# whatshap/whatshap

Hardware: AMD Instinct MI355X
Metric: variant-columns/sec at max-coverage 20 (bipartition-costs/sec reported alongside) (higher is better)
Workload: dtype u32; 1 GPU; synthetic diploid single-individual, max-coverage 20: 1 block of 200000 SNVs (BASELINE configs[2]); blocks=1, blocks_in_flight_per_gpu=1, tables_per_launch=1, max_coverage=20, optimal_cost_checksum=1611545, rendezvous=none

## Files before the change

include/whatshap_amd_debug.h:

```cpp
#ifndef WHATSHAP_AMD_DEBUG_H
#define WHATSHAP_AMD_DEBUG_H

#include "whatshap_amd.h"

#ifdef __cplusplus
extern "C" {
#endif

whamd_status_t whamd_debug_emulate_slot_plan(const whamd_readset_view* readset, const uint32_t* recombcost, size_t n_recombcost,
                                            const whamd_pedigree_view* pedigree, int distrust_genotypes,
                                            const uint32_t* positions, size_t n_positions, int slot_l, int symmetry,
                                            uint32_t* index_out, uint32_t* score_out, uint64_t* n_run_columns_out);

whamd_status_t whamd_debug_emulate_pedslot_plan(const whamd_readset_view* readset, const uint32_t* recombcost, size_t n_recombcost,
                                               const whamd_pedigree_view* pedigree, int distrust_genotypes,
                                               const uint32_t* positions, size_t n_positions, int slot_l,
                                               uint32_t* index_out, uint32_t* transmission_out, uint32_t* score_out,
                                               uint64_t* n_run_columns_out);

whamd_status_t whamd_debug_lazy_terms_check(const whamd_readset_view* readset, const uint32_t* recombcost, size_t n_recombcost,
                                            const whamd_pedigree_view* pedigree, int distrust_genotypes,
                                            const uint32_t* positions, size_t n_positions, const uint8_t* need, int rounds,
                                            int* lazy_out, uint64_t* differences_out, uint64_t* built_before_out, uint64_t* built_after_out);

// ... 5 lines not shown
whamd_status_t whamd_debug_realign_detect_host(const whamd_realign_alignments_view* alignments, const whamd_realign_variants_view* variants,
                                               const whamd_realign_reference_view* reference, const whamd_realign_params* params,
                                               whamd_realign** out);
whamd_status_t whamd_debug_edit_distance_host(uint64_t n_pairs, const uint64_t* query_ptr, const uint8_t* query, const uint64_t* target_ptr,
                                              const uint8_t* target, int use_affine, const float* mismatch_cost, int32_t gap_start,
                                              int32_t gap_extend, int64_t* distance_out);

whamd_status_t whamd_debug_poly_score_host(const whamd_poly_matrix_view* matrices, uint64_t n_matrices, uint32_t min_overlap, uint32_t ploidy,
                                           double err, whamd_poly_scores** out);

whamd_status_t whamd_debug_progeny_score_host(const whamd_progeny_view* problems, uint64_t n_problems, whamd_progeny_scores** out);
whamd_status_t whamd_debug_progeny_score_entries_host(const whamd_progeny_view* problem, uint64_t n_entries, const uint32_t* i, const uint32_t* j,
                                                      double* score_out, uint8_t* stored_out);
whamd_status_t whamd_debug_progeny_pair_score_host(const float* gl, uint64_t n_positions, uint32_t n_samples, uint32_t ploidy, uint64_t pos1,
                                                   uint64_t pos2, uint32_t kind, double* score_out);
whamd_status_t whamd_debug_progeny_variant_types_host(const float* gl, uint64_t n_positions, uint32_t n_samples, uint32_t ploidy, const double* priors,
                                                      const uint32_t* nodes, uint64_t n_nodes, double* llh_out, uint32_t* g0_out, uint32_t* g1_out);

whamd_status_t whamd_debug_haplotag_host(const whamd_haplotag_view* problems, uint64_t n_problems, whamd_haplotag_result** out);

typedef struct whamd_debug_kernel {
	const void* kernel;
	const char* name;
	int32_t large_lds_opted_in;
	int32_t debug_only;
} whamd_debug_kernel;
size_t whamd_debug_solve_kernels(whamd_debug_kernel* out, size_t capacity);

enum {
	WHAMD_LAUNCH_COLUMN = 0,
	WHAMD_LAUNCH_RUN = 1,
	WHAMD_LAUNCH_SLOT_RUN = 2,
	WHAMD_LAUNCH_BATCH = 3,
	WHAMD_LAUNCH_GROUP = 4,
	WHAMD_LAUNCH_GROUP_WALK = 5,
	WHAMD_LAUNCH_TAIL = 6,
	WHAMD_LAUNCH_WINDOW_WALK = 7,
	WHAMD_LAUNCH_TABLES = 8
};

typedef struct whamd_debug_launch {
	const void* kernel;
	uint32_t site;
	uint32_t grid_x, grid_y, block;
	uint32_t lds;
	uint32_t own_stream;
	uint32_t forward;
	int32_t lr, yflags, spec, stamps, tb, nf, ncols, threads;
	int32_t streamed, pack;
	int32_t tight, variant;
	int32_t T, n_ind, mode, wide;
	int32_t ped, sym;
	int32_t entries;
	uint64_t count;
	const char* name;
} whamd_debug_launch;
whamd_status_t whamd_debug_dptable_launches(const whamd_dptable* table, whamd_debug_launch* out, size_t capacity, size_t* n_out);

#ifdef __cplusplus
}
#endif

#endif
```

whatshap_amd/_native.py:

```python

from __future__ import annotations

import ctypes as C
import os
import threading
from typing import Optional, Sequence

import numpy as np

_HERE = os.path.dirname(os.path.abspath(__file__))
LIB_PATH = os.path.join(_HERE, "libwhatshap_amd.so")
DEBUG_LIB_PATH = os.path.join(_HERE, "libwhatshap_amd_debug.so")
ABI_VERSION = 2

WHAMD_OK = 0
WHAMD_ERR_INVALID = 1
WHAMD_ERR_MENDELIAN_CONFLICT = 2
WHAMD_ERR_UNSORTED = 3
WHAMD_ERR_UNSUPPORTED = 4
WHAMD_ERR_DEVICE = 5
WHAMD_ERR_OVERFLOW = 6
WHAMD_ERR_HOST = 7
GT_OTHER = 255

# ... 274 lines not shown
                f"{LIB_PATH} is missing: build the HIP extension first "
                "(python -c 'import __graft_entry__ as g; g.build()' or make -C whatshap_amd/csrc). "
                "whatshap_amd has no CPU fallback."
            )
        _lib = _bind(C.CDLL(LIB_PATH), LIB_PATH)
    return _lib


def debug_lib() -> C.CDLL:
    global _debug_lib
    if _debug_lib is not None:
        return _debug_lib
    if not os.path.exists(DEBUG_LIB_PATH):
        raise ImportError(f"{DEBUG_LIB_PATH} is missing: make -C whatshap_amd/csrc debug (tests and timing scripts only)")
    L = _bind(C.CDLL(DEBUG_LIB_PATH), DEBUG_LIB_PATH)
    L.whamd_debug_emulate_slot_plan.restype = C.c_int
    L.whamd_debug_emulate_slot_plan.argtypes = [
        C.POINTER(ReadSetView), C.POINTER(C.c_uint32), C.c_size_t, C.POINTER(PedigreeView), C.c_int,
        C.POINTER(C.c_uint32), C.c_size_t, C.c_int, C.c_int, C.POINTER(C.c_uint32), C.POINTER(C.c_uint32), C.POINTER(C.c_uint64),
    ]
    L.whamd_debug_emulate_pedslot_plan.restype = C.c_int
    L.whamd_debug_emulate_pedslot_plan.argtypes = [
        C.POINTER(ReadSetView), C.POINTER(C.c_uint32), C.c_size_t, C.POINTER(PedigreeView), C.c_int,
        C.POINTER(C.c_uint32), C.c_size_t, C.c_int, C.POINTER(C.c_uint32), C.POINTER(C.c_uint32), C.POINTER(C.c_uint32), C.POINTER(C.c_uint64),
    ]
    L.whamd_debug_pedmec_heuristic_create_host.restype = C.c_int
    L.whamd_debug_pedmec_heuristic_create_host.argtypes = [C.POINTER(ReadSetView), C.POINTER(C.c_uint32), C.c_size_t, C.POINTER(PedigreeView), C.c_int,
                                                           C.POINTER(C.c_uint32), C.c_size_t, C.c_uint32, C.c_int, C.POINTER(C.c_void_p)]
    L.whamd_debug_realign_detect_host.restype = C.c_int
    L.whamd_debug_realign_detect_host.argtypes = [C.POINTER(RealignAlignmentsView), C.POINTER(RealignVariantsView), C.POINTER(RealignReferenceView),
                                                  C.POINTER(RealignParams), C.POINTER(C.c_void_p)]
    L.whamd_debug_edit_distance_host.restype = C.c_int
    L.whamd_debug_edit_distance_host.argtypes = [C.c_uint64, C.POINTER(C.c_uint64), C.POINTER(C.c_uint8), C.POINTER(C.c_uint64), C.POINTER(C.c_uint8),
                                                 C.c_int, C.POINTER(C.c_float), C.c_int32, C.c_int32, C.POINTER(C.c_int64)]
    L.whamd_debug_poly_score_host.restype = C.c_int
    L.whamd_debug_poly_score_host.argtypes = [C.POINTER(PolyMatrixView), C.c_uint64, C.c_uint32, C.c_uint32, C.c_double, C.POINTER(C.c_void_p)]
    L.whamd_debug_progeny_score_host.restype = C.c_int
    L.whamd_debug_progeny_score_host.argtypes = [C.POINTER(ProgenyView), C.c_uint64, C.POINTER(C.c_void_p)]
    L.whamd_debug_progeny_score_entries_host.restype = C.c_int
    L.whamd_debug_progeny_score_entries_host.argtypes = [C.POINTER(ProgenyView), C.c_uint64, C.POINTER(C.c_uint32), C.POINTER(C.c_uint32),
                                                         C.POINTER(C.c_double), C.POINTER(C.c_uint8)]
    L.whamd_debug_progeny_pair_score_host.restype = C.c_int
    L.whamd_debug_progeny_pair_score_host.argtypes = [C.POINTER(C.c_float), C.c_uint64, C.c_uint32, C.c_uint32, C.c_uint64, C.c_uint64, C.c_uint32,
                                                      C.POINTER(C.c_double)]
    L.whamd_debug_progeny_variant_types_host.restype = C.c_int
    L.whamd_debug_progeny_variant_types_host.argtypes = [C.POINTER(C.c_float), C.c_uint64, C.c_uint32, C.c_uint32, C.POINTER(C.c_double), C.POINTER(C.c_uint32),
                                                         C.c_uint64, C.POINTER(C.c_double), C.POINTER(C.c_uint32), C.POINTER(C.c_uint32)]
    L.whamd_debug_haplotag_host.restype = C.c_int
    L.whamd_debug_haplotag_host.argtypes = [C.POINTER(HaplotagView), C.c_uint64, C.POINTER(C.c_void_p)]
    L.whamd_debug_solve_kernels.restype = C.c_size_t
    L.whamd_debug_solve_kernels.argtypes = [C.POINTER(DebugKernel), C.c_size_t]
    L.whamd_debug_dptable_launches.restype = C.c_int
    L.whamd_debug_dptable_launches.argtypes = [C.c_void_p, C.POINTER(DebugLaunch), C.c_size_t, C.POINTER(C.c_size_t)]
    _debug_lib = L
    return L


def use_debug_library() -> None:
    global _lib
    _lib = debug_lib()


def _bind(L: C.CDLL, path: str) -> C.CDLL:
    H = C.c_void_p
    L.whamd_abi_version.restype = C.c_int
    L.whamd_device_count.restype = C.c_int
    L.whamd_last_error.restype = C.c_char_p
    L.whamd_dptable_create.restype = C.c_int
    L.whamd_dptable_create.argtypes = [
        C.POINTER(ReadSetView), C.POINTER(C.c_uint32), C.c_size_t, C.POINTER(PedigreeView), C.c_int,
        C.POINTER(C.c_uint32), C.c_size_t, C.c_int, C.POINTER(H),
    ]
    L.whamd_dptable_create_with_options.restype = C.c_int
    L.whamd_dptable_create_with_options.argtypes = [
        C.POINTER(ReadSetView), C.POINTER(C.c_uint32), C.c_size_t, C.POINTER(PedigreeView), C.c_int,
        C.POINTER(C.c_uint32), C.c_size_t, C.POINTER(C.c_char_p), C.POINTER(C.c_char_p), C.c_size_t, C.c_int, C.POINTER(H),
    ]
    L.whamd_dptable_solve.restype = C.c_int
    L.whamd_dptable_solve.argtypes = [H]
    L.whamd_dptable_enqueue.restype = C.c_int
    L.whamd_dptable_enqueue.argtypes = [H]
    L.whamd_dptable_wait.restype = C.c_int
    L.whamd_dptable_wait.argtypes = [H]
    L.whamd_dptable_enqueue_many.restype = C.c_int
    L.whamd_dptable_enqueue_many.argtypes = [C.POINTER(H), C.c_size_t]
    L.whamd_dptable_wait_many.restype = C.c_int
    L.whamd_dptable_wait_many.argtypes = [C.POINTER(H), C.c_size_t]
    L.whamd_dptable_release_device.restype = C.c_int
    L.whamd_dptable_release_device.argtypes = [H]
    L.whamd_dptable_destroy.restype = None
    L.whamd_dptable_destroy.argtypes = [H]
    L.whamd_dptable_column_count.restype = C.c_uint64
    L.whamd_dptable_column_count.argtypes = [H]
    L.whamd_dptable_individual_count.restype = C.c_uint32
    L.whamd_dptable_individual_count.argtypes = [H]
    L.whamd_dptable_read_count.restype = C.c_uint32
    L.whamd_dptable_read_count.argtypes = [H]
    L.whamd_dptable_positions.restype = C.c_int
    L.whamd_dptable_positions.argtypes = [H, C.POINTER(C.c_uint32)]
    L.whamd_dptable_get_optimal_score.restype = C.c_int
    L.whamd_dptable_get_optimal_score.argtypes = [H, C.POINTER(C.c_uint32)]
    L.whamd_dptable_get_super_reads.restype = C.c_int
    L.whamd_dptable_get_super_reads.argtypes = [
        H, C.POINTER(C.c_uint8), C.POINTER(C.c_uint8), C.POINTER(C.c_uint32), C.POINTER(C.c_uint32), C.POINTER(C.c_uint32),
    ]
    L.whamd_dptable_get_optimal_partitioning.restype = C.c_int
# ... 260 lines not shown
def plan_summary(problem: ProblemArrays, path: str = "auto") -> dict:
    out = PlanSummary()
    _check(lib().whamd_plan_summarize(*problem.call_args(), path.encode(), C.byref(out)))
    return out.as_dict()


def emulate_slot_plan(problem: ProblemArrays, n_columns: int, slot_l: int = 11, symmetry: int = 1, slot_r: int = 2):
    if slot_r >= 3:
        slot_l += 100
    elif slot_r <= 1:
        slot_l += 200
    idx = np.zeros(max(n_columns, 1), dtype=np.uint32)
    score = C.c_uint32()
    ncols = C.c_uint64()
    D = debug_lib()
    _check(D.whamd_debug_emulate_slot_plan(*problem.call_args(), C.c_int(slot_l), C.c_int(symmetry), _ptr(idx, C.c_uint32),
                                           C.byref(score), C.byref(ncols)), D)
    return idx[:n_columns], int(score.value), int(ncols.value)


def emulate_pedslot_plan(problem: ProblemArrays, n_columns: int, slot_l: int = 0):
    idx = np.zeros(max(n_columns, 1), dtype=np.uint32)
    trans = np.zeros(max(n_columns, 1), dtype=np.uint32)
    score = C.c_uint32()
    ncols = C.c_uint64()
    D = debug_lib()
    _check(D.whamd_debug_emulate_pedslot_plan(*problem.call_args(), C.c_int(slot_l), _ptr(idx, C.c_uint32), _ptr(trans, C.c_uint32),
                                              C.byref(score), C.byref(ncols)), D)
    return idx[:n_columns], trans[:n_columns], int(score.value), int(ncols.value)


def debug_lazy_terms_check(problem: ProblemArrays, need=None, rounds: int = 1) -> dict:
    D = debug_lib()
    fn = D.whamd_debug_lazy_terms_check
    fn.restype = C.c_int
    lazy, diff, before, after = C.c_int(), C.c_uint64(), C.c_uint64(), C.c_uint64()
    need_arr = None if need is None else np.ascontiguousarray(need, dtype=np.uint8)
    _check(fn(*problem.call_args(), None if need_arr is None else _ptr(need_arr, C.c_uint8), C.c_int(int(rounds)), C.byref(lazy), C.byref(diff),
              C.byref(before), C.byref(after)), D)
    return {"lazy": bool(lazy.value), "differences": int(diff.value), "built_before": int(before.value), "built_after": int(after.value)}


class DebugKernel(C.Structure):
    _fields_ = [("kernel", C.c_void_p), ("name", C.c_char_p), ("large_lds_opted_in", C.c_int32), ("debug_only", C.c_int32)]


LAUNCH_SITES = ("column", "run", "slot_run", "batch", "group", "group_walk", "tail", "window_walk", "tables")
LAUNCH_FACTS = ("lr", "yflags", "spec", "stamps", "tb", "nf", "ncols", "threads", "streamed", "pack", "tight", "variant", "T", "n_ind", "mode", "wide",
                "ped", "sym", "entries")


class DebugLaunch(C.Structure):
    _fields_ = ([("kernel", C.c_void_p), ("site", C.c_uint32), ("grid_x", C.c_uint32), ("grid_y", C.c_uint32), ("block", C.c_uint32), ("lds", C.c_uint32),
                 ("own_stream", C.c_uint32), ("forward", C.c_uint32)] + [(f, C.c_int32) for f in LAUNCH_FACTS] + [("count", C.c_uint64), ("name", C.c_char_p)])


def debug_solve_kernels() -> list:
    D = debug_lib()
    n = D.whamd_debug_solve_kernels(None, 0)
    arr = (DebugKernel * n)()
    D.whamd_debug_solve_kernels(arr, n)
    return [{"kernel": k.kernel, "name": k.name.decode(), "large_lds_opted_in": bool(k.large_lds_opted_in), "debug_only": bool(k.debug_only)} for k in arr]


def debug_launches(table) -> list:
    D = debug_lib()
    if table._L is not D:
        raise ValueError("the launch ledger exists in the debug library only (use_debug_library() before the table is made)")
    n = C.c_size_t()
    _check(D.whamd_debug_dptable_launches(table._h, None, 0, C.byref(n)), D)
    arr = (DebugLaunch * max(n.value, 1))()
    _check(D.whamd_debug_dptable_launches(table._h, arr, n.value, C.byref(n)), D)
    out = []
    for r in arr[:n.value]:
        if r.name is None:
            raise RuntimeError(f"a launch of site {LAUNCH_SITES[r.site]} (grid {r.grid_x} x {r.grid_y}, block {r.block}) took a kernel the registry does not list")
        rec = {"name": r.name.decode(), "site": LAUNCH_SITES[r.site], "grid_x": r.grid_x, "grid_y": r.grid_y, "block": r.block, "lds": r.lds,
               "own_stream": bool(r.own_stream), "forward": bool(r.forward), "count": int(r.count)}
        rec.update({f: (None if getattr(r, f) < 0 else getattr(r, f)) for f in LAUNCH_FACTS})
        out.append(rec)
    return out


def _heuristic_result(L, h) -> dict:
    n = int(L.whamd_pedmec_heuristic_column_count(h))
    ns = int(L.whamd_pedmec_heuristic_sample_count(h))
    nr = int(L.whamd_pedmec_heuristic_read_count(h))
    score = C.c_float()
    bip = np.zeros(max(nr, 1), dtype=np.uint8)
    trans = np.zeros(max(n, 1), dtype=np.uint32)
    haps = np.zeros((max(ns, 1), 2, max(n, 1)), dtype=np.int8)
    mut = np.zeros((max(ns, 1), 2, max(n, 1)), dtype=np.uint8)
    sid = np.zeros(max(ns, 1), dtype=np.uint32)
    pos = np.zeros(max(n, 1), dtype=np.uint32)
    _check(L.whamd_pedmec_heuristic_get(h, C.byref(score), _ptr(bip, C.c_uint8), _ptr(trans, C.c_uint32), haps.ctypes.data_as(C.POINTER(C.c_int8)),
                                        _ptr(mut, C.c_uint8), _ptr(sid, C.c_uint32), _ptr(pos, C.c_uint32)), L)
    stats = HeuristicStats()
    _check(L.whamd_pedmec_heuristic_get_stats(h, C.byref(stats)), L)
    return {"score": float(score.value), "bipartition": bip[:nr], "transmission": trans[:n], "haplotypes": haps[:ns, :, :n], "mutated": mut[:ns, :, :n],
            "sample_ids": sid[:ns], "positions": pos[:n], "stats": stats.as_dict()}


def pedmec_heuristic(problem: ProblemArrays, row_limit: int = 256, allow_mutations: bool = True, device: int = 0, host_diagnostic: bool = False) -> dict:
    L = debug_lib() if host_diagnostic else lib()
    h = C.c_void_p()
    a = problem.call_args()
    if host_diagnostic:
        _check(L.whamd_debug_pedmec_heuristic_create_host(*a, C.c_uint32(int(row_limit)), C.c_int(1 if allow_mutations else 0), C.byref(h)), L)
    else:
        _check(L.whamd_pedmec_heuristic_create(*a, C.c_uint32(int(row_limit)), C.c_int(1 if allow_mutations else 0), C.c_int(int(device)), C.byref(h)))
    try:
        return _heuristic_result(L, h)
    finally:
        L.whamd_pedmec_heuristic_destroy(h)


class HeuristicBatch:

    def __init__(self, problems, row_limit: int = 256, allow_mutations: bool = True, device: int = 0):
        L = lib()
        problems = list(problems)
        self._L = L
        self._n = len(problems)
        self._handles = (C.c_void_p * max(self._n, 1))()
        jobs = (HeuristicJob * max(self._n, 1))()
        for i, p in enumerate(problems):
            jobs[i].readset = C.pointer(p.readset_view)
            jobs[i].recombcost = _ptr(p.recombcost, C.c_uint32)
            jobs[i].n_recombcost = p.recombcost.size
            jobs[i].pedigree = C.pointer(p.pedigree_view)
            jobs[i].distrust_genotypes = 1 if p.distrust_genotypes else 0
# ... 97 lines not shown
```

whatshap_amd/blocks.py:

```python

from __future__ import annotations

import contextlib

from typing import Dict, List, Sequence, Tuple

import numpy as np

from ._native import ProblemArrays


def block_weight(n_columns: int, coverage: int, transmissions: int = 1) -> float:
    return float(n_columns) * float(2 ** coverage) * float(transmissions) ** 2


def assign_blocks(weights: Sequence[float], world_size: int) -> List[List[int]]:
    order = sorted(range(len(weights)), key=lambda b: (-weights[b], b))
    load = [0.0] * world_size
    out: List[List[int]] = [[] for _ in range(world_size)]
    for b in order:
        r = min(range(world_size), key=lambda i: (load[i], i))
        out[r].append(b)
        load[r] += weights[b]
    return out
# ... 35 lines not shown
    out = []
    for b, (c0, c1) in enumerate(bounds):
        reads = order[cuts[b]:cuts[b + 1]]
        lengths = lengths_all[reads]
        if reads.size and np.all(np.diff(reads) == 1):
            sel = slice(int(ptr[reads[0]]), int(ptr[reads[-1] + 1]))
        else:
            sel = np.concatenate([np.arange(ptr[r], ptr[r + 1]) for r in reads]) if reads.size else np.zeros(0, np.int64)
        sub_ptr = np.zeros(reads.size + 1, dtype=np.uint64)
        sub_ptr[1:] = np.cumsum(lengths)
        sub = ProblemArrays(sub_ptr, problem.var_position[sel], problem.var_allele[sel], problem.var_quality[sel],
                            problem.read_sample_id[reads], problem.individual_id, problem.triple_ids, geno[:, c0:c1],
                            None if gl is None else gl[:, c0:c1, :], recomb[c0:c1], positions[c0:c1],
                            problem.distrust_genotypes, n_variants=c1 - c0)
        out.append((sub, reads, (c0, c1)))
    return out


_CREATE_POOLS = {}


@contextlib.contextmanager
def _create_pool(n_workers: int):
    from concurrent.futures import ThreadPoolExecutor

    pool = _CREATE_POOLS.get(n_workers)
    if pool is None:
        pool = _CREATE_POOLS[n_workers] = ThreadPoolExecutor(max_workers=n_workers, thread_name_prefix="whamd-create")
    yield pool


def solve_blocks(problems: Sequence[ProblemArrays], device: int = 0, path=None, max_in_flight: int = 8,
                 release: bool = True, devices: Sequence[int] = None, weights: Sequence[float] = None, create_threads: int = None,
                 windows_on_device: int = 1, trace: list = None, eager_create: bool = False, host_threads_per_create: int = None):
    from ._native import NativeTable, device_count, enqueue_many, wait_many

    problems = list(problems)
    if create_threads is None or host_threads_per_create is None:
        import os

        n_cpus = len(os.sched_getaffinity(0))
        if create_threads is None:
            create_threads = max(1, min(16, n_cpus))
        if host_threads_per_create is None:
            host_threads_per_create = max(1, min(2, n_cpus // max(1, create_threads)))
    if devices is None:
        from concurrent.futures import ThreadPoolExecutor

        windows = [problems[start:start + max_in_flight] for start in range(0, len(problems), max_in_flight)]
        tables = []
        n_workers = max(1, min(create_threads, max_in_flight))
        with _create_pool(n_workers) as pool:
            def options_of(window):
                opts = {}
                if len(window) > 4:
                    opts["shared_launches"] = "1"
                if n_workers > 1 and len(window) > 1:
                    opts["host_threads"] = str(max(1, int(host_threads_per_create)))
                return opts or None

            def create(sub, opts):
                return NativeTable(sub, device=device, path=path, solve=False, options=opts)

            def submit_window(window):
                opts = options_of(window)
                return [pool.submit(create, sub, opts) for sub in window]

            all_pending = [submit_window(w) for w in windows] if eager_create else None
            pending = (all_pending[0] if eager_create else submit_window(windows[0])) if windows else []
            releases = []
            in_flight = None

            def collect(window):
                wait_many(window)
                if release:
                    releases.extend(pool.submit(t.release_device) for t in window)
                tables.extend(window)

            import time
            t_begin = time.perf_counter()

            def mark(what, wi):
                if trace is not None:
                    trace.append((what, wi, (time.perf_counter() - t_begin) * 1e3))

            window = None
            ok = False
            try:
                for wi in range(len(windows)):
                    window = [f.result() for f in pending]
                    pending = []
                    mark("created", wi)
                    enqueue_many(window)
                    mark("enqueued", wi)
                    pending = ((all_pending[wi + 1] if eager_create else submit_window(windows[wi + 1])) if wi + 1 < len(windows) else [])
                    if windows_on_device < 2:
                        collect(window)
                        window = None
                        mark("collected", wi)
                        continue
                    if in_flight is not None:
                        done, in_flight = in_flight, None
                        collect(done)
                        mark("collected", wi - 1)
                    in_flight, window = window, None
                if in_flight is not None:
                    done, in_flight = in_flight, None
                    collect(done)
                ok = True
            finally:
                if not ok:
                    leftovers = list(in_flight or []) + [t for t in (window or []) if t not in (in_flight or [])]
# ... 255 lines not shown
```

whatshap_amd/csrc/c_api.cpp:

```cpp
#include <chrono>
#include <cstdio>
#include <cstdlib>
#include <cstring>
#include <functional>
#include <memory>
#include <new>
#include <stdexcept>
#include <string>

#include "debug_build.h"
#ifdef WHAMD_DEBUG_BUILD
#include "../../include/whatshap_amd_debug.h"
#endif
#include "device_runtime.h"
#include "device_table.h"
#include "genotype.h"
#include "heuristic.h"
#include "host_parallel.h"
#include "problem.h"
#include "resident.h"
#include "slots.h"
#include <algorithm>
#include <vector>

// ... 31 lines not shown
		return fail(WHAMD_ERR_HOST, "host-side failure (unknown exception)");
	}
}

double now_ms() {
	return std::chrono::duration<double, std::milli>(std::chrono::steady_clock::now().time_since_epoch()).count();
}

}

namespace whamd {
void set_last_error(const std::string& msg) { g_last_error = msg; }
}

extern "C" {

int whamd_abi_version(void) { return WHAMD_ABI_VERSION; }

int whamd_device_count(void) { return DeviceTable::device_count(); }

whamd_status_t whamd_device_pci_bus_id(int device, char* out, size_t capacity) {
	if (!out || capacity < 16) return fail(WHAMD_ERR_INVALID, "whamd_device_pci_bus_id: buffer of at least 16 bytes expected");
	std::string id;
	if (!DeviceTable::device_pci_bus_id(device, id)) return fail(WHAMD_ERR_DEVICE, "no HIP device " + std::to_string(device));
	if (id.size() + 1 > capacity) return fail(WHAMD_ERR_INVALID, "whamd_device_pci_bus_id: buffer too small");
	std::memcpy(out, id.c_str(), id.size() + 1);
	return WHAMD_OK;
}

const char* whamd_last_error(void) { return g_last_error.c_str(); }

namespace {
whamd_status_t apply_option(whamd_dptable* t, const std::string& k, const char* value);

whamd_status_t create_table(const whamd_readset_view* readset, const uint32_t* recombcost, size_t n_recombcost, const whamd_pedigree_view* pedigree,
                            int distrust_genotypes, const uint32_t* positions, size_t n_positions, const char* const* keys, const char* const* values,
                            size_t n_options, int device, whamd_dptable** out) {
	if (!out) return fail(WHAMD_ERR_INVALID, "out is NULL");
	*out = nullptr;
	if (n_options && (!keys || !values)) return fail(WHAMD_ERR_INVALID, "option arrays are NULL");
	const double t0 = now_ms();
	std::unique_ptr<whamd_dptable> t(new whamd_dptable());
	std::string msg;
	struct ThreadsGuard { uint32_t saved = whamd::host_threads_override(); ~ThreadsGuard() { whamd::host_threads_override() = saved; } } threads_guard;
	for (size_t i = 0; i < n_options; ++i) {
		if (!keys[i] || !values[i]) return fail(WHAMD_ERR_INVALID, "null option");
		if (std::string(keys[i]) == "host_threads") whamd::host_threads_override() = (uint32_t)std::max(0, std::atoi(values[i]));
	}
	whamd_status_t st = build_problem(readset, recombcost, n_recombcost, pedigree, distrust_genotypes != 0,
	                                  positions, n_positions, t->problem, msg, false, true);
	if (st != WHAMD_OK) return fail(st, msg);
	const double t1 = now_ms();
	t->device_index = device;
	for (size_t i = 0; i < n_options; ++i) {
		if (std::string(keys[i]) == "host_threads") continue;
		st = apply_option(t.get(), keys[i], values[i]);
		if (st != WHAMD_OK) return st;
	}
	st = t->device.upload(t->problem, device, msg);
	if (st != WHAMD_OK) return fail(st, msg);
	if (getenv("WHAMD_DEBUG_TIMING"))
		fprintf(stderr, "[whamd timing] create: flatten %.1f ms, plan + upload %.1f ms\n", t1 - t0, now_ms() - t1);
	t->uploaded = true;
	t->stats.host_prepare_ms = now_ms() - t0;
	t->stats.host_flatten_ms = t1 - t0;
	*out = t.release();
	return WHAMD_OK;
}
}

whamd_status_t whamd_dptable_create(const whamd_readset_view* readset, const uint32_t* recombcost,
                                    size_t n_recombcost, const whamd_pedigree_view* pedigree,
                                    int distrust_genotypes, const uint32_t* positions, size_t n_positions,
                                    int device, whamd_dptable** out) {
	return guarded([&]() -> whamd_status_t {
		return create_table(readset, recombcost, n_recombcost, pedigree, distrust_genotypes, positions, n_positions, nullptr, nullptr, 0, device, out);
	});
}

whamd_status_t whamd_dptable_create_with_options(const whamd_readset_view* readset, const uint32_t* recombcost,
                                                 size_t n_recombcost, const whamd_pedigree_view* pedigree,
                                                 int distrust_genotypes, const uint32_t* positions, size_t n_positions,
                                                 const char* const* keys, const char* const* values, size_t n_options,
                                                 int device, whamd_dptable** out) {
	return guarded([&]() -> whamd_status_t {
		return create_table(readset, recombcost, n_recombcost, pedigree, distrust_genotypes, positions, n_positions, keys, values, n_options, device, out);
	});
}

namespace {

whamd_status_t begin_enqueue(whamd_dptable* t) {
	if (!t) return fail(WHAMD_ERR_INVALID, "table is NULL");
	if (t->in_flight) return fail(WHAMD_ERR_INVALID, "a solve of this table is already in flight");
	std::string msg;
	if (!t->uploaded) {
		whamd_status_t st = t->device.upload(t->problem, t->device_index, msg);
		if (st != WHAMD_OK) return fail(st, msg);
		t->uploaded = true;
	}
	const Problem& p = t->problem;
	whamd_solve_stats& s = t->stats;
	s.n_columns = p.n_cols;
	s.n_cells = p.n_cells;
	s.n_costs = p.n_cells * p.T;
	s.algorithmic_bytes = p.algorithmic_bytes;
	s.max_coverage = p.max_k;
	s.transmissions = p.T;
	t->solved = false;
	return WHAMD_OK;
}

// ... 238 lines not shown
	if (index_out) std::memcpy(index_out, s.path_index.data(), s.path_index.size() * sizeof(uint32_t));
	if (transmission_out) std::memcpy(transmission_out, s.path_trans.data(), s.path_trans.size() * sizeof(uint32_t));
	return WHAMD_OK;
}

whamd_status_t whamd_dptable_get_stats(const whamd_dptable* t, whamd_solve_stats* stats_out) {
	if (!t || !stats_out) return fail(WHAMD_ERR_INVALID, "null argument");
	whamd_dptable* tt = const_cast<whamd_dptable*>(t);
	if (t->solved && !t->in_flight) tt->device.read_timing(tt->stats);
	*stats_out = t->stats;
	return WHAMD_OK;
}

namespace {
whamd_status_t apply_option(whamd_dptable* t, const std::string& k, const char* value) {
	const std::string v(value);
	if (k == "path") {
		if (!t->device.set_path(v)) return fail(WHAMD_ERR_INVALID, "unknown path '" + v + "' (auto, slots, resident, column, column_keys)");
		t->uploaded = false;
		return WHAMD_OK;
	}
	if (k == "resident_fold") {
		t->device.set_fold(v != "0");
		t->uploaded = false;
		return WHAMD_OK;
	}
	if (k == "symmetry") {
		t->device.set_symmetry(std::atoi(value));
		t->uploaded = false;
		return WHAMD_OK;
	}
	if (k == "lanes") {
		t->device.set_lanes(std::atoi(value));
		t->uploaded = false;
		return WHAMD_OK;
	}
	if (k == "resident_l") {
		t->device.set_l_pref(std::atoi(value));
		t->uploaded = false;
		return WHAMD_OK;
	}
	if (k == "slot_l") {
		t->device.set_slot_l(std::atoi(value));
		t->uploaded = false;
		return WHAMD_OK;
	}
	if (k == "slot_r") {
		t->device.set_slot_lr(std::atoi(value));
		t->uploaded = false;
		return WHAMD_OK;
	}
	if (k == "shared_launches") {
		t->device.set_shared_launches(v != "0");
		t->uploaded = false;
		return WHAMD_OK;
	}
	if (k == "arena_limit_bytes") {
		t->device.set_arena_limit(std::strtoull(value, nullptr, 10));
		t->uploaded = false;
		return WHAMD_OK;
	}
	return fail(WHAMD_ERR_INVALID, "unknown option '" + k + "'");
}
}

whamd_status_t whamd_dptable_set_option(whamd_dptable* t, const char* key, const char* value) {
	if (!t || !key || !value) return fail(WHAMD_ERR_INVALID, "null argument");
	return apply_option(t, key, value);
}

whamd_status_t whamd_plan_summarize(const whamd_readset_view* readset, const uint32_t* recombcost, size_t n_recombcost,
                                    const whamd_pedigree_view* pedigree, int distrust_genotypes,
                                    const uint32_t* positions, size_t n_positions, const char* path,
                                    whamd_plan_summary* out) {
	return guarded([&]() -> whamd_status_t {
	if (!out) return fail(WHAMD_ERR_INVALID, "out is NULL");
	Problem p;
	std::string msg;
	const double tb0 = now_ms();
	const std::string mode(path ? path : "auto");
	whamd_status_t st = build_problem(readset, recombcost, n_recombcost, pedigree, distrust_genotypes != 0, positions,
	                                  n_positions, p, msg, mode == "genotype_slots");
	if (st != WHAMD_OK) return fail(st, msg);
	SlotPlan sp;
	if (mode == "genotype_slots") {
		whamd_plan_summary s{};
		s.n_columns = p.n_cols;
		s.max_coverage = p.max_k;
		if (plan_forward_slots(p, 0, 0, sp, 0, true)) {
			s.n_steps = sp.steps.size();
			s.n_runs = sp.runs.size();
			bool ok = true;
			uint32_t expect = 0;
			for (const Step& step : sp.steps) {
				if (step.kind != 2) {
					if (debug_env("WHAMD_DEBUG_PLAN")) fprintf(stderr, "[plan] genotype: column %u outside runs (k=%u b=%u f=%u, next k=%u)\n", step.index, p.k[step.index], p.b[step.index], p.f[step.index], step.index + 1 < p.n_cols ? p.k[step.index + 1] : 0);
					ok = ok && step.index == expect; expect = step.index + 1; continue;
				}
				const SlotRun& run = sp.runs[step.index];
				ok = ok && run.c0 == expect && run.lr == 0 && !run.half && run.ncols >= 1 && run.ncols <= (uint32_t)PSLOT_MAXCOLS;
				expect = run.c0 + run.ncols;
				s.n_resident_columns += run.ncols;
				s.max_run_columns = std::max<uint64_t>(s.max_run_columns, run.ncols);
				s.max_workgroups = std::max<uint64_t>(s.max_workgroups, 1ull << run.g);
				uint32_t starts = 0, ends = 0;
				for (uint32_t i = 0; i < run.ncols; ++i) {
// ... 208 lines not shown
                                            const whamd_pedigree_view* pedigree, int distrust_genotypes, const uint32_t* positions, size_t n_positions,
                                            const uint8_t* need_in, int rounds, int* lazy_out, uint64_t* differences_out, uint64_t* built_before_out,
                                            uint64_t* built_after_out) {
	return guarded([&]() -> whamd_status_t {
	Problem eager, lazy;
	std::string msg;
	whamd_status_t st = build_problem(readset, recombcost, n_recombcost, pedigree, distrust_genotypes != 0, positions, n_positions, eager, msg);
	if (st != WHAMD_OK) return fail(st, msg);
	st = build_problem(readset, recombcost, n_recombcost, pedigree, distrust_genotypes != 0, positions, n_positions, lazy, msg, false, true);
	if (st != WHAMD_OK) return fail(st, msg);
	if (lazy_out) *lazy_out = lazy.lazy_terms ? 1 : 0;
	const uint32_t n = eager.n_cols;
	uint64_t before = 0, after = 0, diff = 0;
	for (uint32_t c = 0; c < n; ++c) before += lazy.term_end(c, lazy.T - 1) > lazy.term_begin(c, 0);
	std::vector<uint8_t> need(n, 1);
	if (need_in) for (uint32_t c = 0; c < n; ++c) need[c] = need_in[c] != 0;
	rounds = std::max(1, rounds);
	for (int r = 0; r < rounds; ++r) {
		std::vector<uint8_t> part(n, 0);
		for (uint32_t c = 0; c < n; ++c) part[c] = need[c] && (int)(c % (uint32_t)rounds) == r;
		st = fill_lazy_terms(lazy, part, msg);
		if (st != WHAMD_OK) return fail(st, msg);
	}
	for (uint32_t c = 0; c < n; ++c) {
		after += lazy.term_end(c, lazy.T - 1) > lazy.term_begin(c, 0);
		if (!need[c]) continue;
		bool same = true;
		for (uint32_t t = 0; t < eager.T && same; ++t) {
			const uint64_t a0 = eager.term_begin(c, t), a1 = eager.term_end(c, t), b0 = lazy.term_begin(c, t), b1 = lazy.term_end(c, t);
			same = a1 - a0 == b1 - b0;
			for (uint64_t i = 0; same && i < a1 - a0; ++i)
				same = eager.terms[a0 + i].c == lazy.terms[b0 + i].c && eager.terms[a0 + i].plus == lazy.terms[b0 + i].plus && eager.terms[a0 + i].minus == lazy.terms[b0 + i].minus;
		}
		diff += !same;
	}
	if (eager.fterm_kind != lazy.fterm_kind || eager.fterms.size() != lazy.fterms.size()) diff += n;
	else for (size_t i = 0; i < eager.fterms.size(); ++i) if (eager.fterms[i].c != lazy.fterms[i].c || eager.fterms[i].plus != lazy.fterms[i].plus || eager.fterms[i].minus != lazy.fterms[i].minus) { ++diff; break; }
	if (lazy.value_bound < eager.value_bound) diff += n;
	if (differences_out) *differences_out = diff;
	if (built_before_out) *built_before_out = before;
	if (built_after_out) *built_after_out = after;
	return WHAMD_OK;
	});
}

size_t whamd_debug_solve_kernels(whamd_debug_kernel* out, size_t capacity) { return DeviceTable::debug_solve_kernels(out, capacity); }

whamd_status_t whamd_debug_dptable_launches(const whamd_dptable* table, whamd_debug_launch* out, size_t capacity, size_t* n_out) {
	if (!table || !n_out) return fail(WHAMD_ERR_INVALID, "null argument");
	if (!table->solved) return fail(WHAMD_ERR_INVALID, "the table has not been solved: its ledger is read after whamd_dptable_wait");
	*n_out = table->device.debug_launches(out, capacity);
	return WHAMD_OK;
}
#endif

}

struct whamd_heuristic;
struct HeuristicBatchState {
	whamd::HeurBatch batch;
	std::vector<whamd_heuristic*> members;
	bool collected = false;
	whamd_status_t status = WHAMD_OK;
	std::string message;
	double t_enqueued = 0.0;
};

struct whamd_heuristic {
	whamd::HeurPlan plan;
	whamd::HeurResult result;
	whamd_heuristic_stats stats{};
	std::shared_ptr<HeuristicBatchState> batch;
	bool finished = false;
};

namespace {
whamd_status_t heuristic_collect(whamd_heuristic* h) {
	if (h->finished) return WHAMD_OK;
	if (!h->batch) return fail(WHAMD_ERR_INVALID, "whamd_pedmec_heuristic_enqueue has not run");
	std::shared_ptr<HeuristicBatchState> st = h->batch;
	if (!st->collected) {
		st->collected = true;
		std::vector<whamd::HeurResult> results(st->members.size());
		st->status = st->batch.wait(results.data(), st->message);
		if (st->status == WHAMD_OK) {
			const double t_done = now_ms();
			whamd::parallel_ranges(st->members.size(), whamd::host_threads(st->members.size(), 1), [&](uint64_t i0, uint64_t i1, uint32_t) {
				for (uint64_t i = i0; i < i1; ++i) {
					whamd_heuristic* m = st->members[i];
					const double t0 = now_ms();
					m->result = std::move(results[i]);
					whamd::heuristic_finish(m->plan, m->result);
					m->stats.max_solutions = m->result.max_solutions;
					m->stats.total_solutions = m->result.total_solutions;
					m->stats.device_ms = m->result.device_ms;
					m->stats.host_prepare_ms += std::max(0.0, (t_done - st->t_enqueued) - m->result.device_ms);
					m->stats.host_finish_ms = now_ms() - t0;
				}
			});
		}
		for (whamd_heuristic* m : st->members) { m->finished = st->status == WHAMD_OK; m->batch.reset(); }
	}
	if (st->status != WHAMD_OK) return fail(st->status, st->message);
	return WHAMD_OK;
}

// ... 188 lines not shown
```

whatshap_amd/csrc/device_table.h:

```cpp
#pragma once
#include <string>

#ifdef WHAMD_DEBUG_BUILD
#include "../../include/whatshap_amd_debug.h"
#endif
#include "device_types.h"
#include "problem.h"

namespace whamd {

class DeviceTable {
public:
	DeviceTable();
	~DeviceTable();
	DeviceTable(const DeviceTable&) = delete;
	DeviceTable& operator=(const DeviceTable&) = delete;

	static int device_count();
	static bool device_pci_bus_id(int device, std::string& out);
	whamd_status_t upload(Problem& p, int device, std::string& msg);
	whamd_status_t solve(const Problem& p, Solution& s, whamd_solve_stats& st, std::string& msg);
	whamd_status_t enqueue(const Problem& p, Solution& s, std::string& msg);
	whamd_status_t enqueue_some(const Problem& p, Solution& s, uint64_t budget, bool& done, std::string& msg);
	whamd_status_t wait(const Problem& p, Solution& s, whamd_solve_stats& st, std::string& msg);
	void read_timing(whamd_solve_stats& st);
	static whamd_status_t enqueue_group(DeviceTable* const* tables, const Problem* const* problems, Solution* const* solutions, size_t n_tables, std::string& msg);
	static void wait_last_of_each_stream(DeviceTable* const* tables, size_t n_tables);
	bool group_eligible(const Problem& p) const;
	int device_index() const;
	uint32_t widest_launch() const;
	void abort_enqueue();
	void release_device();
	bool set_path(const std::string& path);
	void set_l_pref(int l);
	void set_slot_l(int l);
	void set_slot_lr(int lr);
	void set_fold(bool v);
	void set_symmetry(int level);
	void set_lanes(int n);
	void set_arena_limit(uint64_t bytes);
	void set_shared_launches(bool v);
	void set_side_by_side(bool v);

#ifdef WHAMD_DEBUG_BUILD
	static size_t debug_solve_kernels(whamd_debug_kernel* out, size_t capacity);
	size_t debug_launches(whamd_debug_launch* out, size_t capacity) const;
#endif

private:
	whamd_status_t enqueue_some_unguarded(const Problem& p, Solution& s, uint64_t budget, bool& done, std::string& msg);
	struct Impl;
	Impl* impl_;
};

}
```

whatshap_amd/csrc/dp_device.hip:

```cpp
#include <hip/hip_runtime.h>

#include <algorithm>
#include <atomic>
#include <cctype>
#include <chrono>
#include <cstdio>
#include <cstdlib>
#include <cstring>
#include <mutex>
#include <string>
#include <vector>

#include "debug_build.h"
#ifdef WHAMD_DEBUG_BUILD
#include "../../include/whatshap_amd_debug.h"
#endif
#include "device_runtime.h"
#include "device_table.h"
#include "genotype.h"

namespace whamd {

namespace {

// ... 266 lines not shown
	std::vector<SuperStep> schedule;
	struct StepBrief { uint32_t entry_off, lds; uint16_t entry_count; uint8_t has_singles, pad; };
	struct EntryBrief { uint16_t grid_x, threads; uint32_t lds_x; GroupVariantPair variant; uint8_t pad[2]; };
	std::vector<StepBrief> step_brief;
	std::vector<EntryBrief> entry_brief;
	std::vector<ResBatchEntry> entries;
	ResBatchEntry* d_entries = nullptr;
	bool use_chunks = false;
	std::vector<BtChunk> chunks;
	BtChunk* d_chunks = nullptr;
	uint32_t* d_unit_x = nullptr;
	uint32_t* d_path2 = nullptr;
	uint32_t* d_trans2 = nullptr;
	uint32_t n_orient_max = 1;
	uint8_t* d_sel = nullptr;
	uint32_t* d_guess = nullptr;
	uint32_t* d_bt_counters = nullptr;
	uint32_t n_spec = 0;
	size_t chunk_lds = 0;
	SlotPlan splan;
	bool use_slots = false;
	int slot_l = 11;
	bool slot_l_set = false;
	int slot_lr = 2;
	int slot_lr_used = 2;
	std::vector<SlotBatchEntry> slot_entries;
	SlotBatchEntry* d_slot_entries = nullptr;
	uint64_t table_bytes = 0;
	BtJob* d_btjobs = nullptr;
	uint32_t* d_job_scores = nullptr;
	bool shared_hint = false;
	bool side_by_side = false;
	int max_lanes = 32;
	struct Window {
		uint32_t step_lo = 0, step_hi = 0;
		uint32_t unit_off = 0, unit_count = 0;
	};
	uint64_t arena_limit = 0;
	bool windowed = false;
	std::vector<Window> windows;
	uint8_t* d_checkpoints = nullptr;
	size_t checkpoint_bytes = 0;
	uint32_t* d_bt_state = nullptr;
	BtJob* d_window_jobs = nullptr;

	whamd_status_t open(int dev, std::string& msg);
	whamd_status_t choose_plan(Problem& p, TableBuild& b, std::string& msg);
	void dump_plan(const Problem& p) const;
	whamd_status_t describe_columns(const Problem& p, TableBuild& b, std::string& msg);
	whamd_status_t lay_out_arena(const Problem& p, TableBuild& b, std::string& msg);
	size_t upload_bound(const Problem& p, const TableBuild& b) const;
	whamd_status_t upload_column_arrays(const Problem& p, TableBuild& b, TableUploader& up, std::string& msg);
	void build_slot_blobs(TableBuild& b) const;
	uint64_t lay_out_slot_tables(const TableBuild& b);
	whamd_status_t upload_slot_arrays(TableBuild& b, TableUploader& up, std::string& msg);
	void make_jobs();
	void make_units(const TableBuild& b);
	whamd_status_t make_windows(const TableBuild& b, TableUploader& up, std::string& msg);
	whamd_status_t take_result_block(uint32_t n, TableUploader& up, std::string& msg);
	whamd_status_t make_chunks(const Problem& p, TableUploader& up, std::string& msg);
	whamd_status_t take_solve_buffers(const Problem& p, TableBuild& b, TableUploader& up, std::string& msg);
	whamd_status_t make_lanes(const TableBuild& b, TableUploader& up, std::string& msg);
	whamd_status_t make_schedule(const TableBuild& b, std::string& msg);
	void make_briefs();
	whamd_status_t upload_entries(TableUploader& up, std::string& msg);
	whamd_status_t launch_table_kernels(const Problem& p, const TableBuild& b, TableUploader& up, std::string& msg);
	whamd_status_t arm_debug_stamps(TableUploader& up, std::string& msg);
	whamd_status_t record_group_backtrace(uint32_t n, TableUploader& up, std::string& msg);
	struct SolveInFlight {
		hipStream_t run_stream = nullptr;
		uint32_t group_tables = 1;
		bool enqueue_open = false;
		size_t next_super = 0;
		uint64_t launches = 0;
		hipStream_t tail_stream = nullptr;
		uint64_t tail_seq = 0;
		bool tail_elsewhere = false;
		bool timing_pending = false;
		static inline std::atomic<uint64_t> tails_submitted{0};
		void rewind(hipStream_t own) { enqueue_open = false; next_super = 0; run_stream = own; }
	} inflight;
#ifdef WHAMD_DEBUG_BUILD
	std::vector<whamd_debug_launch> ledger;
	void note(uint32_t site, const void* kernel, dim3 grid, dim3 block, size_t lds, hipStream_t on, bool forward, const LaunchFacts& facts);
#endif
	struct GroupSubmission;
	void launch_column_step(const Problem& p, const Step& step, const Lane& lane, const uint32_t* prev, uint32_t* cur, uint64_t& launches);
	void launch_run(const ResBatchEntry& e, uint64_t& launches);
	void launch_slot_run(const SlotBatchEntry& e, uint64_t& launches);
	whamd_status_t begin_solve(const Problem& p, Solution& s, std::string& msg);
	whamd_status_t submit_super_step(const Problem& p, const SuperStep& ss, uint64_t& launches, std::string& msg);
	whamd_status_t submit_singles(const Problem& p, const SuperStep& ss, uint64_t& launches, std::string& msg);
	whamd_status_t submit_tail(const Problem& p, std::string& msg, hipStream_t tail_stream = nullptr, bool walked_by_group = false);
	whamd_status_t report_slot_stamps(std::string& msg) const;
	whamd_status_t report_resident_stamps(std::string& msg) const;
	BtGroupEntry h_bt_entry{};
	BtGroupEntry* d_bt_entry = nullptr;
	bool device_superreads = false;
	SuperreadArgs super_args{};
	size_t super_words = 0, super_off = 0;
	bool own_stream_used = false;
	bool upload_pending = false;
	hipStream_t upload_stream = nullptr;

	void adopt(const StreamSet& ss) { stream = ss.stream; ev0 = ss.ev[0]; ev1 = ss.ev[1]; ev2 = ss.ev[2]; ev3 = ss.ev[3]; ev_group = ss.ev[4]; ev_upload = ss.ev[5]; }
	StreamSet stream_set() const {
		StreamSet ss;
		ss.stream = stream; ss.ev[0] = ev0; ss.ev[1] = ev1; ss.ev[2] = ev2; ss.ev[3] = ev3; ss.ev[4] = ev_group; ss.ev[5] = ev_upload; ss.device = device;
		return ss;
	}

	void release_lanes() {
		max_grid_x = 1;
		lanes.clear();
		jobs.clear();
		schedule.clear();
		entries.clear();
		slot_entries.clear();
		windows.clear();
	}

	void release() {
		if (inflight.tail_elsewhere && ev3) (void)hipEventSynchronize(ev3);
		inflight.tail_elsewhere = false;
		if (upload_pending && ev_upload) (void)hipEventSynchronize(ev_upload);
		upload_pending = false;
		release_lanes();
		windowed = false;
		if (stream && own_stream_used && (!allocations.empty() || d_arena)) { (void)hipStreamSynchronize(stream); own_stream_used = false; }
		for (auto& a : allocations) devpool_give(device, a.first, a.second);
		allocations.clear();
		arena_give(device, d_arena, arena_bytes);
		d_arena = nullptr;
		arena_bytes = 0;
		pinned_give(h_pinned, h_pinned_bytes);
		h_pinned = nullptr;
		d_cols = nullptr;
		d_units = nullptr;
		d_pr[0] = d_pr[1] = nullptr;
		d_path_index = d_path_trans = d_score = nullptr;
	}
};

DeviceTable::DeviceTable() : impl_(new Impl()) {}

DeviceTable::~DeviceTable() {
	if (impl_) {
		release_device();
		delete impl_;
	}
}

void DeviceTable::release_device() {
	Impl& m = *impl_;
	(void)hipSetDevice(m.device);
	m.release();
	if (m.stream) {
		if (m.own_stream_used) (void)hipStreamSynchronize(m.stream);
		m.own_stream_used = false;
		streamset_give(m.stream_set());
	}
	m.adopt(StreamSet());
	m.inflight.run_stream = nullptr;
	m.inflight.timing_pending = false;
}

int DeviceTable::device_count() {
	int n = 0;
	if (hipGetDeviceCount(&n) != hipSuccess) return 0;
	return n;
}

bool DeviceTable::device_pci_bus_id(int device, std::string& out) {
	int n = 0;
	if (hipGetDeviceCount(&n) != hipSuccess || device < 0 || device >= n) return false;
	char text[64] = {0};
	if (hipDeviceGetPCIBusId(text, (int)sizeof text - 1, device) != hipSuccess) return false;
	out = text;
	for (char& ch : out) ch = (char)tolower((unsigned char)ch);
	return true;
}

static void append_segments(uint32_t mask, std::vector<uint32_t>& out, uint16_t& count) {
	uint32_t src = 0;
	count = 0;
	for (uint32_t bit = 0; bit < 32;) {
		if (!((mask >> bit) & 1u)) { ++bit; continue; }
		uint32_t len = 0;
		while (bit + len < 32 && ((mask >> (bit + len)) & 1u)) ++len;
		out.push_back(src | (bit << 8) | (len << 16));
		++count;
		src += len;
		bit += len;
	}
}

bool DeviceTable::set_path(const std::string& path) {
	if (path != "auto" && path != "column" && path != "column_keys" && path != "resident" && path != "slots") return false;
	impl_->path = path;
	return true;
}

void DeviceTable::set_l_pref(int l) { impl_->l_pref = std::max(4, std::min(l, RES_LMAX)); }
void DeviceTable::set_lanes(int n) { impl_->max_lanes = n < 1 ? 1 : (n > 64 ? 64 : n); }

void DeviceTable::set_fold(bool v) { impl_->fold = v; }
void DeviceTable::set_slot_l(int l) { impl_->slot_l = std::max(2, std::min(l, 12)); impl_->slot_l_set = true; }
void DeviceTable::set_slot_lr(int lr) { impl_->slot_lr = lr >= 3 ? 3 : (lr <= 1 ? 1 : 2); }

void DeviceTable::set_arena_limit(uint64_t bytes) { impl_->arena_limit = bytes; }
void DeviceTable::set_shared_launches(bool v) { impl_->shared_hint = v; }
void DeviceTable::set_side_by_side(bool v) { impl_->side_by_side = v; }
void DeviceTable::set_symmetry(int level) { impl_->symmetry = level < 0 ? 0 : (level > 2 ? 2 : level); }


whamd_status_t DeviceTable::Impl::open(int dev, std::string& msg) {
	Impl& m = *this;
	m.device = dev;
	const whamd_status_t opened = open_device(dev, msg);
	if (opened != WHAMD_OK) return opened;
	if (!m.stream) {
		StreamSet ss;
		if (!streamset_take(dev, ss)) { msg = "could not create the table's stream and events"; return WHAMD_ERR_DEVICE; }
		m.adopt(ss);
	}
	m.release();
	return WHAMD_OK;
}

whamd_status_t DeviceTable::Impl::choose_plan(Problem& p, TableBuild& b, std::string& msg) {
	Impl& m = *this;
	m.wide = !select_kernels(p.T, p.n_ind, m.fused, m.keysfn);
	if (m.wide && (p.T > (uint32_t)MAX_T_WIDE || p.n_ind > (uint32_t)MAX_IND_WIDE)) {
		msg = "no device kernel for T=" + std::to_string(p.T) + ", individuals=" + std::to_string(p.n_ind);
		return WHAMD_ERR_UNSUPPORTED;
	}
	for (uint32_t c = 0; c < p.n_cols && !m.wide; ++c) m.wide = p.term_end(c, p.T - 1) - p.term_begin(c, 0) > (uint64_t)COL_MAXTERMS;
	b.force_keys = m.path == "column_keys" || m.wide;
	const bool want_resident = (m.path == "auto" || m.path == "resident") && !m.wide;
	size_t free_b = 0, total_b = 0;
	HIP_TRY(hipMemGetInfo(&free_b, &total_b));
	if (free_b < total_b / 2) {
		genotype_release_cache();
		HIP_TRY(hipMemGetInfo(&free_b, &total_b));
	}
	if (free_b < total_b / 4) {
		arena_release();
		devpool_release();
		HIP_TRY(hipMemGetInfo(&free_b, &total_b));
	}
	free_b += arena_idle_bytes(m.device);
	b.free_b = free_b;
	int slot_lr = m.slot_lr, slot_l = m.slot_l;
	if (m.shared_hint && p.T == 1 && p.max_k >= 18 && !m.slot_l_set && m.slot_lr == 2) { slot_lr = 3; slot_l = 12; }
	if (p.T == 1 && p.max_k >= 21 && p.max_k <= 22 && !m.slot_l_set && m.slot_lr == 2 && !debug_env("WHAMD_NO_WIDE_LAYOUT")) { slot_lr = 3; slot_l = 12; }
	m.slot_lr_used = slot_lr;
	m.use_slots = (m.path == "auto" || m.path == "slots") && !m.wide && plan_forward_slots(p, p.T > 1 ? (m.slot_l_set ? -m.slot_l : 0) : std::max(8, slot_l), m.symmetry, m.splan, slot_lr);
	if (m.use_slots && m.splan.ped && m.splan.table_words * 4ull > free_b / 4) m.use_slots = false;
	m.table_bytes = m.use_slots && m.splan.ped ? m.splan.table_words * 4ull : 0ull;
	if (p.lazy_terms) {
		std::vector<uint8_t> need(p.n_cols, 1);
		if (m.use_slots && m.splan.ped) for (uint32_t c = 0; c < p.n_cols; ++c) need[c] = m.splan.col_to_row[c] < 0;
		const whamd_status_t st = fill_lazy_terms(p, need, msg);
		if (st != WHAMD_OK) return st;
	}
	if (m.use_slots) {
		m.plan = ResidentPlan();
		m.plan.steps = m.splan.steps;
		m.plan.component_first_step = m.splan.component_first_step;
		m.plan.col_to_res.assign(p.n_cols, -1);
	} else {
		m.splan = SlotPlan();
		plan_forward(p, want_resident, m.l_pref, m.fold, m.plan, m.symmetry);
	}
	m.device_superreads = p.n_ind == 1 && p.T == 1 && p.P == 2 && !p.distrust && p.h2p.size() >= 2 && p.h2p[0] == 0 && p.h2p[1] == 1 && p.genotype.size() >= p.n_cols &&
	                      !debug_env("WHAMD_HOST_SUPERREADS");
	return WHAMD_OK;
}

void DeviceTable::Impl::dump_plan(const Problem& p) const {
	const Impl& m = *this;
	for (const Step& st : m.plan.steps) {
		if (st.kind == 0) { fprintf(stderr, "[plan] column %u k=%u b=%u f=%u\n", st.index, p.k[st.index], p.b[st.index], p.f[st.index]); continue; }
		if (st.kind == 2) {
			const SlotRun& r = m.splan.runs[st.index];
			fprintf(stderr, "[plan] slot run c0=%u ncols=%u g=%u L=%u half=%u ends=%u has_prev=%u in_identity=%u in_half=%u mirror_pos=%u in_occ=%x out_occ=%x mirror_out=%u\n",
			        r.c0, r.ncols, r.g, r.L, r.half, r.n_ends, r.has_prev, r.in_identity, r.in_half, r.in_mirror_pos, r.in_occ, r.out_occ, r.mirror_out);
			if (m.splan.ped) fprintf(stderr, "[plan]   pedigree run: T=%u forms per value=%u table words=%u record words per workgroup=%u\n", 1u << m.splan.pextra[st.index].tb,
			                         m.splan.pextra[st.index].nf, m.splan.pextra[st.index].s_off + r.ncols * 64u * pslot_ns(m.splan.pextra[st.index].nf), m.splan.pextra[st.index].rec_words);
			continue;
		}
		const ResSegment& sgm = m.plan.segments[st.index];
		fprintf(stderr, "[plan] run c0=%u ncols=%u g=%u threads=%u max_l=%u stage_words=%u\n", sgm.c0, sgm.ncols, sgm.g, sgm.threads, sgm.max_l, sgm.stage_words);
		for (uint32_t i = 0; i < sgm.ncols; ++i) {
			const ResColumn& rc = m.plan.columns[sgm.col_off + i];
			const ResBacktrace& rb = m.plan.backtrace[sgm.col_off + i];
			fprintf(stderr, "[plan]   col %u mode=%u nfold=%u Lb=%u Lf=%u ebits=%u epos0=%u nthr=%u stage_off=%u nwords=%u | bt layout=%u n_g=%u n_l=%u\n",
			        sgm.c0 + i, rc.mode, rc.nfold, rc.Lb, rc.Lf, rc.ebits, rc.epos[0], rc.nthr, rc.stage_off, rc.nwords, rb.layout, rb.n_g, rb.n_l);
		}
	}
}

whamd_status_t DeviceTable::Impl::describe_columns(const Problem& p, TableBuild& b, std::string& msg) {
	Impl& m = *this;
	const uint32_t n = b.n, ni = b.ni, tbits = b.tbits;
	if (p.terms.size() >= 0xFFFFFFFFull || (uint64_t)p.col_ptr[n] * ni >= 0xFFFFFFFFull) {
		msg = "problem too large for 32-bit device offsets";
		return WHAMD_ERR_UNSUPPORTED;
	}
	m.cols.resize(n);
	b.term_ptr32.resize((size_t)n * (p.T + 1));
	RawVec<uint32_t>& term_ptr32 = b.term_ptr32;
	parallel_ranges(n, host_threads(n, 16384), [&m, &p, &term_ptr32, n, ni, tbits](uint64_t c0, uint64_t c1, uint32_t) {
		for (uint32_t c = (uint32_t)c0; c < (uint32_t)c1; ++c) {
			DevColumn d{};
			d.k = p.k[c];
			d.b = p.b[c];
			d.f = p.f[c];
			d.recomb = p.recomb[c];
			d.delta_off = (uint32_t)(p.col_ptr[c] * ni);
			d.term_off = (uint32_t)((size_t)c * (p.T + 1));
			for (uint32_t t = 0; t <= p.T; ++t) term_ptr32[(size_t)c * (p.T + 1) + t] = (uint32_t)p.term_ptr[(size_t)c * p.T + t];
			d.ebits = d.k - d.f;
			d.is_last = (c + 1 == n);
			d.eloop = std::min<uint32_t>(d.ebits, QMAX);
			d.nplanes = d.ebits + tbits;
			m.cols[c] = d;
		}
	});
	return WHAMD_OK;
}

whamd_status_t DeviceTable::Impl::lay_out_arena(const Problem& p, TableBuild& b, std::string& msg) {
	Impl& m = *this;
	const uint32_t n = b.n;
	const bool ped_slots = b.ped_slots;
	std::vector<uint32_t>& segs = b.segs;
	uint64_t bt = 0, seg_bt = 0;
	size_t seg_cursor = 0, slot_cursor = 0;
	uint32_t max_f = 0, max_keys_f = 0;
	const uint64_t reserve = (3ull << 30) + (uint64_t)n * 1024ull + m.table_bytes;
	auto slot_record_bytes = [&m, ped_slots](size_t ri) -> uint64_t {
		const SlotRun& run = m.splan.runs[ri];
		if (ped_slots) return (uint64_t)m.splan.pextra[ri].rec_words * 4ull << run.g;
		return (uint64_t)run.n_ends * run.threads * (1ull << (run.g - run.half));
	};
	uint64_t arena_cap = b.free_b > reserve ? b.free_b - reserve : 0;
	if (m.arena_limit) arena_cap = std::min<uint64_t>(arena_cap, m.arena_limit);
	b.arena_cap = arena_cap;
	std::vector<uint32_t>& window_first_col = b.window_first_col;
	uint64_t bt_max = 0;
	auto open_unit = [&bt, &bt_max, &window_first_col, arena_cap](uint32_t c, uint64_t bytes) -> bool {
		if (bytes + 16 > arena_cap) return false;
		if (bt + bytes + 16 > arena_cap) {
			bt_max = std::max(bt_max, bt);
			bt = 0;
			window_first_col.push_back(c);
		}
		return true;
	};
	auto unit_too_large = [&msg, &b](uint32_t c) {
		msg = "the backtrace record of the unit at column " + std::to_string(c) + " alone does not fit in the arena (" + std::to_string(b.arena_cap >> 20) +
		      " MiB of " + std::to_string(b.free_b >> 20) + " MiB free HBM)";
		return WHAMD_ERR_UNSUPPORTED;
	};
	for (uint32_t c = 0; c < n; ++c) {
		DevColumn& d = m.cols[c];
		const bool in_slot_run = m.use_slots && m.splan.col_to_row[c] >= 0;
		d.seg_off = (uint32_t)segs.size();
		const uint32_t kmask = d.k >= 32 ? 0xFFFFFFFFu : ((1u << d.k) - 1u);
		if (!in_slot_run) {
			append_segments(p.fwd_mask[c], segs, d.nseg_fwd);
			append_segments(kmask & ~p.fwd_mask[c], segs, d.nseg_end);
		}
		d.bt_off = bt;
		if (m.use_slots && m.splan.col_to_row[c] >= 0) {
			d.mode = 3;
			d.res_idx = (uint32_t)m.splan.col_to_row[c];
			if (slot_cursor < m.splan.runs.size() && m.splan.runs[slot_cursor].c0 == c) {
				SlotRun& run = m.splan.runs[slot_cursor];
				if (!open_unit(c, slot_record_bytes(slot_cursor))) return unit_too_large(c);
				run.rec_lo = (uint32_t)bt;
				run.rec_hi = (uint32_t)(bt >> 32);
				seg_bt = bt;
				bt += slot_record_bytes(slot_cursor);
				max_f = std::max(max_f, run.L + run.g);
				++slot_cursor;
			}
			d.bt_off = seg_bt;
		} else if (m.plan.col_to_res[c] >= 0) {
			d.mode = 2;
			d.res_idx = (uint32_t)m.plan.col_to_res[c];
			if (seg_cursor < m.plan.segments.size() && m.plan.segments[seg_cursor].c0 == c) {
				ResSegment& sgm = m.plan.segments[seg_cursor];
				if (!open_unit(c, (uint64_t)sgm.stage_words * (1ull << sgm.g) * 8ull)) return unit_too_large(c);
				sgm.bt_lo = (uint32_t)bt;
				sgm.bt_hi = (uint32_t)(bt >> 32);
				seg_bt = bt;
				bt += (uint64_t)sgm.stage_words * (1ull << sgm.g) * 8ull;
				++seg_cursor;
			}
			d.bt_off = seg_bt;
		} else {
			const bool fused_ok = !b.force_keys && !d.is_last && d.f >= 6 && d.ebits <= (uint32_t)QMAX;
			d.mode = fused_ok ? 0u : 1u;
			const uint64_t bytes = d.mode == 0 ? (uint64_t)d.nplanes * p.T * (1ull << (d.f - 6)) * 8ull : (uint64_t)p.T * (1ull << d.f) * 4ull;
			if (!open_unit(c, bytes)) return unit_too_large(c);
			d.bt_off = bt;
			bt += bytes;
			if (d.mode != 0) max_keys_f = std::max(max_keys_f, d.f);
		}
		bt = (bt + 15ull) & ~15ull;
		max_f = std::max(max_f, d.f);
	}
	b.laps.lap("column descriptors (host)");
	bt = std::max(bt_max, bt);
	b.bt = bt;
	b.max_f = max_f;
	b.max_keys_f = max_keys_f;
	b.exchange_bytes = (size_t)(1ull << max_f) * p.T * 4;
	m.bt_bytes = bt;
	m.windowed = !window_first_col.empty();
	m.checkpoint_bytes = b.exchange_bytes;
	const uint64_t need = bt + (2ull + window_first_col.size()) * b.exchange_bytes + (1ull << max_keys_f) * p.T * 8ull;
	if (need + (1ull << 30) > b.free_b) {
		msg = "backtrace arena of " + std::to_string(need >> 20) + " MiB does not fit in free HBM (" + std::to_string(b.free_b >> 20) + " MiB)";
		return WHAMD_ERR_UNSUPPORTED;
	}
	return WHAMD_OK;
}

size_t DeviceTable::Impl::upload_bound(const Problem& p, const TableBuild& b) const {
	const Impl& m = *this;
	const size_t delta_count = p.n_ind == 0 ? std::max<size_t>(p.col_ptr[b.n], 1) : (size_t)p.col_ptr[b.n] * p.n_ind;
	const size_t super_upload = m.device_superreads ? ((size_t)b.n + 1) * 8 + b.n + 1024 : 0;
	return m.cols.size() * sizeof(DevColumn) + delta_count * sizeof(int32_t) + b.term_ptr32.size() * 4 + (p.terms.size() + p.fterms.size()) * sizeof(DevTerm) + b.segs.size() * 4 +
	       m.plan.columns.size() * (sizeof(ResColumn) + sizeof(ResBacktrace) + sizeof(PedColumn)) + m.plan.ped_terms.size() * sizeof(PedTerm) +
	       (m.splan.rows.size() + SLOT_ROW_PAD) * sizeof(SlotRow) + m.splan.prows.size() * sizeof(PedSlotRow) + m.splan.bt_cols.size() * (sizeof(SlotBtCol) + 8) +
	       m.splan.runs.size() * (sizeof(SlotRun) + sizeof(PedSlotExtra) + sizeof(BtUnit) + sizeof(SlotBatchEntry) + 64) + m.plan.segments.size() * (sizeof(ResBatchEntry) + sizeof(BtUnit)) + super_upload + ((size_t)8 << 20);
}

whamd_status_t DeviceTable::Impl::upload_column_arrays(const Problem& p, TableBuild& b, TableUploader& up, std::string& msg) {
	Impl& m = *this;
	const uint32_t n = b.n;
	static_assert(sizeof(CostTerm) == sizeof(DevTerm), "Problem::terms / fterms are uploaded as they are");
	const RawVec<CostTerm>& terms = p.terms;
	const int32_t* delta_src = p.delta.data();
	size_t delta_count = (size_t)p.col_ptr[n] * p.n_ind;
	if (p.n_ind == 0) { b.delta_fallback.assign(std::max<size_t>(p.col_ptr[n], 1), 0); delta_src = b.delta_fallback.data(); delta_count = b.delta_fallback.size(); }
	const bool sparse_columns = m.use_slots && !b.ped_slots && p.T == 1 && !m.windowed && !debug_env("WHAMD_DENSE_COLUMN_UPLOAD");
	if (sparse_columns) {
		std::vector<std::pair<size_t, size_t>> pc_cols, pc_delta, pc_tptr, pc_terms;
		for (uint32_t c = 0; c < n;) {
			if (m.splan.col_to_row[c] >= 0) { ++c; continue; }
			uint32_t e = c + 1;
			while (e < n && m.splan.col_to_row[e] < 0) ++e;
			pc_cols.emplace_back((size_t)c * sizeof(DevColumn), (size_t)e * sizeof(DevColumn));
			pc_delta.emplace_back((size_t)p.col_ptr[c] * p.n_ind * sizeof(int32_t), (size_t)p.col_ptr[e] * p.n_ind * sizeof(int32_t));
			pc_tptr.emplace_back((size_t)c * (p.T + 1) * sizeof(uint32_t), (size_t)e * (p.T + 1) * sizeof(uint32_t));
// ... 9 lines not shown
		HIP_TRY(up.up((void**)&m.d_cols, m.cols.data(), m.cols.size() * sizeof(DevColumn)));
		HIP_TRY(up.up((void**)&m.dp.delta, delta_src, delta_count * sizeof(int32_t)));
		HIP_TRY(up.up((void**)&m.dp.term_ptr, b.term_ptr32.data(), b.term_ptr32.size() * sizeof(uint32_t)));
		HIP_TRY(up.up((void**)&m.dp.terms, terms.data(), terms.size() * sizeof(DevTerm)));
	}
	m.dp.cols = m.d_cols;
	if (m.device_superreads) {
		m.super_args = SuperreadArgs{};
		HIP_TRY(up.up((void**)&m.super_args.col_ptr, p.col_ptr.data(), ((size_t)n + 1) * sizeof(uint64_t)));
		HIP_TRY(up.up((void**)&m.super_args.genotype, p.genotype.data(), (size_t)n));
		m.super_args.delta = m.dp.delta;
		m.super_args.n_cols = n;
		m.super_words = (size_t)n + ((size_t)2 * n + 3) / 4;
	}
	b.d_fterms = nullptr;
	if (!p.fterms.empty()) HIP_TRY(up.up((void**)&b.d_fterms, p.fterms.data(), p.fterms.size() * sizeof(DevTerm)));
	HIP_TRY(up.up((void**)&m.dp.segs, b.segs.data(), b.segs.size() * sizeof(uint32_t)));
	HIP_TRY(up.up((void**)&m.dp.res_cols, m.plan.columns.data(), m.plan.columns.size() * sizeof(ResColumn)));
	HIP_TRY(up.up((void**)&m.dp.res_bt, m.plan.backtrace.data(), m.plan.backtrace.size() * sizeof(ResBacktrace)));
	m.plan.ped_columns.resize(m.plan.ped_columns.empty() ? 0 : m.plan.columns.size());
	HIP_TRY(up.up((void**)&m.dp.ped_cols, m.plan.ped_columns.data(), m.plan.ped_columns.size() * sizeof(PedColumn)));
	HIP_TRY(up.up((void**)&m.dp.ped_terms, m.plan.ped_terms.data(), m.plan.ped_terms.size() * sizeof(PedTerm)));
	b.laps.lap("column arrays: allocations + copies");
	return WHAMD_OK;
}

void DeviceTable::Impl::build_slot_blobs(TableBuild& b) const {
	const Impl& m = *this;
	b.slot_blob_off.assign(m.splan.runs.size(), 0);
	b.slot_blob_words.assign(m.splan.runs.size(), 0);
	size_t words = 0;
	for (size_t ri = 0; ri < m.splan.runs.size(); ++ri) {
		const SlotRun& run = m.splan.runs[ri];
		b.slot_blob_off[ri] = (uint32_t)words;
		b.slot_blob_words[ri] = (uint32_t)((size_t)run.ncols * (sizeof(SlotBtCol) / 4) + (run.n_ends + 3) / 4 + 1);
		words += b.slot_blob_words[ri];
	}
	b.slot_blob.resize(words);
	uint32_t* blob = b.slot_blob.data();
	const uint32_t* blob_off = b.slot_blob_off.data();
	parallel_ranges(m.splan.runs.size(), host_threads(m.splan.runs.size(), 512), [&m, blob, blob_off](uint64_t r0, uint64_t r1, uint32_t) {
		for (size_t ri = r0; ri < r1; ++ri) {
			const SlotRun& run = m.splan.runs[ri];
			uint32_t* dst = blob + blob_off[ri];
			const size_t col_words = (size_t)run.ncols * (sizeof(SlotBtCol) / 4);
			std::memcpy(dst, m.splan.bt_cols.data() + run.row_off, col_words * 4);
			const size_t end_words = (run.n_ends + 3) / 4 + 1;
			std::memset(dst + col_words, 0, end_words * 4);
			if (run.n_ends) std::memcpy(dst + col_words, m.splan.end_slots.data() + m.splan.end_off[ri], run.n_ends);
		}
	});
}

uint64_t DeviceTable::Impl::lay_out_slot_tables(const TableBuild& b) {
	Impl& m = *this;
	uint64_t slot_tab_words = 0;
	for (SlotRun& run : m.splan.runs) {
		auto pad4 = [](uint64_t v) { return (v + 3ull) & ~3ull; };
		const bool xrun = (run.yflags & 1u) && (run.lr == 2u || (run.lr == 3u && !debug_env("WHAMD_NO_XRUN8"))) && run.ncols <= (uint32_t)SLOT_XCOLS &&
		                  run.n_ends <= (uint32_t)SLOT_XENDS && !debug_env("WHAMD_NO_XRUN");
		const uint64_t ncp = xrun ? ((run.ncols + 7u) & ~7u) : run.ncols;
		run.tab_g = (uint32_t)slot_tab_words;
		slot_tab_words += pad4(ncp << (run.g - run.half));
		run.tab_w = (uint32_t)slot_tab_words;
		slot_tab_words += pad4(ncp * (run.threads >> 6));
		run.tab_sl = (uint32_t)slot_tab_words;
		slot_tab_words += ncp * 64u;
		if (xrun) {
			run.yflags |= 8u;
			slot_tab_words = (slot_tab_words + 15u) & ~(uint64_t)15;
			run.tab_kr = (uint32_t)slot_tab_words;
			slot_tab_words += pad4((((uint64_t)run.ncols + SLOT_XPAD) << run.lr) + run.ncols + SLOT_XPAD);
			run.tab_par = (uint32_t)slot_tab_words;
			slot_tab_words += pad4((uint64_t)run.threads + (1ull << (run.g - run.half)));
		}
	}
	slot_tab_words += (uint64_t)SLOT_XCOLS * 64u;
	if (b.laps.on) {
		size_t nx = 0, not_y = 0, not_lr = 0, long_run = 0, many_ends = 0;
		for (const SlotRun& run : m.splan.runs) {
			nx += (run.yflags & 8u) != 0;
			not_y += !(run.yflags & 1u); not_lr += run.lr != 2u && run.lr != 3u; long_run += run.ncols > (uint32_t)SLOT_XCOLS; many_ends += run.n_ends > (uint32_t)SLOT_XENDS;
		}
		fprintf(stderr, "[whamd timing]   X runs: %zu of %zu (not Y form %zu, cells per thread %zu, more than %d columns %zu, more than %d ending reads %zu)\n", nx, m.splan.runs.size(), not_y,
		        not_lr, SLOT_XCOLS, long_run, SLOT_XENDS, many_ends);
	}
	return slot_tab_words;
}

whamd_status_t DeviceTable::Impl::upload_slot_arrays(TableBuild& b, TableUploader& up, std::string& msg) {
	Impl& m = *this;
	build_slot_blobs(b);
	b.laps.lap("slot backtrace blobs (host)");
	if (!m.splan.rows.empty()) m.splan.rows.resize(m.splan.rows.size() + SLOT_ROW_PAD);
	HIP_TRY(up.up((void**)&m.dp.slot_rows, m.splan.rows.data(), m.splan.rows.size() * sizeof(SlotRow)));
	b.laps.lap("slot rows: allocation + copy");
	HIP_TRY(up.up((void**)&m.dp.slot_blob, b.slot_blob.data(), b.slot_blob.size() * sizeof(uint32_t)));
	HIP_TRY(up.up((void**)&m.dp.slot_ctrl, m.splan.ctrl.data(), m.splan.ctrl.size() * sizeof(uint32_t)));
	m.dp.slot_tab = nullptr;
	b.d_runs = nullptr;
	if (m.use_slots && !b.ped_slots) {
		const uint64_t slot_tab_words = lay_out_slot_tables(b);
		if (slot_tab_words >= 0xFFFFFFFFull) { msg = "slot-run tables exceed 32-bit offsets"; return WHAMD_ERR_UNSUPPORTED; }
		HIP_TRY(up.up((void**)&b.d_runs, m.splan.runs.data(), m.splan.runs.size() * sizeof(SlotRun)));
		b.laps.lap("slot blobs, control words, runs: allocations + copies");
		HIP_TRY(up.alloc((void**)&m.dp.slot_tab, slot_tab_words * 4));
		b.laps.lap("slot tables: allocation");
	}
	m.dp.pslot_rows = nullptr;
	m.dp.pslot_tab = nullptr;
	b.d_pextra = nullptr;
	if (b.ped_slots) {
		HIP_TRY(up.up((void**)&m.dp.pslot_rows, m.splan.prows.data(), m.splan.prows.size() * sizeof(PedSlotRow)));
		HIP_TRY(up.up((void**)&b.d_runs, m.splan.runs.data(), m.splan.runs.size() * sizeof(SlotRun)));
		HIP_TRY(up.up((void**)&b.d_pextra, m.splan.pextra.data(), m.splan.pextra.size() * sizeof(PedSlotExtra)));
		HIP_TRY(up.alloc((void**)&m.dp.pslot_tab, m.table_bytes));
	}
	b.laps.lap("slot rows / blobs / control words: allocations + copies");
	return WHAMD_OK;
}

void DeviceTable::Impl::make_jobs() {
	Impl& m = *this;
	m.release_lanes();
	Impl::Job final_job;
	final_job.final = true;
	std::vector<Impl::Job> component_jobs;
	const std::vector<uint32_t>& first = m.plan.component_first_step;
	size_t largest = 0;
	for (size_t k = 0; k < first.size(); ++k) largest = std::max<size_t>(largest, (k + 1 < first.size() ? first[k + 1] : m.plan.steps.size()) - first[k]);
	const bool worth_splitting = largest * 5 < m.plan.steps.size() * 4 || debug_env("WHAMD_SPLIT_COMPONENTS");
// ... 115 lines not shown
	m.d_bt_counters = res + 2 * (size_t)n + m.jobs.size();
	if (m.device_superreads) {
		m.super_args.out = res + m.super_off;
		m.super_args.path_index = m.d_path_index;
	}
	return WHAMD_OK;
}

namespace {

struct OrientationGenerators {
	std::vector<int> of_individual;
	std::vector<uint32_t> tflip;
	explicit OrientationGenerators(const Problem& p) : of_individual(std::max<uint32_t>(p.n_ind, 1), -1) {
		if (p.n_ind < 2 || p.n_ind > BT_GENERATORS) return;
		for (uint32_t s = 0; s < p.n_ind; ++s) {
			uint32_t as_parent = 0, as_child = 0;
			for (uint32_t t3 = 0; t3 < p.n_triples; ++t3) {
				if (p.triples[t3][0] == s) as_parent |= 1u << (2 * t3);
				if (p.triples[t3][1] == s) as_parent |= 1u << (2 * t3 + 1);
				if (p.triples[t3][2] == s) as_child |= 3u << (2 * t3);
			}
			if (as_parent && as_child) continue;
			if (!as_parent && !as_child) continue;
			of_individual[s] = (int)tflip.size();
			tflip.push_back(as_parent | as_child);
		}
	}
	void orient(const Problem& p, uint32_t c_last, BtChunk& ch) const {
		ch.n_orient = 1;
		for (uint32_t q = 0; q < BT_GENERATORS; ++q) ch.flip[q] = 0;
		if (p.n_triples == 0 && p.n_ind <= 1) {
			const uint32_t fb = p.f[c_last];
			ch.flip[0] = fb >= BT_STATE_TSHIFT ? BT_STATE_XMASK : ((1u << fb) - 1u);
			ch.n_orient = 2;
			return;
		}
		if (tflip.empty()) return;
		const ColumnEntry* col = p.col_begin(c_last);
		uint32_t bit = 0;
		for (uint32_t j = 0; j < p.k[c_last]; ++j) {
			if (!((p.fwd_mask[c_last] >> j) & 1u)) continue;
			const int gq = of_individual[col[j].sample];
			if (gq >= 0) ch.flip[gq] |= 1u << bit;
			++bit;
		}
		for (size_t q = 0; q < tflip.size(); ++q) ch.flip[q] |= tflip[q] << BT_STATE_TSHIFT;
		ch.n_orient = 1u << tflip.size();
	}
};

}

whamd_status_t DeviceTable::Impl::make_chunks(const Problem& p, TableUploader& up, std::string& msg) {
	Impl& m = *this;
	const uint32_t n = p.n_cols;
	m.use_chunks = false;
	m.chunks.clear();
	m.n_spec = 0;
	for (SlotRun& run : m.splan.runs) run.spec_id = 0;
	const bool trio_runs = !m.use_slots && !m.plan.ped_columns.empty();
	if (trio_runs) for (ResSegment& sgm : m.plan.segments) sgm.in_mirror_bit = 0;
	m.dp.spec_keys = nullptr;
	if (!((m.use_slots || trio_runs) && m.jobs.size() == 1 && !m.windowed && !getenv("WHAMD_BT_SEQUENTIAL") && m.units.size() > 2u * BT_CHUNK_RUNS)) return WHAMD_OK;
	m.use_chunks = true;
	const OrientationGenerators generators(p);
	BtChunk cur{};
	cur.n_orient = 1;
	uint32_t runs_in_chunk = 0;
	for (uint32_t u = 0; u < m.units.size(); ++u) {
		const bool is_run = m.units[u].kind == 2 || m.units[u].kind == 3 || (trio_runs && m.units[u].kind == 1);
		if (is_run && runs_in_chunk >= (uint32_t)BT_CHUNK_RUNS && u > 0) {
			m.chunks.push_back(cur);
			cur = BtChunk{};
			cur.unit_off = u;
			cur.spec_id = ++m.n_spec;
			generators.orient(p, m.units[u].c0 + m.units[u].ncols - 1, cur);
			runs_in_chunk = 0;
			const Step& st = m.plan.steps[m.jobs[0].steps[m.jobs[0].steps.size() - 1 - u]];
			if (trio_runs) m.plan.segments[st.index].in_mirror_bit = m.n_spec;
			else m.splan.runs[st.index].spec_id = m.n_spec;
		}
		runs_in_chunk += is_run;
		++cur.unit_count;
	}
	m.chunks.push_back(cur);
	HIP_TRY(up.up((void**)&m.d_chunks, m.chunks.data(), m.chunks.size() * sizeof(BtChunk)));
	m.n_orient_max = 1;
	for (const BtChunk& ch : m.chunks) m.n_orient_max = std::max(m.n_orient_max, ch.n_orient);
	HIP_TRY(up.alloc((void**)&m.d_unit_x, (size_t)m.n_orient_max * m.units.size() * 4));
	HIP_TRY(up.alloc((void**)&m.d_path2, (size_t)m.n_orient_max * n * 4));
	HIP_TRY(up.alloc((void**)&m.d_trans2, (size_t)m.n_orient_max * n * 4));
	HIP_TRY(up.alloc((void**)&m.d_sel, m.units.size() + 16));
	HIP_TRY(up.alloc((void**)&m.d_guess, m.chunks.size() * 4));
	uint32_t stride = 64;
	for (const SlotRun& run : m.splan.runs) if (run.spec_id) stride = std::max(stride, (run.threads >> 6) << (run.g - run.half));
	if (trio_runs) for (const ResSegment& sgm : m.plan.segments) if (sgm.in_mirror_bit) stride = std::max(stride, (sgm.threads >> 6) << sgm.g);
	m.dp.spec_stride = stride;
	HIP_TRY(up.alloc((void**)&m.dp.spec_keys, ((size_t)m.n_spec + 1) * stride * 8));
	return WHAMD_OK;
}

whamd_status_t DeviceTable::Impl::take_solve_buffers(const Problem& p, TableBuild& b, TableUploader& up, std::string& msg) {
	Impl& m = *this;
	HIP_TRY(up.up((void**)&m.d_units, m.units.data(), m.units.size() * sizeof(BtUnit)));
	{
		uint32_t max_stage = 0;
		for (const ResSegment& sgm : m.plan.segments) max_stage = std::max(max_stage, sgm.stage_words);
		for (size_t ri = 0; ri < m.splan.runs.size(); ++ri)
			max_stage = std::max(max_stage, b.ped_slots ? m.splan.pextra[ri].rec_words / 2u : (m.splan.runs[ri].n_ends * m.splan.runs[ri].threads + 7) / 8);
		m.bt_lds = (size_t)2 * RES_MAXCOLS * 128 + 512 + 16 + (size_t)BT_CELLS * 4 + (size_t)RES_MAXCOLS * 4 + (size_t)max_stage * 8 + 16;
		m.chunk_lds = (size_t)(32 + 4 + BT_CELLS + BT_CHUNK_BLOB) * 4 + (size_t)max_stage * 8 + 16;
	}
	void* d_rtab = nullptr;
	const bool ped_plan = !m.plan.ped_columns.empty();
	HIP_TRY(up.alloc(&d_rtab, m.plan.columns.size() * (ped_plan ? PED_TABLE : RES_TABLE) * sizeof(int32_t)));
	m.dp.res_tables = ped_plan ? nullptr : (int32_t*)d_rtab;
	m.dp.ped_tables = ped_plan ? (int32_t*)d_rtab : nullptr;
	b.laps.lap("jobs, backtrace units, schedule");
	b.laps.next_stage();
	{
		size_t got = 0;
		void* d_bt = arena_take(m.device, b.bt, got);
		if (!d_bt) {
			HIP_TRY(hipMalloc(&d_bt, std::max<size_t>(b.bt, 16)));
			got = std::max<size_t>(b.bt, 16);
		}
		m.d_arena = d_bt;
		m.arena_bytes = got;
		m.dp.bt = (uint8_t*)d_bt;
	}
	b.laps.next_stage();
	m.key_entries = (size_t)(1ull << b.max_keys_f) * p.T;
	HIP_TRY(up.alloc((void**)&m.dp.keys, m.key_entries * 8));
	HIP_TRY(up.alloc((void**)&m.dp.last_keys, (size_t)MAX_T_WIDE * 8));
	HIP_TRY(up.alloc((void**)&m.d_pr[0], b.exchange_bytes));
	HIP_TRY(up.alloc((void**)&m.d_pr[1], b.exchange_bytes));
	HIP_TRY(pinned_take((m.super_off + (m.device_superreads ? m.super_words : 0)) * sizeof(uint32_t), (void**)&m.h_pinned, &m.h_pinned_bytes));
	return WHAMD_OK;
}

whamd_status_t DeviceTable::Impl::make_lanes(const TableBuild& b, TableUploader& up, std::string& msg) {
	Impl& m = *this;
	const size_t lane_bytes = 2 * b.exchange_bytes;
	const size_t by_memory = std::max<size_t>(1, ((size_t)1 << 30) / std::max<size_t>(lane_bytes, 1));
	const size_t n_lanes = std::max<size_t>(1, std::min<size_t>(std::min<size_t>((size_t)m.max_lanes, by_memory), m.jobs.size()));
	m.lanes.assign(n_lanes, Impl::Lane());
	std::vector<uint64_t> load(n_lanes, 0);
	std::vector<uint32_t> order;
	for (uint32_t j = 1; j < m.jobs.size(); ++j) order.push_back(j);
	std::stable_sort(order.begin(), order.end(), [&m](uint32_t x, uint32_t y) { return m.jobs[x].steps.size() > m.jobs[y].steps.size(); });
	m.lanes[0].jobs.push_back(0);
	load[0] = m.jobs[0].steps.size() + 1;
	for (uint32_t j : order) {
		const size_t l = (size_t)(std::min_element(load.begin(), load.end()) - load.begin());
		m.lanes[l].jobs.push_back(j);
		load[l] += m.jobs[j].steps.size() + 1;
	}
	m.lanes[0].d_pr[0] = m.d_pr[0];
	m.lanes[0].d_pr[1] = m.d_pr[1];
	m.lanes[0].d_keys = m.dp.keys;
	for (size_t l = 1; l < n_lanes; ++l) {
		HIP_TRY(up.alloc((void**)&m.lanes[l].d_pr[0], b.exchange_bytes));
		HIP_TRY(up.alloc((void**)&m.lanes[l].d_pr[1], b.exchange_bytes));
		HIP_TRY(up.alloc((void**)&m.lanes[l].d_keys, m.key_entries * 8));
	}
	return WHAMD_OK;
}

whamd_status_t DeviceTable::Impl::make_schedule(const TableBuild& b, std::string& msg) {
	Impl& m = *this;
	const bool ped_slots = b.ped_slots;
	struct Cursor { size_t job_i = 0, step_i = 0; uint32_t flip = 0; };
	std::vector<Cursor> cur(m.lanes.size());
	for (;;) {
		Impl::SuperStep ss;
		ss.entry_off = (uint32_t)(m.use_slots ? m.slot_entries.size() : m.entries.size());
		for (size_t li = 0; li < m.lanes.size(); ++li) {
			Impl::Lane& lane = m.lanes[li];
			Cursor& c = cur[li];
			if (c.job_i == lane.jobs.size()) continue;
			const uint32_t job_id = lane.jobs[c.job_i];
			const Impl::Job& job = m.jobs[job_id];
			const uint32_t si = job.steps[c.step_i];
			const bool first = c.step_i == 0, last = c.step_i + 1 == job.steps.size();
			const Step& step = m.plan.steps[si];
			ss.io[0] = lane.d_pr[c.flip]; ss.io[1] = lane.d_pr[c.flip ^ 1];
			if (step.kind == 2) {
				SlotBatchEntry e{};
				e.run = m.splan.runs[step.index];
// ... 171 lines not shown
		K(resident_segment_ped<false, true>),
		WHAMD_RUNX(24, false), WHAMD_RUNX(32, false), WHAMD_RUNX(0, false), WHAMD_RUNX(8, false), WHAMD_RUNX(16, false),
		K(slot_groupx<2, false>), K(slot_groupx<3, false>),
#ifdef WHAMD_DEBUG_BUILD
		WHAMD_RUNX(24, true), WHAMD_RUNX(32, true),
		WHAMD_PSLOTX(2, 2), WHAMD_PSLOTX(2, 4), WHAMD_PSLOTX(4, 2), WHAMD_PSLOTX(4, 4), WHAMD_PSLOTX(2, 16), WHAMD_PSLOTX(2, PSLOT_FACT),
#endif
		WHAMD_PSLOT(2, 4), WHAMD_PSLOT(4, 2), WHAMD_PSLOT(4, 4),
		WHAMD_PSLOT(2, 16), K(pedslot_group<2, 16>),
		WHAMD_PSLOT(2, PSLOT_FACT), K(pedslot_group<2, PSLOT_FACT>),
		WHAMD_PSLOT(4, PSLOT_FACT4), K(pedslot_group<4, PSLOT_FACT4>),
		K(pedslot_group<2, 2>), K(pedslot_group<2, 4>), K(pedslot_group<4, 2>), K(pedslot_group<4, 4>),
	};
#undef K
#undef WHAMD_RUNX
#undef WHAMD_PSLOT
#undef WHAMD_PSLOTX
	count = sizeof(kernels) / sizeof(kernels[0]);
	return kernels;
}

static whamd_status_t opt_in_large_lds(int device, std::string& msg) {
	static std::mutex attr_mu;
	static unsigned long long attr_done = 0;
	std::lock_guard<std::mutex> lock(attr_mu);
	if (device < 64 && ((attr_done >> device) & 1ull)) return WHAMD_OK;
	size_t count = 0;
	const void* const* kernels = large_lds_kernels(count);
	for (size_t i = 0; i < count; ++i) HIP_TRY(hipFuncSetAttribute(kernels[i], hipFuncAttributeMaxDynamicSharedMemorySize, 160 * 1024));
	if (device < 64) attr_done |= 1ull << device;
	return WHAMD_OK;
}

whamd_status_t DeviceTable::Impl::record_group_backtrace(uint32_t n, TableUploader& up, std::string& msg) {
	Impl& m = *this;
	m.d_bt_entry = nullptr;
	if (!m.use_chunks) return WHAMD_OK;
	BtGroupEntry& e = m.h_bt_entry;
	e = BtGroupEntry{};
	e.P = m.dp;
	e.units = m.d_units; e.chunks = m.d_chunks;
	e.n_chunks = (uint32_t)m.chunks.size(); e.n_units = (uint32_t)m.units.size(); e.n_orient_max = m.n_orient_max; e.n_cols = n;
	e.path2 = m.d_path2; e.trans2 = m.d_trans2; e.out_score = m.d_score; e.unit_x2 = m.d_unit_x; e.guess = m.d_guess; e.sel = m.d_sel; e.counters = m.d_bt_counters;
	e.path_index = m.d_path_index; e.path_trans = m.d_path_trans;
	if (m.device_superreads) e.super = m.super_args;
	void* d_entry = nullptr;
	HIP_TRY(up.alloc(&d_entry, sizeof(BtGroupEntry)));
	HIP_TRY(hipMemcpyAsync(d_entry, &m.h_bt_entry, sizeof(BtGroupEntry), hipMemcpyHostToDevice, up.stream));
	HIP_TRY(hipEventRecord(m.ev_upload, up.stream));
	m.d_bt_entry = (BtGroupEntry*)d_entry;
	return WHAMD_OK;
}

whamd_status_t DeviceTable::upload(Problem& p, int device, std::string& msg) {
	Impl& m = *impl_;
	whamd_status_t st = m.open(device, msg);
	if (st != WHAMD_OK || p.n_cols == 0) return st;
	TableBuild b;
	b.n = p.n_cols;
	b.tbits = 2 * p.n_triples;
	b.ni = std::max<uint32_t>(p.n_ind, 1);
	m.dp.n_cols = b.n;
	m.dp.T = p.T;
	m.dp.tbits = b.tbits;
	m.dp.n_ind = p.n_ind;
	if ((st = m.choose_plan(p, b, msg)) != WHAMD_OK) return st;
	b.ped_slots = m.use_slots && m.splan.ped;
	b.laps.next_stage();
	if (debug_env("WHAMD_DEBUG_PLAN")) m.dump_plan(p);
	if ((st = m.describe_columns(p, b, msg)) != WHAMD_OK) return st;
	if ((st = m.lay_out_arena(p, b, msg)) != WHAMD_OK) return st;
	m.upload_stream = debug_env("WHAMD_UPLOAD_ON_TABLE_STREAM") ? nullptr : upload_stream_of(device);
	if (!m.upload_stream) m.upload_stream = m.stream;
	if (m.upload_stream == m.stream) m.own_stream_used = true;
	TableUploader up(device, m.upload_stream, m.allocations);
	b.laps.lap("staging area taken");
	up.open_block(m.upload_bound(p, b));
	b.laps.lap("staging image sized, device block taken");
	if ((st = m.upload_column_arrays(p, b, up, msg)) != WHAMD_OK) return st;
	if ((st = m.upload_slot_arrays(b, up, msg)) != WHAMD_OK) return st;
	m.make_jobs();
	m.make_units(b);
	if ((st = m.make_windows(b, up, msg)) != WHAMD_OK) return st;
	if ((st = m.take_result_block(b.n, up, msg)) != WHAMD_OK) return st;
	if ((st = m.make_chunks(p, up, msg)) != WHAMD_OK) return st;
	if ((st = m.take_solve_buffers(p, b, up, msg)) != WHAMD_OK) return st;
	if ((st = m.make_lanes(b, up, msg)) != WHAMD_OK) return st;
	if ((st = m.make_schedule(b, msg)) != WHAMD_OK) return st;
	m.make_briefs();
	if ((st = m.upload_entries(up, msg)) != WHAMD_OK) return st;
	if ((st = m.launch_table_kernels(p, b, up, msg)) != WHAMD_OK) return st;
	b.laps.summary((double)b.bt / 1e9);
	if ((st = m.arm_debug_stamps(up, msg)) != WHAMD_OK) return st;
	if ((st = opt_in_large_lds(device, msg)) != WHAMD_OK) return st;
	return m.record_group_backtrace(b.n, up, msg);
}

namespace {

SegmentFn segment_kernel(bool stamps, bool sym) {
#ifdef WHAMD_DEBUG_BUILD
	if (stamps) return resident_segment<true, true>;
#endif
	return sym ? resident_segment<false, true> : resident_segment<false, false>;
}

PedSegmentFn ped_segment_kernel(bool stamps, bool spec) {
#ifdef WHAMD_DEBUG_BUILD
	if (stamps) return resident_segment_ped<true>;
#endif
	return spec ? resident_segment_ped<false, true> : resident_segment_ped<false>;
}

ResBatchFn resident_batch_kernel(bool sym) { return sym ? resident_batch<true> : resident_batch<false>; }

#ifdef WHAMD_DEBUG_BUILD
PedSlotRunFn pedslot_runx_kernel(uint32_t tb, uint32_t nf, uint32_t xc, bool spec) {
#define WHAMD_ROW(TB, NF) { pedslot_runx<TB, NF, 16, true>, pedslot_runx<TB, NF, 16, false>, pedslot_runx<TB, NF, 32, true>, pedslot_runx<TB, NF, 32, false> }
	static const PedSlotRunFn table[6][4] = {WHAMD_ROW(2, PSLOT_FACT), WHAMD_ROW(2, 16), WHAMD_ROW(2, 2), WHAMD_ROW(2, 4), WHAMD_ROW(4, 2), WHAMD_ROW(4, 4)};
#undef WHAMD_ROW
	const int row = tb == 2 ? (nf == (uint32_t)PSLOT_FACT ? 0 : nf == 16 ? 1 : nf == 2 ? 2 : 3) : (nf == 2 ? 4 : 5);
	return table[row][(xc == 16 ? 0 : 2) + (spec ? 0 : 1)];
}
#endif

PedSlotRunFn pedslot_run_kernel(uint32_t tb, uint32_t nf, bool spec, bool packed) {
#define WHAMD_ROW(TB, NF) { pedslot_run<TB, NF, true, true>, pedslot_run<TB, NF, true, false>, pedslot_run<TB, NF, false, true>, pedslot_run<TB, NF, false, false> }
	static const PedSlotRunFn table[7][4] = {WHAMD_ROW(2, PSLOT_FACT), WHAMD_ROW(4, PSLOT_FACT4), WHAMD_ROW(2, 16), WHAMD_ROW(2, 2), WHAMD_ROW(2, 4), WHAMD_ROW(4, 2), WHAMD_ROW(4, 4)};
#undef WHAMD_ROW
	const int row = tb == 2 && nf == (uint32_t)PSLOT_FACT ? 0 : tb == 4 && nf == (uint32_t)PSLOT_FACT4 ? 1 : tb == 2 ? (nf == 16 ? 2 : nf == 2 ? 3 : 4) : (nf == 2 ? 5 : 6);
	return table[row][(spec ? 0 : 2) + (packed ? 0 : 1)];
}

SlotRunXFn slot_runx_kernel(uint32_t xc, bool stamps, bool spec) {
#define WHAMD_PAIR(XC, STAMPS) { slot_runx<2, XC, STAMPS, true>, slot_runx<2, XC, STAMPS, false> }
#ifdef WHAMD_DEBUG_BUILD
	static const SlotRunXFn stamped[2][2] = {WHAMD_PAIR(24, true), WHAMD_PAIR(32, true)};
	if (stamps && xc) return stamped[xc == 24 ? 0 : 1][spec ? 0 : 1];
#endif
	static const SlotRunXFn table[5][2] = {WHAMD_PAIR(0, false), WHAMD_PAIR(8, false), WHAMD_PAIR(16, false), WHAMD_PAIR(24, false), WHAMD_PAIR(32, false)};
#undef WHAMD_PAIR
	return table[xc / 8][spec ? 0 : 1];
}

SlotRunFn slot_run_kernel(uint32_t lr, bool yform, bool stamps, bool spec) {
#ifdef WHAMD_DEBUG_BUILD
#define WHAMD_ROW(LR, YF) { slot_run<LR, true, true, YF>, slot_run<LR, true, false, YF>, slot_run<LR, false, true, YF>, slot_run<LR, false, false, YF> }
#else
// ... 57 lines not shown
	const uint32_t c = step.index;
	const DevColumn& d = m.cols[c];
#ifdef WHAMD_DEBUG_BUILD
	const auto column_facts = [&m](const Problem& pr, const DevColumn& col) { LaunchFacts f; f.T = (int32_t)pr.T; f.n_ind = (int32_t)m.dp.n_ind; f.mode = (int32_t)col.mode; f.wide = m.wide; return f; };
#endif
	if (d.mode == 0) {
		const uint32_t threads = 1u << d.f;
		const uint32_t block = std::min<uint32_t>(256, threads);
		hipLaunchKernelGGL(m.fused, dim3(threads / block), dim3(block), 0, rs, dp, c, prev, cur);
		WHAMD_NOTE(m, WHAMD_LAUNCH_COLUMN, (const void*)m.fused, dim3(threads / block), dim3(block), 0, rs, true, column_facts(p, d));
		launches += 1;
	} else {
		const uint64_t total = (1ull << (d.f + d.ebits - d.eloop)) * (m.wide ? p.T : 1u);
		const uint32_t block = (uint32_t)std::min<uint64_t>(256, (total + 63) / 64 * 64);
		if (m.wide) hipLaunchKernelGGL(column_step_wide, dim3((uint32_t)((total + block - 1) / block)), dim3(block), 0, rs, dp, c, prev, (uint32_t)total);
		else hipLaunchKernelGGL(m.keysfn, dim3((uint32_t)((total + block - 1) / block)), dim3(block), 0, rs, dp, c, prev, (uint32_t)total);
		WHAMD_NOTE(m, WHAMD_LAUNCH_COLUMN, m.wide ? (const void*)column_step_wide : (const void*)m.keysfn, dim3((uint32_t)((total + block - 1) / block)), dim3(block), 0, rs, true, column_facts(p, d));
		const uint32_t entries = (1u << d.f) * p.T;
		const uint32_t fblock = std::min<uint32_t>(256, (entries + 63) / 64 * 64);
		hipLaunchKernelGGL(column_finalize, dim3((entries + fblock - 1) / fblock), dim3(fblock), 0, rs, dp, c, cur, entries);
		WHAMD_NOTE(m, WHAMD_LAUNCH_COLUMN, (const void*)column_finalize, dim3((entries + fblock - 1) / fblock), dim3(fblock), 0, rs, true, column_facts(p, d));
		launches += 2;
	}
}

void DeviceTable::Impl::launch_run(const ResBatchEntry& e, uint64_t& launches) {
	Impl& m = *this;
	const ResSegment& sg = e.sg;
	const hipStream_t rs = m.inflight.run_stream;
	const bool stamps = DEBUG_BUILD && m.dp.dbg != nullptr;
#ifdef WHAMD_DEBUG_BUILD
	const auto segment_facts = [&sg, stamps](bool spec, bool sym) {
		LaunchFacts f;
		f.ped = sg.kind == 1; f.stamps = stamps; f.ncols = (int32_t)sg.ncols; f.threads = (int32_t)sg.threads;
		if (sg.kind == 1) f.spec = spec; else f.sym = sym;
		return f;
	};
#endif
	if (sg.kind == 1) {
		const size_t words = ((size_t)sg.ncols * (PED_LDSWORDS + PED_TABLE) + (size_t)sg.n_terms * 2 + 3) & ~(size_t)3;
		const size_t lds_ped = words * 4 + 2 * ((size_t)16 << sg.max_l) + (size_t)sg.stage_words * 8;
		const PedSegmentFn kernel = ped_segment_kernel(stamps, sg.in_mirror_bit && m.use_chunks);
		hipLaunchKernelGGL(kernel, dim3(1u << sg.g), dim3(sg.threads), lds_ped, rs, m.dp, sg, e.prev, e.cur);
		WHAMD_NOTE(m, WHAMD_LAUNCH_RUN, (const void*)kernel, dim3(1u << sg.g), dim3(sg.threads), lds_ped, rs, true, segment_facts(sg.in_mirror_bit && m.use_chunks, false));
	} else {
		const size_t lds = (size_t)sg.ncols * (64 + RES_TABLE) * 4 + 2 * ((size_t)4 << sg.max_l) + (size_t)sg.stage_words * 8;
		const SegmentFn kernel = segment_kernel(stamps, sg.half || sg.in_half || sg.mirror_out);
		hipLaunchKernelGGL(kernel, dim3(1u << (sg.g - sg.half)), dim3(sg.threads), lds, rs, m.dp, sg, e.prev, e.cur, e.score_out);
		WHAMD_NOTE(m, WHAMD_LAUNCH_RUN, (const void*)kernel, dim3(1u << (sg.g - sg.half)), dim3(sg.threads), lds, rs, true, segment_facts(false, sg.half || sg.in_half || sg.mirror_out));
	}
	launches += 1;
}

void DeviceTable::Impl::launch_slot_run(const SlotBatchEntry& e, uint64_t& launches) {
	Impl& m = *this;
	const SlotRun& run = e.run;
	const hipStream_t rs = m.inflight.run_stream;
	const bool spec = run.spec_id != 0 && m.use_chunks && !debug_env("WHAMD_NO_SPEC_KERNEL");
	const bool stamps = DEBUG_BUILD && (m.dp.dbg != nullptr || m.dp.dbg_flags != 0);
	launches += 1;
	if (m.splan.ped) {
		const PedSlotExtra& ex = m.splan.pextra[e.pad];
		size_t lds = pedslot_lds_bytes(run.threads, run.ncols, ex);
		PedSlotRunFn kernel = pedslot_run_kernel(ex.tb, ex.nf, spec, (run.yflags & 16u) != 0);
#ifdef WHAMD_DEBUG_BUILD
		if ((run.yflags & 8u) && !m.side_by_side) {
			const uint32_t xc = run.ncols <= 16u ? 16u : 32u;
			lds = pedslotx_lds_bytes(run.threads, xc);
			kernel = pedslot_runx_kernel(ex.tb, ex.nf, xc, spec);
		}
#endif
		hipLaunchKernelGGL(kernel, dim3(1u << run.g), dim3(run.threads), lds, rs, m.dp, run, ex, e.prev, e.cur);
#ifdef WHAMD_DEBUG_BUILD
		LaunchFacts facts = LaunchFacts::of_run(run, spec, stamps);
		facts.ped = 1; facts.tb = (int32_t)ex.tb; facts.nf = (int32_t)ex.nf; facts.pack = (run.yflags & 16u) != 0;
		WHAMD_NOTE(m, WHAMD_LAUNCH_SLOT_RUN, (const void*)kernel, dim3(1u << run.g), dim3(run.threads), lds, rs, true, facts);
#endif
		return;
	}
	const dim3 grid(1u << (run.g - run.half)), block(run.threads);
	if ((run.yflags & 8u) && run.lr == 2u) {
		const bool streamed = m.side_by_side || debug_env("WHAMD_XSTREAM") || (grid.x >= 1024u && !debug_env("WHAMD_NO_WIDE_LAYOUT"));
		const size_t lds_x = streamed ? (size_t)2 * run.threads * 16 : slotx_lds_bytes(run.threads, (run.ncols + 7u) & ~7u);
		const uint32_t pack = (grid.x <= 32u && !m.side_by_side && !debug_env("WHAMD_NO_XCD_PACK")) ? 1u : 0u;
		const uint32_t xc = streamed ? 0u : (run.ncols <= 8u && !stamps) ? 8u : (run.ncols <= 16u && !stamps) ? 16u : run.ncols <= 24u ? 24u : 32u;
		const SlotRunXFn kernel = slot_runx_kernel(xc, stamps, spec);
		hipLaunchKernelGGL(kernel, dim3(pack ? grid.x * 8u : grid.x), block, lds_x, rs, m.dp, run, e.prev, e.cur, e.score_out, pack);
#ifdef WHAMD_DEBUG_BUILD
		LaunchFacts facts = LaunchFacts::of_run(run, spec, stamps);
		facts.ped = 0; facts.streamed = streamed; facts.pack = (int32_t)pack;
		WHAMD_NOTE(m, WHAMD_LAUNCH_SLOT_RUN, (const void*)kernel, dim3(pack ? grid.x * 8u : grid.x), block, lds_x, rs, true, facts);
#endif
		return;
	}
	const size_t lds = slot_run_lds_bytes(run.threads, run.lr, run.ncols);
	const SlotRunFn kernel = slot_run_kernel(run.lr, (run.yflags & 1u) != 0, stamps, spec);
	hipLaunchKernelGGL(kernel, grid, block, lds, rs, m.dp, run, e.prev, e.cur, e.score_out);
#ifdef WHAMD_DEBUG_BUILD
	LaunchFacts facts = LaunchFacts::of_run(run, spec, stamps);
	facts.ped = 0;
	WHAMD_NOTE(m, WHAMD_LAUNCH_SLOT_RUN, (const void*)kernel, grid, block, lds, rs, true, facts);
#endif
}

whamd_status_t DeviceTable::enqueue_some(const Problem& p, Solution& s, uint64_t budget, bool& done, std::string& msg) {
	const whamd_status_t status = enqueue_some_unguarded(p, s, budget, done, msg);
	if (status != WHAMD_OK) abort_enqueue();
	return status;
}

void DeviceTable::abort_enqueue() {
	Impl& m = *impl_;
	if (m.stream) {
		(void)hipSetDevice(m.device);
		(void)hipStreamSynchronize(m.stream);
		(void)hipGetLastError();
	}
	m.inflight.rewind(m.stream);
}

whamd_status_t DeviceTable::Impl::begin_solve(const Problem& p, Solution& s, std::string& msg) {
	Impl& m = *this;
	const hipStream_t rs = m.inflight.run_stream;
	const uint32_t n = p.n_cols;
	s.path_index.assign(n, 0);
	s.path_trans.assign(n, 0);
	s.superreads_done = false;
	m.inflight.launches = 0;
	m.inflight.next_super = 0;
#ifdef WHAMD_DEBUG_BUILD
	m.ledger.clear();
#endif
	if (n == 0) return WHAMD_OK;
	if (rs == m.stream) m.own_stream_used = true;
	if (m.ev_upload && (m.upload_pending || rs != m.stream)) HIP_TRY(hipStreamWaitEvent(rs, m.ev_upload, 0));
	for (const Impl::Lane& lane : m.lanes) HIP_TRY(hipMemsetAsync(lane.d_keys, 0xFF, m.key_entries * 8, rs));
	HIP_TRY(hipMemsetAsync(m.dp.last_keys, 0xFF, (size_t)MAX_T_WIDE * 8, rs));
	if (m.use_chunks) HIP_TRY(hipMemsetAsync(m.dp.spec_keys, 0xFF, ((size_t)m.n_spec + 1) * m.dp.spec_stride * 8, rs));
	if (m.windowed) HIP_TRY(hipMemsetAsync(m.d_path_trans, 0, (size_t)n * 4, rs));
	m.inflight.timing_pending = false;
	HIP_TRY(hipEventRecord(m.ev0, rs));
	if (!m.plan.ped_columns.empty()) {
		const uint32_t entries = (uint32_t)m.plan.ped_columns.size() * PED_TABLE;
		hipLaunchKernelGGL(ped_tables, dim3((entries + 255) / 256), dim3(256), 0, rs, m.dp.ped_cols, (uint32_t)m.plan.ped_columns.size(), m.dp.ped_tables);
		WHAMD_NOTE(m, WHAMD_LAUNCH_TABLES, (const void*)ped_tables, dim3((entries + 255) / 256), dim3(256), 0, rs, false, LaunchFacts());
	} else if (!m.use_slots && !m.plan.columns.empty()) {
		const uint32_t entries = (uint32_t)m.plan.columns.size() * RES_TABLE;
		hipLaunchKernelGGL(resident_tables, dim3((entries + 255) / 256), dim3(256), 0, rs, m.dp.res_cols, (uint32_t)m.plan.columns.size(), m.dp.res_tables);
		WHAMD_NOTE(m, WHAMD_LAUNCH_TABLES, (const void*)resident_tables, dim3((entries + 255) / 256), dim3(256), 0, rs, false, LaunchFacts());
	}
	return WHAMD_OK;
}

whamd_status_t DeviceTable::Impl::submit_super_step(const Problem& p, const SuperStep& ss, uint64_t& launches, std::string& msg) {
	Impl& m = *this;
	const hipStream_t rs = m.inflight.run_stream;
	const dim3 grid(ss.grid_x, ss.entry_count), block(ss.threads);
	if (ss.ck_load >= 0) HIP_TRY(hipMemcpyAsync(ss.io[0], m.d_checkpoints + (size_t)ss.ck_load * m.checkpoint_bytes, m.checkpoint_bytes, hipMemcpyDeviceToDevice, rs));
	if (ss.entry_count == 1) {
		if (m.use_slots) m.launch_slot_run(m.slot_entries[ss.entry_off], launches);
		else m.launch_run(m.entries[ss.entry_off], launches);
	} else if (ss.entry_count > 1) {
		if (m.use_slots) { const SlotBatchFn kernel = slot_batch_kernel(m.slot_lr_used); hipLaunchKernelGGL(kernel, grid, block, ss.lds, rs, m.dp, m.d_slot_entries + ss.entry_off); }
		else { const ResBatchFn kernel = resident_batch_kernel(ss.sym); hipLaunchKernelGGL(kernel, grid, block, ss.lds, rs, m.dp, m.d_entries + ss.entry_off); }
#ifdef WHAMD_DEBUG_BUILD
		LaunchFacts facts;
		facts.entries = (int32_t)ss.entry_count;
		if (m.use_slots) facts.lr = m.slot_lr_used; else facts.sym = ss.sym;
		WHAMD_NOTE(m, WHAMD_LAUNCH_BATCH, m.use_slots ? (const void*)slot_batch_kernel(m.slot_lr_used) : (const void*)resident_batch_kernel(ss.sym), grid, block, ss.lds, rs, true, facts);
#endif
		launches += 1;
	}
	const whamd_status_t st = m.submit_singles(p, ss, launches, msg);
	if (st != WHAMD_OK) return st;
	if (ss.ck_save >= 0) HIP_TRY(hipMemcpyAsync(m.d_checkpoints + (size_t)ss.ck_save * m.checkpoint_bytes, ss.io[1], m.checkpoint_bytes, hipMemcpyDeviceToDevice, rs));
	if (ss.bt_window >= 0)
	{
		hipLaunchKernelGGL(backtrace_kernel, dim3(1), dim3(1024), m.bt_lds, rs, m.dp, m.d_units, m.d_window_jobs + ss.bt_window,
		                   m.d_path_index, m.d_path_trans, m.d_score);
		WHAMD_NOTE(m, WHAMD_LAUNCH_WINDOW_WALK, (const void*)backtrace_kernel, dim3(1), dim3(1024), m.bt_lds, rs, false, LaunchFacts());
	}
	return WHAMD_OK;
}

whamd_status_t DeviceTable::Impl::submit_singles(const Problem& p, const SuperStep& ss, uint64_t& launches, std::string& msg) {
	Impl& m = *this;
	const hipStream_t rs = m.inflight.run_stream;
	for (const Impl::Single& sg : ss.singles) {
		const Impl::Lane& lane = m.lanes[sg.lane];
		if (sg.zero_prev) HIP_TRY(hipMemsetAsync(lane.d_pr[sg.flip], 0, 4 * (size_t)p.T, rs));
		m.launch_column_step(p, m.plan.steps[sg.step], lane, lane.d_pr[sg.flip], lane.d_pr[sg.flip ^ 1], launches);
		if (sg.score_job >= 0)
			HIP_TRY(hipMemcpyAsync(m.d_job_scores + sg.score_job, lane.d_pr[sg.flip ^ 1], 4, hipMemcpyDeviceToDevice, rs));
	}
	return WHAMD_OK;
}

whamd_status_t DeviceTable::Impl::submit_tail(const Problem& p, std::string& msg, hipStream_t tail_stream, bool walked_by_group) {
	Impl& m = *this;
	const hipStream_t ts = tail_stream ? tail_stream : m.stream;
	m.inflight.tail_elsewhere = ts != m.stream;
	if (ts == m.stream) m.own_stream_used = true;
	m.inflight.tail_stream = ts;
	m.inflight.tail_seq = ++Impl::SolveInFlight::tails_submitted;
	const uint32_t n = p.n_cols;
	HIP_TRY(hipGetLastError());
	if (!walked_by_group) HIP_TRY(hipEventRecord(m.ev1, ts));
	if (walked_by_group) {
	} else if (m.use_chunks) {
		hipLaunchKernelGGL(backtrace_chunks, dim3(m.n_orient_max * (uint32_t)m.chunks.size()), dim3(256), m.chunk_lds, ts, m.dp, m.d_units, m.d_chunks,
		                   (uint32_t)m.chunks.size(), (uint32_t)m.units.size(), 0u, m.n_orient_max, m.d_path2, m.d_trans2, m.d_score, m.d_unit_x, m.d_guess, m.d_sel, m.d_bt_counters);
		hipLaunchKernelGGL(backtrace_chunks, dim3(1), dim3(256), m.chunk_lds, ts, m.dp, m.d_units, m.d_chunks,
		                   (uint32_t)m.chunks.size(), (uint32_t)m.units.size(), 1u, m.n_orient_max, m.d_path2, m.d_trans2, m.d_score, m.d_unit_x, m.d_guess, m.d_sel, m.d_bt_counters);
		hipLaunchKernelGGL(backtrace_gather, dim3((uint32_t)m.units.size()), dim3(64), 0, ts, m.d_units, (uint32_t)m.units.size(), n, m.d_path2, m.d_trans2, m.d_sel,
		                   m.d_path_index, m.d_path_trans);
		WHAMD_NOTE(m, WHAMD_LAUNCH_TAIL, (const void*)backtrace_chunks, dim3(m.n_orient_max * (uint32_t)m.chunks.size()), dim3(256), m.chunk_lds, ts, false, LaunchFacts());
		WHAMD_NOTE(m, WHAMD_LAUNCH_TAIL, (const void*)backtrace_chunks, dim3(1), dim3(256), m.chunk_lds, ts, false, LaunchFacts());
		WHAMD_NOTE(m, WHAMD_LAUNCH_TAIL, (const void*)backtrace_gather, dim3((uint32_t)m.units.size()), dim3(64), 0, ts, false, LaunchFacts());
	} else if (!m.windowed) {
		hipLaunchKernelGGL(backtrace_kernel, dim3((uint32_t)m.jobs.size()), dim3(1024), m.bt_lds, ts, m.dp, m.d_units, m.d_btjobs,
		                   m.d_path_index, m.d_path_trans, m.d_score);
		WHAMD_NOTE(m, WHAMD_LAUNCH_TAIL, (const void*)backtrace_kernel, dim3((uint32_t)m.jobs.size()), dim3(1024), m.bt_lds, ts, false, LaunchFacts());
	}
	HIP_TRY(hipGetLastError());
	HIP_TRY(hipEventRecord(m.ev2, ts));
	if (m.device_superreads && !walked_by_group) {
		hipLaunchKernelGGL(superreads_single, dim3((n + 255u) / 256u), dim3(256), 0, ts, m.super_args);
		WHAMD_NOTE(m, WHAMD_LAUNCH_TAIL, (const void*)superreads_single, dim3((n + 255u) / 256u), dim3(256), 0, ts, false, LaunchFacts());
		HIP_TRY(hipGetLastError());
	}
	HIP_TRY(hipMemcpyAsync(m.h_pinned, m.d_path_index, (m.super_off + (m.device_superreads ? m.super_words : 0)) * sizeof(uint32_t), hipMemcpyDeviceToHost, ts));
	HIP_TRY(hipEventRecord(m.ev3, ts));
	return WHAMD_OK;
}

whamd_status_t DeviceTable::enqueue_some_unguarded(const Problem& p, Solution& s, uint64_t budget, bool& done, std::string& msg) {
	Impl& m = *impl_;
	const uint32_t n = p.n_cols;
	done = false;
	if (n) HIP_TRY(hipSetDevice(m.device));
	if (!m.inflight.enqueue_open) {
		m.inflight.enqueue_open = true;
		m.inflight.run_stream = m.stream;
		m.inflight.group_tables = 1;
		const whamd_status_t st = m.begin_solve(p, s, msg);
		if (st != WHAMD_OK) return st;
		if (n == 0) {
			s.optimal_score = 0;
			m.inflight.enqueue_open = false;
			done = true;
			return WHAMD_OK;
		}
	}
	uint64_t launches = 0;
	while (m.inflight.next_super < m.schedule.size() && launches < budget) {
		const whamd_status_t st = m.submit_super_step(p, m.schedule[m.inflight.next_super++], launches, msg);
		if (st != WHAMD_OK) return st;
	}
	m.inflight.launches += launches;
	if (m.inflight.next_super < m.schedule.size()) return WHAMD_OK;
	const whamd_status_t st = m.submit_tail(p, msg);
	if (st != WHAMD_OK) return st;
	m.inflight.enqueue_open = false;
	done = true;
	return WHAMD_OK;
}

bool DeviceTable::group_eligible(const Problem& p) const {
	const Impl& m = *impl_;
	if (p.n_cols == 0 || !m.use_slots || m.windowed || m.inflight.enqueue_open || m.dp.dbg || (m.dp.dbg_flags && m.splan.ped)) return false;
	if (!m.splan.ped && m.slot_lr_used != 2 && m.slot_lr_used != 3) return false;
	return debug_env("WHAMD_NO_GROUP") == nullptr;
}

int DeviceTable::device_index() const { return impl_->device; }
uint32_t DeviceTable::widest_launch() const { return impl_->max_grid_x; }

struct DeviceTable::Impl::GroupSubmission {
	struct Batch { SlotGroupArgs args; uint32_t grid_x = 0, threads = 0; size_t lds = 0; };
	DeviceTable* const* tables;
	const Problem* const* problems;
	Solution* const* solutions;
	const size_t n;
	Impl& lead;
	std::string& msg;
	bool tight = false;
	size_t max_steps = 0;
	std::vector<Batch> batches;
	std::vector<uint8_t> counted;
	std::vector<uint64_t> table_launches;
	std::vector<uint8_t> walked;
#ifdef WHAMD_DEBUG_BUILD
	const bool touch_fat = debug_env("WHAMD_GROUP_TOUCH_ENTRIES") != nullptr;
	volatile uint64_t fat_sink = 0;
#endif

	GroupSubmission(DeviceTable* const* t, const Problem* const* p, Solution* const* s, size_t n_tables, std::string& m)
		: tables(t), problems(p), solutions(s), n(n_tables), lead(*t[0]->impl_), msg(m), batches(GROUP_VARIANTS), counted(n_tables * GROUP_VARIANTS, 0),
// ... 237 lines not shown
	return WHAMD_OK;
}

whamd_status_t DeviceTable::Impl::report_resident_stamps(std::string& msg) const {
	const Impl& m = *this;
	std::vector<unsigned long long> d(m.plan.segments.size() * 8);
	HIP_TRY(hipMemcpy(d.data(), m.dp.dbg, d.size() * 8, hipMemcpyDeviceToHost));
	unsigned long long a = 0, b = 0, c2 = 0, cols = 0, p1 = 0, p2 = 0, p3 = 0, ns = 0;
	for (size_t i = 0; i < m.plan.segments.size(); ++i) { a += d[8 * i]; b += d[8 * i + 1]; c2 += d[8 * i + 2]; cols += d[8 * i + 3]; p1 += d[8 * i + 4]; p2 += d[8 * i + 5]; p3 += d[8 * i + 6]; ns += d[8 * i + 7]; }
	if (!m.plan.ped_columns.empty() || (m.dp.dbg_flags & 4u))
		fprintf(stderr, "[whamd timing] run prologue (wave 0 of workgroup 0), cycles after the first instruction: kernel arguments usable %.0f, first loaded data %.0f, everything staged %.0f\n",
		        (double)p2 / std::max<unsigned long long>(ns, 1), (double)p3 / std::max<unsigned long long>(ns, 1), (double)p1 / std::max<unsigned long long>(ns, 1));
	else
	fprintf(stderr, "[whamd timing] per barrier step (wave 0 of workgroup 0, %.1f steps per run): hot words %.0f, evaluate %.0f, barrier %.0f cycles\n",
	        (double)ns / m.plan.segments.size(), (double)p1 / std::max<unsigned long long>(ns, 1), (double)p2 / std::max<unsigned long long>(ns, 1), (double)p3 / std::max<unsigned long long>(ns, 1));
	{
		unsigned long long b3[6] = {0, 0, 0, 0, 0, 0};
		HIP_TRY(hipMemcpy(b3, m.dp.dbg + m.dp.dbg_wg_off + 4 * 512 * 2, sizeof b3, hipMemcpyDeviceToHost));
		if (b3[2]) fprintf(stderr, "[whamd timing] backtrace per run: record load + prefetch %.0f cycles, walk + hand-over %.0f cycles (%llu runs); of the latter: local exit index %.0f, chain %.0f, logical indices + stores %.0f\n",
		                   (double)b3[0] / b3[2], (double)b3[1] / b3[2], b3[2], (double)b3[3] / b3[2], (double)b3[4] / b3[2], (double)b3[5] / b3[2]);
	}
	if (m.plan.segments.size() > 104) {
		std::vector<unsigned long long> wg(4 * 512 * 2);
		HIP_TRY(hipMemcpy(wg.data(), m.dp.dbg + m.dp.dbg_wg_off, wg.size() * 8, hipMemcpyDeviceToHost));
		unsigned long long prev_end = 0;
		for (int sgi = 0; sgi < 4; ++sgi) {
			const uint32_t G = 1u << m.plan.segments[100 + sgi].g;
			unsigned long long s0 = ~0ull, s1 = 0, e0 = ~0ull, e1 = 0;
			for (uint32_t ww = 0; ww < G; ++ww) {
				const unsigned long long a2 = wg[((size_t)sgi * 512 + ww) * 2], b2 = wg[((size_t)sgi * 512 + ww) * 2 + 1];
				s0 = std::min(s0, a2); s1 = std::max(s1, a2); e0 = std::min(e0, b2); e1 = std::max(e1, b2);
			}
			fprintf(stderr, "[whamd timing] run %d (%u workgroups): first start +%.2f us after previous run's last end; starts spread %.2f us; first end %.2f us, last end %.2f us after first start\n",
			        100 + sgi, G, prev_end ? (double)(s0 - prev_end) / 100.0 : 0.0, (double)(s1 - s0) / 100.0, (double)(e0 - s0) / 100.0, (double)(e1 - s0) / 100.0);
			prev_end = e1;
		}
	}
	float f01 = 0;
	(void)hipEventElapsedTime(&f01, m.ev0, m.ev1);
	fprintf(stderr, "[whamd timing] segments %zu cols %llu | cycles/segment: prologue %.0f columns %.0f (%.0f per column) store %.0f | fwd %.3f ms, %.2f us per segment\n",
	        m.plan.segments.size(), cols, (double)a / m.plan.segments.size(), (double)b / m.plan.segments.size(),
	        (double)b / std::max<unsigned long long>(cols, 1), (double)c2 / m.plan.segments.size(), f01, f01 * 1e3 / m.plan.segments.size());
	return WHAMD_OK;
}

whamd_status_t DeviceTable::wait(const Problem& p, Solution& s, whamd_solve_stats& st, std::string& msg) {
	Impl& m = *impl_;
	if (p.n_cols == 0) return WHAMD_OK;
	HIP_TRY(hipSetDevice(m.device));
	const uint64_t launches = m.inflight.launches;
	if (m.inflight.tail_elsewhere) HIP_TRY(hipEventSynchronize(m.ev3));
	else { HIP_TRY(hipStreamSynchronize(m.stream)); m.own_stream_used = false; }
	m.upload_pending = false;
	const uint32_t n = p.n_cols;
	std::memcpy(s.path_index.data(), m.h_pinned, (size_t)n * 4);
	std::memcpy(s.path_trans.data(), m.h_pinned + n, (size_t)n * 4);
	s.optimal_score = m.h_pinned[2 * (size_t)n];
	if (m.device_superreads) {
		const uint32_t* q = m.h_pinned + m.super_off;
		const uint8_t* h = (const uint8_t*)(q + n);
		if (std::memchr(h, SUPERREAD_CONFLICT, (size_t)2 * n) == nullptr) {
			s.quality.resize(n);
			s.allele0.resize(n);
			s.allele1.resize(n);
			std::memcpy(s.quality.data(), q, (size_t)n * 4);
			std::memcpy(s.allele0.data(), h, n);
			std::memcpy(s.allele1.data(), h + n, n);
			s.superreads_done = true;
		}
	}
	for (size_t j = 1; j < m.jobs.size(); ++j) s.optimal_score += m.h_pinned[2 * (size_t)n + j];
	st.forward_ms = st.backtrace_ms = st.total_ms = 0;
	m.inflight.timing_pending = true;
	st.forward_launches = launches;
	st.group_tables = m.inflight.group_tables;
	st.bt_chunks = st.bt_missed = st.bt_rewalked = 0;
	if (m.use_chunks) {
		const uint32_t* c = m.h_pinned + 2 * (size_t)n + m.jobs.size();
		st.bt_chunks = (uint32_t)m.chunks.size();
		st.bt_missed = c[0];
		st.bt_rewalked = c[1];
		if (debug_env("WHAMD_BT_STATS")) fprintf(stderr, "[whamd backtrace] %zu chunks, %u guesses missed (%u of them only in the transmission value), %u units walked again (of %zu)\n", m.chunks.size(), c[0], c[2], c[1], m.units.size());
	}
	whamd_status_t reported = m.dp.dbg && m.use_slots ? m.report_slot_stamps(msg) : WHAMD_OK;
	if (reported == WHAMD_OK && m.dp.dbg && !m.plan.segments.empty()) reported = m.report_resident_stamps(msg);
	return reported;
}

#ifdef WHAMD_DEBUG_BUILD
namespace {

template <int T, int NIND>
const void* column_pair(bool keys) {
	FusedFn ff;
	KeysFn kf;
	pick<T, NIND>(ff, kf);
	return keys ? reinterpret_cast<const void*>(kf) : reinterpret_cast<const void*>(ff);
}

const std::vector<whamd_debug_kernel>& solve_kernels() {
#define K(...) {reinterpret_cast<const void*>((__VA_ARGS__)), #__VA_ARGS__, 0, 0}
#define D(...) {reinterpret_cast<const void*>((__VA_ARGS__)), #__VA_ARGS__, 0, 1}
#define WHAMD_COLUMN(T, NIND) {column_pair<T, NIND>(false), "column_step_fused<" #T ", " #NIND ">", 0, 0}, {column_pair<T, NIND>(true), "column_step_keys<" #T ", " #NIND ">", 0, 0}
#define WHAMD_PSLOT(TB, NF) K(pedslot_run<TB, NF, true, true>), K(pedslot_run<TB, NF, true, false>), K(pedslot_run<TB, NF, false, true>), K(pedslot_run<TB, NF, false, false>)
#define WHAMD_PSLOTX(TB, NF) D(pedslot_runx<TB, NF, 16, true>), D(pedslot_runx<TB, NF, 16, false>), D(pedslot_runx<TB, NF, 32, true>), D(pedslot_runx<TB, NF, 32, false>)
#define WHAMD_RUNX(XC) K(slot_runx<2, XC, false, true>), K(slot_runx<2, XC, false, false>)
// ... 4 lines not shown
			WHAMD_COLUMN(4, 3), WHAMD_COLUMN(4, 4), WHAMD_COLUMN(4, 5), WHAMD_COLUMN(4, 6),
			WHAMD_COLUMN(16, 4), WHAMD_COLUMN(16, 5), WHAMD_COLUMN(16, 6),
			K(column_step_wide), K(column_finalize),
			K(ped_tables), K(resident_tables),
			K(resident_segment<false, false>), K(resident_segment<false, true>), D(resident_segment<true, true>),
			K(resident_segment_ped<false>), K(resident_segment_ped<false, true>), D(resident_segment_ped<true>),
			K(resident_batch<false>), K(resident_batch<true>),
			WHAMD_RUN(1, false), WHAMD_RUN(2, false), WHAMD_RUN(2, true), WHAMD_RUN(3, false), WHAMD_RUN(3, true),
			WHAMD_RUNX(0), WHAMD_RUNX(8), WHAMD_RUNX(16), WHAMD_RUNX(24), WHAMD_RUNX(32),
			D(slot_runx<2, 24, true, true>), D(slot_runx<2, 24, true, false>), D(slot_runx<2, 32, true, true>), D(slot_runx<2, 32, true, false>),
			K(slot_batch<1>), K(slot_batch<2>), K(slot_batch<3>),
			WHAMD_PSLOT(2, 2), WHAMD_PSLOT(2, 4), WHAMD_PSLOT(4, 2), WHAMD_PSLOT(4, 4), WHAMD_PSLOT(2, 16), WHAMD_PSLOT(2, PSLOT_FACT), WHAMD_PSLOT(4, PSLOT_FACT4),
			WHAMD_PSLOTX(2, 2), WHAMD_PSLOTX(2, 4), WHAMD_PSLOTX(4, 2), WHAMD_PSLOTX(4, 4), WHAMD_PSLOTX(2, 16), WHAMD_PSLOTX(2, PSLOT_FACT),
			K(slot_group<2, false, false>), K(slot_group<2, false, true>), K(slot_group<3, false, false>), K(slot_group<3, false, true>), D(slot_group<2, true, false>),
			K(slot_groupx<2, false>), K(slot_groupx<3, false>),
			K(pedslot_group<2, 2>), K(pedslot_group<2, 4>), K(pedslot_group<4, 2>), K(pedslot_group<4, 4>), K(pedslot_group<2, 16>),
			K(pedslot_group<2, PSLOT_FACT>), K(pedslot_group<4, PSLOT_FACT4>),
			K(backtrace_kernel), K(backtrace_chunks), K(backtrace_gather), K(superreads_single),
			K(backtrace_chunks_group), K(backtrace_gather_group), K(superreads_group),
		};
		size_t count = 0;
		const void* const* opted = large_lds_kernels(count);
		for (whamd_debug_kernel& k : t) k.large_lds_opted_in = std::find(opted, opted + count, k.kernel) != opted + count;
		return t;
	}();
#undef K
#undef D
#undef WHAMD_COLUMN
#undef WHAMD_PSLOT
#undef WHAMD_PSLOTX
#undef WHAMD_RUNX
#undef WHAMD_RUN
	return table;
}

}

size_t DeviceTable::debug_solve_kernels(whamd_debug_kernel* out, size_t capacity) {
	const std::vector<whamd_debug_kernel>& t = solve_kernels();
	for (size_t i = 0; out && i < t.size() && i < capacity; ++i) out[i] = t[i];
	return t.size();
}

size_t DeviceTable::debug_launches(whamd_debug_launch* out, size_t capacity) const {
	const std::vector<whamd_debug_launch>& ledger = impl_->ledger;
	for (size_t i = 0; out && i < ledger.size() && i < capacity; ++i) {
		out[i] = ledger[i];
		for (const whamd_debug_kernel& k : solve_kernels())
			if (k.kernel == ledger[i].kernel) { out[i].name = k.name; break; }
	}
	return ledger.size();
}

void DeviceTable::Impl::note(uint32_t site, const void* kernel, dim3 grid, dim3 block, size_t lds, hipStream_t on, bool forward, const LaunchFacts& facts) {
	whamd_debug_launch rec = facts;
	rec.kernel = kernel;
	rec.site = site;
	rec.grid_x = grid.x; rec.grid_y = grid.y; rec.block = block.x;
	rec.lds = (uint32_t)lds;
	rec.own_stream = on == stream ? 1u : 0u;
	rec.forward = forward ? 1u : 0u;
	rec.count = 0;
	rec.name = nullptr;
	for (whamd_debug_launch& have : ledger)
		if (std::memcmp(&have, &rec, offsetof(whamd_debug_launch, count)) == 0) { have.count += 1; return; }
	rec.count = 1;
	ledger.push_back(rec);
}
#endif


}
```

whatshap_amd/csrc/slot_plan.cpp:

```cpp
#include <algorithm>
#include <cstdlib>
#include <cstring>
#include <chrono>
#include <iterator>
#include <cstdio>
#include <thread>

#include "debug_build.h"
#include "slots.h"

namespace whamd {

namespace {

struct RunDraft {
	uint32_t c0 = 0, ncols = 0, g = 0, L = 0, lw = 0;
	std::vector<int32_t> entry_read;
	std::vector<int32_t> exit_read;
	bool symmetric = true;
};

inline uint32_t parity32(uint32_t v) { return (uint32_t)__builtin_popcount(v) & 1u; }

}
// ... 298 lines not shown
			}
			const uint32_t ne = ped ? prows_g[rows_mark + i].n_end : rows_g[rows_mark + i].n_end;
			const uint32_t s0 = ped ? prows_g[rows_mark + i].info0 : (rows_g[rows_mark + i].end[0].info & 31u);
			const uint32_t byte = std::min(ne, 3u) | ((ne ? (s0 & 31u) : 0u) << 2);
			if (ped) plan.ctrl[run.ctrl_off + (i >> 2)] |= byte << ((i & 3u) * 8u);
			else {
				const uint32_t qm = ne ? ((rows_g[rows_mark + i].end[0].info >> 8) & 255u) : 0u;
				const uint32_t xbuf = ne ? ((rows_g[rows_mark + i].end[0].info >> 16) & 1u) : 0u;
				plan.ctrl[run.ctrl_off + (i >> 1)] |= (byte | (qm << 7) | (xbuf << 15)) << ((i & 1u) * 16u);
			}
		}
		run.lr = (uint32_t)lr;
		run.row_off = (uint32_t)rows_mark;
		run.n_ends = 0;
		for (size_t i = rows_mark; i < c1; ++i) run.n_ends += ped ? prows_g[i].n_end : rows_g[i].n_end;
		if (ped) {
			PedSlotExtra ex{};
			ex.tb = TB;
			ex.nf = 2;
			for (uint32_t i = 0; i < d.ncols && !genotype_mode; ++i)
				for (uint32_t t = 0; t < p.T; ++t) {
					const uint32_t cnt = (uint32_t)(p.term_end(c + i, t) - p.term_begin(c + i, t));
					ex.nf = std::max(ex.nf, cnt > 4 ? 16u : (cnt > 2 ? 4u : 2u));
				}
			if (fact) ex.nf = fact_nf;
			if (fact_nf == (uint32_t)PSLOT_FACT4) { ex.pad[0] = p.fact4_roles[0]; ex.pad[1] = p.fact4_roles[1]; }
			ex.fwn = d.ncols * pslot_ta(ex.nf, p.T) * pslot_na(ex.nf);
			ex.arow = (ex.fwn + 3u) & ~3u;
			ex.rec_words = ((d.ncols + 3u) / 4u) * (64u << d.lw);
			plan.pextra.push_back(ex);
		}
		run.threads = 64u << d.lw;
		run.has_prev = c > 0;
		run.half = (use_symmetry > 0 && symmetric && g >= 1) ? 1u : 0u;
		for (uint32_t s = 0; s < nslots; ++s) {
			if (d.entry_read[s] >= 0) run.in_occ |= 1u << s;
			if (d.exit_read[s] >= 0) run.out_occ |= 1u << s;
		}
		plan.steps.push_back(Step{2, (uint32_t)plan.runs.size()});
		plan.runs.push_back(run);
		plan.end_off.push_back((uint32_t)ends_mark);
		plan.start_off.push_back((uint32_t)starts_mark);
		drafts.push_back(d);
		plan.n_run_columns += d.ncols;
		c = c1;
	}
	};
	std::vector<RunDraft> drafts;
	const auto tp1 = std::chrono::steady_clock::now();
	const long pf1 = thread_minor_faults();
	long pf2 = pf1;
	auto tp2 = tp1;
	{
		constexpr uint32_t PLAN_PIECE = 8192;
		const uint32_t n_pieces = std::max<uint32_t>(1, n / PLAN_PIECE);
		std::vector<SlotPlan> parts(n_pieces);
		std::vector<std::vector<RunDraft>> part_drafts(n_pieces);
		std::vector<uint32_t> bounds(n_pieces + 1);
		for (uint32_t t = 0; t <= n_pieces; ++t) bounds[t] = (uint32_t)((uint64_t)n * t / n_pieces);
		parallel_ranges(n_pieces, host_threads(n_pieces, 1), [&](uint64_t q0, uint64_t q1, uint32_t) {
			for (uint64_t q = q0; q < q1; ++q) plan_range(bounds[q], bounds[q + 1], parts[q], part_drafts[q]);
		});
		tp2 = std::chrono::steady_clock::now();
		pf2 = thread_minor_faults();
		const uint32_t n_threads = n_pieces;
		{
			size_t n_steps = 0, n_runs = 0, n_ends_all = 0, n_starts = 0, n_ctrl = 0, n_extra = 0;
			for (const SlotPlan& q : parts) {
				n_steps += q.steps.size(); n_runs += q.runs.size(); n_ends_all += q.end_slots.size(); n_starts += q.start_slots.size();
				n_ctrl += q.ctrl.size(); n_extra += q.pextra.size();
			}
			plan.steps.reserve(n_steps); plan.runs.reserve(n_runs); plan.end_off.reserve(n_runs); plan.start_off.reserve(n_runs);
			plan.end_slots.reserve(n_ends_all); plan.start_slots.reserve(n_starts); plan.ctrl.reserve(n_ctrl); plan.pextra.reserve(n_extra);
			drafts.reserve(n_runs);
		}
		for (uint32_t t = 0; t < n_threads; ++t) {
			const SlotPlan& q = parts[t];
			const uint32_t run_base = (uint32_t)plan.runs.size();
			const uint32_t end_base = (uint32_t)plan.end_slots.size(), ctrl_base = (uint32_t)plan.ctrl.size();
			for (Step st : q.steps) { if (st.kind == 2) st.index += run_base; plan.steps.push_back(st); }
			for (SlotRun run : q.runs) { run.ctrl_off += ctrl_base; plan.runs.push_back(run); }
			plan.pextra.insert(plan.pextra.end(), q.pextra.begin(), q.pextra.end());
			for (uint32_t off : q.end_off) plan.end_off.push_back(off + end_base);
			for (uint32_t off : q.start_off) plan.start_off.push_back(off + (uint32_t)plan.start_slots.size());
			plan.start_slots.insert(plan.start_slots.end(), q.start_slots.begin(), q.start_slots.end());
			plan.end_slots.insert(plan.end_slots.end(), q.end_slots.begin(), q.end_slots.end());
			plan.ctrl.insert(plan.ctrl.end(), q.ctrl.begin(), q.ctrl.end());
			plan.n_run_columns += q.n_run_columns;
			drafts.insert(drafts.end(), std::make_move_iterator(part_drafts[t].begin()), std::make_move_iterator(part_drafts[t].end()));
		}
	}
	const auto tp3 = std::chrono::steady_clock::now();
	const long pf3 = thread_minor_faults();
	for (size_t si = 0; si < plan.steps.size(); ++si) {
		const uint32_t c0 = plan.steps[si].kind == 2 ? plan.runs[plan.steps[si].index].c0 : plan.steps[si].index;
		if (!ped && (si == 0 || p.b[c0] == 0)) plan.component_first_step.push_back((uint32_t)si);
	}
	if (!ped && (lr == 2 || lr == 3) && !debug_env("WHAMD_NO_YFORM")) {
		std::vector<uint8_t> pure(n, 0);
		std::vector<uint64_t> B((size_t)n + 1, 0);
		parallel_ranges(n, host_threads(n, 8192), [&](uint64_t c_lo, uint64_t c_hi, uint32_t) {
			for (uint32_t c = (uint32_t)c_lo; c < (uint32_t)c_hi; ++c) {
				uint64_t kstar = 0;
				uint32_t Cp = RES_ABSENT, Cm = RES_ABSENT, Cc = INF;
				for (uint64_t q = p.term_begin(c, 0); q < p.term_end(c, 0); ++q) {
					const CostTerm& t = p.terms[q];
					if (t.plus) Cp = t.c; else if (t.minus) Cm = t.c; else Cc = std::min(Cc, t.c);
				}
				pure[c] = Cp != RES_ABSENT && Cm != RES_ABSENT && Cc == INF;
				if (pure[c]) {
					kstar = (uint64_t)(uint32_t)(Cp + Cm);
				} else {
// ... 152 lines not shown
```

whatshap_amd/csrc/slots.h:

```cpp
#pragma once
#include <cstdint>
#include <memory>
#include <string>
#include <utility>
#include <vector>

#include "problem.h"
#include "host_parallel.h"
#include "resident.h"

namespace whamd {

constexpr int SLOT_LR = 3;
constexpr int SLOT_LANE = 6;
constexpr int SLOT_LWMAX = 3;
constexpr int SLOT_GMAX = 12;
constexpr int SLOT_MAXSLOTS = 26;
constexpr int SLOT_MAXCOLS = 64;
constexpr int SLOT_MAXEND = 8;
constexpr int PSLOT_MAXEND = 4;
constexpr int SLOT_MAXENDS_RUN = 96;
constexpr int32_t SLOT_DELTA_LIMIT = 1 << 22;

struct SlotRow {
// ... 111 lines not shown
	const uint32_t* ctrl;
	uint8_t* bt;
	unsigned long long* spec_keys;
	uint32_t spec_stride, pad2;
};
static_assert(sizeof(SlotBatchEntry) == 320 && sizeof(SlotBatchEntry) % 64 == 0, "entries are fetched with wide scalar loads, whole 64-byte lines");

constexpr int SLOT_GROUP_MAX = 248;
struct SlotGroupArgs {
	uint32_t n, pad;
	const SlotBatchEntry* entry[SLOT_GROUP_MAX];
};

struct SlotBtCol {
	uint8_t k, kf, pad[2];
	uint8_t slot[28];
};
static_assert(sizeof(SlotBtCol) == 32, "SlotBtCol must stay 8 dwords");

struct SlotBtUnit {
	uint32_t kind, c0, ncols, blob_off;
	uint32_t g, L, n_ends, threads;
	uint32_t bt_lo, bt_hi, half, blob_words;
	uint32_t f_exit, lr, pad0[2];
	uint8_t exit_slot[32];
	uint8_t exit_pos[32];
};
static_assert(sizeof(SlotBtUnit) == 128, "SlotBtUnit must stay 32 words");

template <class T>
using NoInitAllocator = NoInitAlloc<T>;

struct SlotPlan {
	std::vector<Step> steps;
	std::vector<SlotRun> runs;
	std::vector<SlotRow, NoInitAllocator<SlotRow>> rows;
	std::vector<SlotBtCol, NoInitAllocator<SlotBtCol>> bt_cols;
	std::vector<uint8_t> end_slots;
	std::vector<uint32_t> end_off;
	std::vector<uint32_t> f_exit;
	std::vector<std::vector<uint8_t>> exit_slot;
	std::vector<uint32_t> ctrl;
	std::vector<int32_t> col_to_row;
	std::vector<uint32_t> component_first_step;
	uint64_t n_run_columns = 0;
	bool ped = false;
	std::vector<uint8_t> start_slots;
	std::vector<uint32_t> start_off;
	std::vector<PedSlotRow, NoInitAllocator<PedSlotRow>> prows;
	std::vector<PedSlotExtra> pextra;
	uint64_t table_words = 0;
};

bool plan_forward_slots(const Problem& p, int l_pref, int use_symmetry, SlotPlan& plan, int lr = 2, bool genotype_mode = false);

bool emulate_slot_plan(const Problem& p, const SlotPlan& plan, std::vector<uint32_t>& path_index, uint32_t& score, std::string& msg);
bool emulate_pedslot_plan(const Problem& p, const SlotPlan& plan, std::vector<uint32_t>& path_index, std::vector<uint32_t>& path_trans,
                          uint32_t& score, std::string& msg);
uint32_t pedslot_table_entry(const Problem& p, const SlotPlan& plan, uint32_t run_index, int kind, uint32_t unit, uint32_t c, uint32_t t, uint32_t f);

}
```

Before: 2.219 million variant-columns/s.

## Launch leading slot runs as a preview during table create, continue in solve

```diff
diff --git a/include/whatshap_amd_debug.h b/include/whatshap_amd_debug.h
--- a/include/whatshap_amd_debug.h
+++ b/include/whatshap_amd_debug.h
@@ -81,10 +81,31 @@
 	int32_t T, n_ind, mode, wide;
 	int32_t ped, sym;
 	int32_t entries;
+	int32_t preview;
+	int32_t reserved;
 	uint64_t count;
 	const char* name;
 } whamd_debug_launch;
 whamd_status_t whamd_debug_dptable_launches(const whamd_dptable* table, whamd_debug_launch* out, size_t capacity, size_t* n_out);
+
+typedef struct whamd_debug_preview {
+	int32_t ran, continued;
+	uint32_t pieces, launched_steps, agreed_steps, reserved;
+	const char* why_not;
+} whamd_debug_preview;
+whamd_status_t whamd_debug_dptable_preview(const whamd_dptable* table, whamd_debug_preview* out);
+
+typedef struct whamd_debug_preview_plan_result {
+	uint32_t n_pieces, pieces, steps, n_steps;
+	int32_t chunked_predicted, chunked, windowed, reserved;
+	uint32_t n_seeds_predicted, n_seeds, stride_predicted, stride;
+	uint64_t arena_predicted, arena_laid_out, exchange_predicted, exchange_laid_out;
+	const char* why_not;
+} whamd_debug_preview_plan_result;
+whamd_status_t whamd_debug_preview_plan(const whamd_readset_view* readset, const uint32_t* recombcost, size_t n_recombcost,
+                                        const whamd_pedigree_view* pedigree, int distrust_genotypes,
+                                        const uint32_t* positions, size_t n_positions, uint32_t pieces, whamd_debug_preview_plan_result* out,
+                                        uint64_t* rec_predicted, uint64_t* rec_laid_out, uint32_t* spec_predicted, uint32_t* spec_laid_out, size_t capacity);
 
 #ifdef __cplusplus
 }
diff --git a/whatshap_amd/_native.py b/whatshap_amd/_native.py
--- a/whatshap_amd/_native.py
+++ b/whatshap_amd/_native.py
@@ -350,6 +350,8 @@
     L.whamd_debug_solve_kernels.argtypes = [C.POINTER(DebugKernel), C.c_size_t]
     L.whamd_debug_dptable_launches.restype = C.c_int
     L.whamd_debug_dptable_launches.argtypes = [C.c_void_p, C.POINTER(DebugLaunch), C.c_size_t, C.POINTER(C.c_size_t)]
+    L.whamd_debug_dptable_preview.restype = C.c_int
+    L.whamd_debug_dptable_preview.argtypes = [C.c_void_p, C.POINTER(DebugPreview)]
     _debug_lib = L
     return L
 
@@ -716,7 +718,47 @@
 
 class DebugLaunch(C.Structure):
     _fields_ = ([("kernel", C.c_void_p), ("site", C.c_uint32), ("grid_x", C.c_uint32), ("grid_y", C.c_uint32), ("block", C.c_uint32), ("lds", C.c_uint32),
-                 ("own_stream", C.c_uint32), ("forward", C.c_uint32)] + [(f, C.c_int32) for f in LAUNCH_FACTS] + [("count", C.c_uint64), ("name", C.c_char_p)])
+                 ("own_stream", C.c_uint32), ("forward", C.c_uint32)] + [(f, C.c_int32) for f in LAUNCH_FACTS] +
+                [("preview", C.c_int32), ("reserved", C.c_int32), ("count", C.c_uint64), ("name", C.c_char_p)])
+
+
+class DebugPreview(C.Structure):
+    _fields_ = [("ran", C.c_int32), ("continued", C.c_int32), ("pieces", C.c_uint32), ("launched_steps", C.c_uint32), ("agreed_steps", C.c_uint32),
+                ("reserved", C.c_uint32), ("why_not", C.c_char_p)]
+
+
+def debug_preview(table) -> dict:
+    D = debug_lib()
+    if table._L is not D:
+        raise ValueError("the preview's record exists in the debug library only (use_debug_library() before the table is made)")
+    out = DebugPreview()
+    _check(D.whamd_debug_dptable_preview(table._h, C.byref(out)), D)
+    return {"ran": bool(out.ran), "continued": bool(out.continued), "pieces": int(out.pieces), "launched_steps": int(out.launched_steps),
+            "agreed_steps": int(out.agreed_steps), "why_not": (out.why_not or b"").decode()}
+
+
+class DebugPreviewPlan(C.Structure):
+    _fields_ = [("n_pieces", C.c_uint32), ("pieces", C.c_uint32), ("steps", C.c_uint32), ("n_steps", C.c_uint32),
+                ("chunked_predicted", C.c_int32), ("chunked", C.c_int32), ("windowed", C.c_int32), ("reserved", C.c_int32),
+                ("n_seeds_predicted", C.c_uint32), ("n_seeds", C.c_uint32), ("stride_predicted", C.c_uint32), ("stride", C.c_uint32),
+                ("arena_predicted", C.c_uint64), ("arena_laid_out", C.c_uint64), ("exchange_predicted", C.c_uint64), ("exchange_laid_out", C.c_uint64),
+                ("why_not", C.c_char_p)]
+
+
+def debug_preview_plan(problem: ProblemArrays, pieces: int = 0) -> dict:
+    D = debug_lib()
+    fn = D.whamd_debug_preview_plan
+    fn.restype = C.c_int
+    out = DebugPreviewPlan()
+    _check(fn(*problem.call_args(), C.c_uint32(pieces), C.byref(out), None, None, None, None, C.c_size_t(0)), D)
+    n = int(out.steps)
+    arrays = {"rec_predicted": np.zeros(max(n, 1), dtype=np.uint64), "rec_laid_out": np.zeros(max(n, 1), dtype=np.uint64),
+              "spec_predicted": np.zeros(max(n, 1), dtype=np.uint32), "spec_laid_out": np.zeros(max(n, 1), dtype=np.uint32)}
+    _check(fn(*problem.call_args(), C.c_uint32(pieces), C.byref(out), _ptr(arrays["rec_predicted"], C.c_uint64), _ptr(arrays["rec_laid_out"], C.c_uint64),
+              _ptr(arrays["spec_predicted"], C.c_uint32), _ptr(arrays["spec_laid_out"], C.c_uint32), C.c_size_t(n)), D)
+    rec = {name: (getattr(out, name).decode() if name == "why_not" else int(getattr(out, name))) for name, _ in DebugPreviewPlan._fields_ if name != "reserved"}
+    rec.update({k: v[:n] for k, v in arrays.items()})
+    return rec
 
 
 def debug_solve_kernels() -> list:
@@ -740,7 +782,7 @@
         if r.name is None:
             raise RuntimeError(f"a launch of site {LAUNCH_SITES[r.site]} (grid {r.grid_x} x {r.grid_y}, block {r.block}) took a kernel the registry does not list")
         rec = {"name": r.name.decode(), "site": LAUNCH_SITES[r.site], "grid_x": r.grid_x, "grid_y": r.grid_y, "block": r.block, "lds": r.lds,
-               "own_stream": bool(r.own_stream), "forward": bool(r.forward), "count": int(r.count)}
+               "own_stream": bool(r.own_stream), "forward": bool(r.forward), "count": int(r.count), "preview": bool(r.preview)}
         rec.update({f: (None if getattr(r, f) < 0 else getattr(r, f)) for f in LAUNCH_FACTS})
         out.append(rec)
     return out
diff --git a/whatshap_amd/blocks.py b/whatshap_amd/blocks.py
--- a/whatshap_amd/blocks.py
+++ b/whatshap_amd/blocks.py
@@ -111,12 +111,12 @@
         n_workers = max(1, min(create_threads, max_in_flight))
         with _create_pool(n_workers) as pool:
             def options_of(window):
-                opts = {}
+                opts = {"preview": "0"}
                 if len(window) > 4:
                     opts["shared_launches"] = "1"
                 if n_workers > 1 and len(window) > 1:
                     opts["host_threads"] = str(max(1, int(host_threads_per_create)))
-                return opts or None
+                return opts
 
             def create(sub, opts):
                 return NativeTable(sub, device=device, path=path, solve=False, options=opts)
diff --git a/whatshap_amd/csrc/c_api.cpp b/whatshap_amd/csrc/c_api.cpp
--- a/whatshap_amd/csrc/c_api.cpp
+++ b/whatshap_amd/csrc/c_api.cpp
@@ -107,12 +107,13 @@
 	if (st != WHAMD_OK) return fail(st, msg);
 	const double t1 = now_ms();
 	t->device_index = device;
+	t->device.set_thread_budget(whamd::host_threads_override() != 0);
 	for (size_t i = 0; i < n_options; ++i) {
 		if (std::string(keys[i]) == "host_threads") continue;
 		st = apply_option(t.get(), keys[i], values[i]);
 		if (st != WHAMD_OK) return st;
 	}
-	st = t->device.upload(t->problem, device, msg);
+	st = t->device.upload(t->problem, device, msg, true);
 	if (st != WHAMD_OK) return fail(st, msg);
 	if (getenv("WHAMD_DEBUG_TIMING"))
 		fprintf(stderr, "[whamd timing] create: flatten %.1f ms, plan + upload %.1f ms\n", t1 - t0, now_ms() - t1);
@@ -457,6 +458,17 @@
 	}
 	if (k == "shared_launches") {
 		t->device.set_shared_launches(v != "0");
+		t->uploaded = false;
+		return WHAMD_OK;
+	}
+	if (k == "preview") {
+		if (v != "auto" && v != "0" && v != "1") return fail(WHAMD_ERR_INVALID, "option preview: auto, 0 or 1 expected, got '" + v + "'");
+		t->device.set_preview(v == "auto" ? -1 : std::atoi(value));
+		t->uploaded = false;
+		return WHAMD_OK;
+	}
+	if (k == "preview_pieces") {
+		t->device.set_preview_pieces((uint32_t)std::max(0, std::atoi(value)));
 		t->uploaded = false;
 		return WHAMD_OK;
 	}
@@ -771,6 +783,27 @@
 	*n_out = table->device.debug_launches(out, capacity);
 	return WHAMD_OK;
 }
+
+whamd_status_t whamd_debug_dptable_preview(const whamd_dptable* table, whamd_debug_preview* out) {
+	if (!table || !out) return fail(WHAMD_ERR_INVALID, "null argument");
+	table->device.debug_preview(out);
+	return WHAMD_OK;
+}
+
+whamd_status_t whamd_debug_preview_plan(const whamd_readset_view* readset, const uint32_t* recombcost, size_t n_recombcost,
+                                        const whamd_pedigree_view* pedigree, int distrust_genotypes,
+                                        const uint32_t* positions, size_t n_positions, uint32_t pieces, whamd_debug_preview_plan_result* out,
+                                        uint64_t* rec_predicted, uint64_t* rec_laid_out, uint32_t* spec_predicted, uint32_t* spec_laid_out, size_t capacity) {
+	return guarded([&]() -> whamd_status_t {
+	if (!out) return fail(WHAMD_ERR_INVALID, "out is NULL");
+	Problem p;
+	std::string msg;
+	whamd_status_t st = build_problem(readset, recombcost, n_recombcost, pedigree, distrust_genotypes != 0, positions, n_positions, p, msg);
+	if (st != WHAMD_OK) return fail(st, msg);
+	st = DeviceTable::debug_preview_plan(p, pieces, out, rec_predicted, rec_laid_out, spec_predicted, spec_laid_out, capacity, msg);
+	return st == WHAMD_OK ? WHAMD_OK : fail(st, msg);
+	});
+}
 #endif
 
 }
diff --git a/whatshap_amd/csrc/device_table.h b/whatshap_amd/csrc/device_table.h
--- a/whatshap_amd/csrc/device_table.h
+++ b/whatshap_amd/csrc/device_table.h
@@ -18,7 +18,7 @@
 
 	static int device_count();
 	static bool device_pci_bus_id(int device, std::string& out);
-	whamd_status_t upload(Problem& p, int device, std::string& msg);
+	whamd_status_t upload(Problem& p, int device, std::string& msg, bool from_create = false);
 	whamd_status_t solve(const Problem& p, Solution& s, whamd_solve_stats& st, std::string& msg);
 	whamd_status_t enqueue(const Problem& p, Solution& s, std::string& msg);
 	whamd_status_t enqueue_some(const Problem& p, Solution& s, uint64_t budget, bool& done, std::string& msg);
@@ -40,11 +40,17 @@
 	void set_lanes(int n);
 	void set_arena_limit(uint64_t bytes);
 	void set_shared_launches(bool v);
+	void set_preview(int mode);
+	void set_preview_pieces(uint32_t pieces);
+	void set_thread_budget(bool v);
 	void set_side_by_side(bool v);
 
 #ifdef WHAMD_DEBUG_BUILD
 	static size_t debug_solve_kernels(whamd_debug_kernel* out, size_t capacity);
 	size_t debug_launches(whamd_debug_launch* out, size_t capacity) const;
+	void debug_preview(whamd_debug_preview* out) const;
+	static whamd_status_t debug_preview_plan(Problem& p, uint32_t pieces, whamd_debug_preview_plan_result* out, uint64_t* rec_predicted, uint64_t* rec_laid_out,
+	                                         uint32_t* spec_predicted, uint32_t* spec_laid_out, size_t capacity, std::string& msg);
 #endif
 
 private:
diff --git a/whatshap_amd/csrc/dp_device.hip b/whatshap_amd/csrc/dp_device.hip
--- a/whatshap_amd/csrc/dp_device.hip
+++ b/whatshap_amd/csrc/dp_device.hip
@@ -342,12 +342,13 @@
 	size_t upload_bound(const Problem& p, const TableBuild& b) const;
 	whamd_status_t upload_column_arrays(const Problem& p, TableBuild& b, TableUploader& up, std::string& msg);
 	void build_slot_blobs(TableBuild& b) const;
-	uint64_t lay_out_slot_tables(const TableBuild& b);
+	uint64_t lay_out_slot_tables(const TableBuild& b, bool report = true);
 	whamd_status_t upload_slot_arrays(TableBuild& b, TableUploader& up, std::string& msg);
 	void make_jobs();
 	void make_units(const TableBuild& b);
 	whamd_status_t make_windows(const TableBuild& b, TableUploader& up, std::string& msg);
 	whamd_status_t take_result_block(uint32_t n, TableUploader& up, std::string& msg);
+	void cut_chunks(const Problem& p);
 	whamd_status_t make_chunks(const Problem& p, TableUploader& up, std::string& msg);
 	whamd_status_t take_solve_buffers(const Problem& p, TableBuild& b, TableUploader& up, std::string& msg);
 	whamd_status_t make_lanes(const TableBuild& b, TableUploader& up, std::string& msg);
@@ -377,8 +378,8 @@
 	struct GroupSubmission;
 	void launch_column_step(const Problem& p, const Step& step, const Lane& lane, const uint32_t* prev, uint32_t* cur, uint64_t& launches);
 	void launch_run(const ResBatchEntry& e, uint64_t& launches);
-	void launch_slot_run(const SlotBatchEntry& e, uint64_t& launches);
-	whamd_status_t begin_solve(const Problem& p, Solution& s, std::string& msg);
+	void launch_slot_run(const DevProblem& dp, const SlotBatchEntry& e, uint64_t& launches);
+	whamd_status_t begin_solve(const Problem& p, Solution& s, std::string& msg, bool behind_preview = false);
 	whamd_status_t submit_super_step(const Problem& p, const SuperStep& ss, uint64_t& launches, std::string& msg);
 	whamd_status_t submit_singles(const Problem& p, const SuperStep& ss, uint64_t& launches, std::string& msg);
 	whamd_status_t submit_tail(const Problem& p, std::string& msg, hipStream_t tail_stream = nullptr, bool walked_by_group = false);
@@ -393,6 +394,48 @@
 	bool upload_pending = false;
 	hipStream_t upload_stream = nullptr;
 
+	enum PreviewWhy : uint32_t { PV_RAN = 0, PV_OFF, PV_NOT_CREATE, PV_NOT_SLOTS, PV_DEBUG_SWITCH, PV_SHARED, PV_THREAD_BUDGET, PV_COMPONENTS, PV_FEW_PIECES, PV_NOT_ALONE, PV_NO_LEADING_RUNS,
+	                           PV_ROW_PAD, PV_ARENA, PV_WHYS };
+	struct Preview {
+		int mode = -1;
+		uint32_t pieces_wanted = 0;
+		bool thread_budget = false;
+		bool counted = false;
+		uint32_t why = PV_NOT_CREATE;
+		uint32_t pieces = 0;
+		uint32_t launched = 0;
+		uint32_t agreed = 0;
+		bool launching = false;
+		bool pending = false;
+		bool continued = false;
+		bool use_chunks = false;
+		uint64_t launches = 0;
+		std::vector<SlotRun> runs;
+		DevProblem dp{};
+		uint32_t* d_pr[2] = {nullptr, nullptr};
+		size_t exchange_bytes = 0;
+		unsigned long long* spec_keys = nullptr;
+		size_t spec_bytes = 0;
+		std::vector<std::pair<void*, size_t>> allocations;
+	} preview;
+	static inline std::atomic<int> tables_on_device[64];
+	void give_preview_block() {
+		for (auto& a : preview.allocations) devpool_give(device, a.first, a.second);
+		preview.allocations.clear();
+	}
+	struct PreviewPlan {
+		uint32_t why = PV_NOT_CREATE, pieces = 0, steps = 0, end_col = 0, n_spec = 0, stride = 64, max_f = 0;
+		bool chunked = false;
+		uint64_t arena = 0, tab_words = 0;
+		size_t ctrl_words = 0;
+		std::vector<uint64_t> rec;
+		std::vector<uint32_t> spec;
+	};
+	void plan_preview(const Problem& p, const TableBuild& b, bool from_create, PreviewPlan& out);
+	whamd_status_t start_preview(const Problem& p, TableBuild& b, bool from_create, std::string& msg);
+	void verify_preview();
+	whamd_status_t arm_keys(std::string& msg);
+
 	void adopt(const StreamSet& ss) { stream = ss.stream; ev0 = ss.ev[0]; ev1 = ss.ev[1]; ev2 = ss.ev[2]; ev3 = ss.ev[3]; ev_group = ss.ev[4]; ev_upload = ss.ev[5]; }
 	StreamSet stream_set() const {
 		StreamSet ss;
@@ -420,6 +463,12 @@
 		if (stream && own_stream_used && (!allocations.empty() || d_arena)) { (void)hipStreamSynchronize(stream); own_stream_used = false; }
 		for (auto& a : allocations) devpool_give(device, a.first, a.second);
 		allocations.clear();
+		give_preview_block();
+		if (preview.why != PV_NOT_CREATE) {
+			Preview fresh;
+			fresh.mode = preview.mode; fresh.pieces_wanted = preview.pieces_wanted; fresh.thread_budget = preview.thread_budget; fresh.counted = preview.counted;
+			preview = std::move(fresh);
+		}
 		arena_give(device, d_arena, arena_bytes);
 		d_arena = nullptr;
 		arena_bytes = 0;
@@ -451,6 +500,8 @@
 		streamset_give(m.stream_set());
 	}
 	m.adopt(StreamSet());
+	if (m.preview.counted && m.device >= 0 && m.device < 64) Impl::tables_on_device[m.device].fetch_sub(1);
+	m.preview.counted = false;
 	m.inflight.run_stream = nullptr;
 	m.inflight.timing_pending = false;
 }
@@ -501,6 +552,9 @@
 void DeviceTable::set_arena_limit(uint64_t bytes) { impl_->arena_limit = bytes; }
 void DeviceTable::set_shared_launches(bool v) { impl_->shared_hint = v; }
 void DeviceTable::set_side_by_side(bool v) { impl_->side_by_side = v; }
+void DeviceTable::set_preview(int mode) { impl_->preview.mode = mode < 0 ? -1 : (mode ? 1 : 0); }
+void DeviceTable::set_preview_pieces(uint32_t pieces) { impl_->preview.pieces_wanted = pieces; }
+void DeviceTable::set_thread_budget(bool v) { impl_->preview.thread_budget = v; }
 void DeviceTable::set_symmetry(int level) { impl_->symmetry = level < 0 ? 0 : (level > 2 ? 2 : level); }
 
 
@@ -515,6 +569,7 @@
 		m.adopt(ss);
 	}
 	m.release();
+	if (!m.preview.counted && dev >= 0 && dev < 64) { Impl::tables_on_device[dev].fetch_add(1); m.preview.counted = true; }
 	return WHAMD_OK;
 }
 
@@ -621,6 +676,19 @@
 	return WHAMD_OK;
 }
 
+static uint32_t column_step_mode(bool force_keys, bool is_last, uint32_t f, uint32_t ebits) { return (!force_keys && !is_last && f >= 6 && ebits <= (uint32_t)QMAX) ? 0u : 1u; }
+static uint64_t column_record_bytes(uint32_t mode, uint32_t T, uint32_t f, uint32_t nplanes) {
+	return mode == 0 ? (uint64_t)nplanes * T * (1ull << (f - 6)) * 8ull : (uint64_t)T * (1ull << f) * 4ull;
+}
+static uint64_t arena_capacity(uint64_t free_b, uint32_t n, uint64_t table_bytes, uint64_t arena_limit) {
+	const uint64_t reserve = (3ull << 30) + (uint64_t)n * 1024ull + table_bytes;
+	uint64_t cap = free_b > reserve ? free_b - reserve : 0;
+	if (arena_limit) cap = std::min<uint64_t>(cap, arena_limit);
+	return cap;
+}
+static uint64_t arena_behind(uint64_t bt, uint64_t bytes) { return (bt + bytes + 15ull) & ~15ull; }
+static uint64_t slot_run_record_bytes(const SlotRun& run) { return (uint64_t)run.n_ends * run.threads * (1ull << (run.g - run.half)); }
+
 whamd_status_t DeviceTable::Impl::lay_out_arena(const Problem& p, TableBuild& b, std::string& msg) {
 	Impl& m = *this;
 	const uint32_t n = b.n;
@@ -629,14 +697,12 @@
 	uint64_t bt = 0, seg_bt = 0;
 	size_t seg_cursor = 0, slot_cursor = 0;
 	uint32_t max_f = 0, max_keys_f = 0;
-	const uint64_t reserve = (3ull << 30) + (uint64_t)n * 1024ull + m.table_bytes;
 	auto slot_record_bytes = [&m, ped_slots](size_t ri) -> uint64_t {
 		const SlotRun& run = m.splan.runs[ri];
 		if (ped_slots) return (uint64_t)m.splan.pextra[ri].rec_words * 4ull << run.g;
-		return (uint64_t)run.n_ends * run.threads * (1ull << (run.g - run.half));
+		return slot_run_record_bytes(run);
 	};
-	uint64_t arena_cap = b.free_b > reserve ? b.free_b - reserve : 0;
-	if (m.arena_limit) arena_cap = std::min<uint64_t>(arena_cap, m.arena_limit);
+	const uint64_t arena_cap = arena_capacity(b.free_b, n, m.table_bytes, m.arena_limit);
 	b.arena_cap = arena_cap;
 	std::vector<uint32_t>& window_first_col = b.window_first_col;
 	uint64_t bt_max = 0;
@@ -692,9 +758,8 @@
 			}
 			d.bt_off = seg_bt;
 		} else {
-			const bool fused_ok = !b.force_keys && !d.is_last && d.f >= 6 && d.ebits <= (uint32_t)QMAX;
-			d.mode = fused_ok ? 0u : 1u;
-			const uint64_t bytes = d.mode == 0 ? (uint64_t)d.nplanes * p.T * (1ull << (d.f - 6)) * 8ull : (uint64_t)p.T * (1ull << d.f) * 4ull;
+			d.mode = column_step_mode(b.force_keys, d.is_last, d.f, d.ebits);
+			const uint64_t bytes = column_record_bytes(d.mode, p.T, d.f, d.nplanes);
 			if (!open_unit(c, bytes)) return unit_too_large(c);
 			d.bt_off = bt;
 			bt += bytes;
@@ -810,7 +875,7 @@
 	});
 }
 
-uint64_t DeviceTable::Impl::lay_out_slot_tables(const TableBuild& b) {
+uint64_t DeviceTable::Impl::lay_out_slot_tables(const TableBuild& b, bool report) {
 	Impl& m = *this;
 	uint64_t slot_tab_words = 0;
 	for (SlotRun& run : m.splan.runs) {
@@ -834,7 +899,7 @@
 		}
 	}
 	slot_tab_words += (uint64_t)SLOT_XCOLS * 64u;
-	if (b.laps.on) {
+	if (b.laps.on && report) {
 		size_t nx = 0, not_y = 0, not_lr = 0, long_run = 0, many_ends = 0;
 		for (const SlotRun& run : m.splan.runs) {
 			nx += (run.yflags & 8u) != 0;
@@ -1056,52 +1121,77 @@
 
 }
 
-whamd_status_t DeviceTable::Impl::make_chunks(const Problem& p, TableUploader& up, std::string& msg) {
-	Impl& m = *this;
-	const uint32_t n = p.n_cols;
+namespace {
+template <class IsRun, class Starts>
+uint32_t cut_chunk_starts(size_t n_units, IsRun is_run, Starts starts) {
+	uint32_t n_spec = 0, runs_in_chunk = 0;
+	for (size_t u = 0; u < n_units; ++u) {
+		const bool run = is_run(u);
+		if (run && runs_in_chunk >= (uint32_t)BT_CHUNK_RUNS && u > 0) {
+			starts(u, ++n_spec);
+			runs_in_chunk = 0;
+		}
+		runs_in_chunk += run;
+	}
+	return n_spec;
+}
+bool backtrace_is_chunked(bool on_runs, size_t n_jobs, bool windowed, size_t n_units) {
+	return on_runs && n_jobs == 1 && !windowed && !getenv("WHAMD_BT_SEQUENTIAL") && n_units > 2u * BT_CHUNK_RUNS;
+}
+uint32_t seed_stride_of(uint32_t stride, const SlotRun& run) { return std::max(stride, (run.threads >> 6) << (run.g - run.half)); }
+}
+
+void DeviceTable::Impl::cut_chunks(const Problem& p) {
+	Impl& m = *this;
 	m.use_chunks = false;
 	m.chunks.clear();
 	m.n_spec = 0;
 	for (SlotRun& run : m.splan.runs) run.spec_id = 0;
 	const bool trio_runs = !m.use_slots && !m.plan.ped_columns.empty();
 	if (trio_runs) for (ResSegment& sgm : m.plan.segments) sgm.in_mirror_bit = 0;
-	m.dp.spec_keys = nullptr;
-	if (!((m.use_slots || trio_runs) && m.jobs.size() == 1 && !m.windowed && !getenv("WHAMD_BT_SEQUENTIAL") && m.units.size() > 2u * BT_CHUNK_RUNS)) return WHAMD_OK;
+	if (!backtrace_is_chunked(m.use_slots || trio_runs, m.jobs.size(), m.windowed, m.units.size())) return;
 	m.use_chunks = true;
 	const OrientationGenerators generators(p);
-	BtChunk cur{};
-	cur.n_orient = 1;
-	uint32_t runs_in_chunk = 0;
-	for (uint32_t u = 0; u < m.units.size(); ++u) {
-		const bool is_run = m.units[u].kind == 2 || m.units[u].kind == 3 || (trio_runs && m.units[u].kind == 1);
-		if (is_run && runs_in_chunk >= (uint32_t)BT_CHUNK_RUNS && u > 0) {
+	BtChunk first{};
+	first.n_orient = 1;
+	m.chunks.push_back(first);
+	m.n_spec = cut_chunk_starts(m.units.size(),
+		[&m, trio_runs](size_t u) { return m.units[u].kind == 2 || m.units[u].kind == 3 || (trio_runs && m.units[u].kind == 1); },
+		[&m, &p, &generators, trio_runs](size_t u, uint32_t id) {
+			m.chunks.back().unit_count = (uint32_t)u - m.chunks.back().unit_off;
+			BtChunk cur{};
+			cur.unit_off = (uint32_t)u;
+			cur.spec_id = id;
+			generators.orient(p, m.units[u].c0 + m.units[u].ncols - 1, cur);
 			m.chunks.push_back(cur);
-			cur = BtChunk{};
-			cur.unit_off = u;
-			cur.spec_id = ++m.n_spec;
-			generators.orient(p, m.units[u].c0 + m.units[u].ncols - 1, cur);
-			runs_in_chunk = 0;
 			const Step& st = m.plan.steps[m.jobs[0].steps[m.jobs[0].steps.size() - 1 - u]];
-			if (trio_runs) m.plan.segments[st.index].in_mirror_bit = m.n_spec;
-			else m.splan.runs[st.index].spec_id = m.n_spec;
-		}
-		runs_in_chunk += is_run;
-		++cur.unit_count;
-	}
-	m.chunks.push_back(cur);
-	HIP_TRY(up.up((void**)&m.d_chunks, m.chunks.data(), m.chunks.size() * sizeof(BtChunk)));
+			if (trio_runs) m.plan.segments[st.index].in_mirror_bit = id;
+			else m.splan.runs[st.index].spec_id = id;
+		});
+	m.chunks.back().unit_count = (uint32_t)m.units.size() - m.chunks.back().unit_off;
 	m.n_orient_max = 1;
 	for (const BtChunk& ch : m.chunks) m.n_orient_max = std::max(m.n_orient_max, ch.n_orient);
+	uint32_t stride = 64;
+	for (const SlotRun& run : m.splan.runs) if (run.spec_id) stride = seed_stride_of(stride, run);
+	if (trio_runs) for (const ResSegment& sgm : m.plan.segments) if (sgm.in_mirror_bit) stride = std::max(stride, (sgm.threads >> 6) << sgm.g);
+	m.dp.spec_stride = stride;
+}
+
+whamd_status_t DeviceTable::Impl::make_chunks(const Problem& p, TableUploader& up, std::string& msg) {
+	Impl& m = *this;
+	const uint32_t n = p.n_cols;
+	m.dp.spec_keys = nullptr;
+	m.cut_chunks(p);
+	if (!m.use_chunks) return WHAMD_OK;
+	const uint32_t stride = m.dp.spec_stride;
+	HIP_TRY(up.up((void**)&m.d_chunks, m.chunks.data(), m.chunks.size() * sizeof(BtChunk)));
 	HIP_TRY(up.alloc((void**)&m.d_unit_x, (size_t)m.n_orient_max * m.units.size() * 4));
 	HIP_TRY(up.alloc((void**)&m.d_path2, (size_t)m.n_orient_max * n * 4));
 	HIP_TRY(up.alloc((void**)&m.d_trans2, (size_t)m.n_orient_max * n * 4));
 	HIP_TRY(up.alloc((void**)&m.d_sel, m.units.size() + 16));
 	HIP_TRY(up.alloc((void**)&m.d_guess, m.chunks.size() * 4));
-	uint32_t stride = 64;
-	for (const SlotRun& run : m.splan.runs) if (run.spec_id) stride = std::max(stride, (run.threads >> 6) << (run.g - run.half));
-	if (trio_runs) for (const ResSegment& sgm : m.plan.segments) if (sgm.in_mirror_bit) stride = std::max(stride, (sgm.threads >> 6) << sgm.g);
-	m.dp.spec_stride = stride;
-	HIP_TRY(up.alloc((void**)&m.dp.spec_keys, ((size_t)m.n_spec + 1) * stride * 8));
+	if (m.preview.spec_keys && m.preview.spec_bytes >= ((size_t)m.n_spec + 1) * stride * 8) m.dp.spec_keys = m.preview.spec_keys;
+	else HIP_TRY(up.alloc((void**)&m.dp.spec_keys, ((size_t)m.n_spec + 1) * stride * 8));
 	return WHAMD_OK;
 }
 
@@ -1124,22 +1214,35 @@
 	b.laps.lap("jobs, backtrace units, schedule");
 	b.laps.next_stage();
 	{
-		size_t got = 0;
-		void* d_bt = arena_take(m.device, b.bt, got);
-		if (!d_bt) {
-			HIP_TRY(hipMalloc(&d_bt, std::max<size_t>(b.bt, 16)));
-			got = std::max<size_t>(b.bt, 16);
-		}
-		m.d_arena = d_bt;
-		m.arena_bytes = got;
-		m.dp.bt = (uint8_t*)d_bt;
+		if (m.d_arena && m.arena_bytes < std::max<size_t>(b.bt, 16)) {
+			HIP_TRY(hipStreamSynchronize(m.stream));
+			arena_give(m.device, m.d_arena, m.arena_bytes);
+			m.d_arena = nullptr;
+			m.arena_bytes = 0;
+		}
+		if (!m.d_arena) {
+			size_t got = 0;
+			void* d_bt = arena_take(m.device, b.bt, got);
+			if (!d_bt) {
+				HIP_TRY(hipMalloc(&d_bt, std::max<size_t>(b.bt, 16)));
+				got = std::max<size_t>(b.bt, 16);
+			}
+			m.d_arena = d_bt;
+			m.arena_bytes = got;
+		}
+		m.dp.bt = (uint8_t*)m.d_arena;
 	}
 	b.laps.next_stage();
 	m.key_entries = (size_t)(1ull << b.max_keys_f) * p.T;
 	HIP_TRY(up.alloc((void**)&m.dp.keys, m.key_entries * 8));
 	HIP_TRY(up.alloc((void**)&m.dp.last_keys, (size_t)MAX_T_WIDE * 8));
-	HIP_TRY(up.alloc((void**)&m.d_pr[0], b.exchange_bytes));
-	HIP_TRY(up.alloc((void**)&m.d_pr[1], b.exchange_bytes));
+	if (m.preview.d_pr[0] && m.preview.exchange_bytes >= b.exchange_bytes) {
+		m.d_pr[0] = m.preview.d_pr[0];
+		m.d_pr[1] = m.preview.d_pr[1];
+	} else {
+		HIP_TRY(up.alloc((void**)&m.d_pr[0], b.exchange_bytes));
+		HIP_TRY(up.alloc((void**)&m.d_pr[1], b.exchange_bytes));
+	}
 	HIP_TRY(pinned_take((m.super_off + (m.device_superreads ? m.super_words : 0)) * sizeof(uint32_t), (void**)&m.h_pinned, &m.h_pinned_bytes));
 	return WHAMD_OK;
 }
@@ -1417,7 +1520,200 @@
 	return WHAMD_OK;
 }
 
-whamd_status_t DeviceTable::upload(Problem& p, int device, std::string& msg) {
+void DeviceTable::Impl::plan_preview(const Problem& p, const TableBuild& b, bool from_create, PreviewPlan& out) {
+	Impl& m = *this;
+	const Preview& pv = m.preview;
+	const uint32_t n = b.n, n_pieces = slot_plan_pieces(n);
+	out = PreviewPlan();
+	auto none = [&out](uint32_t why) { out.why = why; };
+	if (pv.mode == 0 || debug_env("WHAMD_NO_PREVIEW")) return none(PV_OFF);
+	if (!from_create) return none(PV_NOT_CREATE);
+	if (!m.use_slots || m.splan.ped || p.T != 1) return none(PV_NOT_SLOTS);
+	if (debug_env("WHAMD_DEBUG_STAMPS") || debug_env("WHAMD_SLOT_STAMPS") || debug_env("WHAMD_SLOT_SKIP")) return none(PV_DEBUG_SWITCH);
+	if (m.shared_hint || m.side_by_side) return none(PV_SHARED);
+	if (m.plan.component_first_step.size() != 1) return none(PV_COMPONENTS);
+	if (n_pieces < 2) return none(PV_FEW_PIECES);
+	if (pv.mode < 0) {
+		if (pv.thread_budget) return none(PV_THREAD_BUDGET);
+		if (n_pieces < 8) return none(PV_FEW_PIECES);
+		if (m.device < 0 || m.device >= 64 || Impl::tables_on_device[m.device].load() != 1) return none(PV_NOT_ALONE);
+	}
+	out.pieces = std::min(n_pieces - 1, pv.pieces_wanted ? pv.pieces_wanted : std::max(1u, n_pieces / 6));
+	const uint32_t col_limit = slot_plan_piece_begin(n, out.pieces);
+	const std::vector<Step>& steps = m.plan.steps;
+	const std::vector<SlotRun>& runs = m.splan.runs;
+	uint32_t S = 0;
+	while (S < steps.size() && steps[S].kind == 2 && steps[S].index == S && runs[S].c0 + runs[S].ncols <= col_limit) ++S;
+	if (S == 0 || S >= steps.size()) return none(PV_NO_LEADING_RUNS);
+	out.end_col = runs[S - 1].c0 + runs[S - 1].ncols;
+	if ((size_t)out.end_col + SLOT_ROW_PAD > m.splan.rows.size()) return none(PV_ROW_PAD);
+	const uint64_t tab_words_all = m.lay_out_slot_tables(b, false);
+	out.tab_words = (S < runs.size() ? runs[S].tab_g : tab_words_all) + (uint64_t)SLOT_XCOLS * 64u;
+	out.ctrl_words = (size_t)runs[S - 1].ctrl_off + SLOT_CTRL_WORDS;
+	if (tab_words_all >= 0xFFFFFFFFull || out.ctrl_words > m.splan.ctrl.size()) return none(PV_NO_LEADING_RUNS);
+	out.rec.assign(S, 0);
+	uint64_t bt = 0;
+	{
+		const uint64_t cap = arena_capacity(b.free_b, n, m.table_bytes, m.arena_limit);
+		for (size_t k = 0; k < steps.size(); ++k) {
+			uint64_t bytes = 0;
+			if (steps[k].kind == 2) bytes = slot_run_record_bytes(runs[steps[k].index]);
+			else {
+				const uint32_t c = steps[k].index, f = p.f[c], ebits = p.k[c] - f;
+				bytes = column_record_bytes(column_step_mode(b.force_keys, c + 1 == n, f, ebits), p.T, f, ebits + b.tbits);
+			}
+			if (bt + bytes + 16 > cap) return none(PV_ARENA);
+			if (k < S) out.rec[k] = bt;
+			bt = arena_behind(bt, bytes);
+		}
+		if (bt + (1ull << 31) > b.free_b) return none(PV_ARENA);
+	}
+	out.arena = bt;
+	out.spec.assign(S, 0);
+	out.stride = 64;
+	out.chunked = backtrace_is_chunked(true, 1, false, steps.size());
+	if (out.chunked)
+		out.n_spec = cut_chunk_starts(steps.size(), [&steps](size_t u) { return steps[steps.size() - 1 - u].kind == 2; },
+			[&](size_t u, uint32_t id) {
+				const size_t k = steps.size() - 1 - u;
+				out.stride = seed_stride_of(out.stride, runs[steps[k].index]);
+				if (k < S) out.spec[k] = id;
+			});
+	out.max_f = p.max_k;
+	for (const SlotRun& run : runs) out.max_f = std::max(out.max_f, run.L + run.g);
+	out.steps = S;
+	out.why = PV_RAN;
+}
+
+whamd_status_t DeviceTable::Impl::start_preview(const Problem& p, TableBuild& b, bool from_create, std::string& msg) {
+	Impl& m = *this;
+	Preview& pv = m.preview;
+	PreviewPlan pp;
+	m.plan_preview(p, b, from_create, pp);
+	pv.why = pp.why;
+	if (pp.why != PV_RAN) return WHAMD_OK;
+	const uint32_t n = b.n, S = pp.steps, pieces = pp.pieces, end_col = pp.end_col, n_spec = pp.n_spec, stride = pp.stride, max_f = pp.max_f;
+	const uint64_t bt = pp.arena, tab_words = pp.tab_words;
+	const size_t ctrl_words = pp.ctrl_words;
+	const bool chunked = pp.chunked;
+	const std::vector<uint64_t>& rec = pp.rec;
+	const std::vector<uint32_t>& spec = pp.spec;
+	const std::vector<SlotRun>& runs = m.splan.runs;
+	b.laps.lap("preview: steps, offsets, seeds (host)");
+	auto take = [&m](void** out, size_t bytes) {
+		size_t got = 0;
+		const hipError_t e = devpool_take(m.device, std::max<size_t>(bytes, 16), out, &got);
+		if (e == hipSuccess) m.allocations.emplace_back(*out, got);
+		return e;
+	};
+	{
+		size_t got = 0;
+		void* d_bt = arena_take(m.device, bt, got);
+		if (!d_bt) {
+			HIP_TRY(hipMalloc(&d_bt, std::max<size_t>(bt, 16)));
+			got = std::max<size_t>(bt, 16);
+		}
+		m.d_arena = d_bt;
+		m.arena_bytes = got;
+	}
+	pv.exchange_bytes = (size_t)(1ull << max_f) * p.T * 4;
+	HIP_TRY(take((void**)&pv.d_pr[0], pv.exchange_bytes));
+	HIP_TRY(take((void**)&pv.d_pr[1], pv.exchange_bytes));
+	pv.spec_bytes = chunked ? ((size_t)n_spec + 1) * stride * 8 : 0;
+	if (chunked) HIP_TRY(take((void**)&pv.spec_keys, pv.spec_bytes));
+	DevProblem hdp{};
+	hdp.n_cols = n; hdp.T = p.T; hdp.tbits = b.tbits; hdp.n_ind = p.n_ind;
+	{
+		const hipStream_t us = m.upload_stream;
+		TableUploader up(m.device, us, pv.allocations);
+		const size_t row_count = (size_t)end_col + SLOT_ROW_PAD;
+		up.open_block(row_count * sizeof(SlotRow) + ctrl_words * 4 + (size_t)S * sizeof(SlotRun) + 4096);
+		const SlotRun* d_runs = nullptr;
+		HIP_TRY(up.up((void**)&hdp.slot_rows, m.splan.rows.data(), row_count * sizeof(SlotRow)));
+		HIP_TRY(up.up((void**)&hdp.slot_ctrl, m.splan.ctrl.data(), ctrl_words * 4));
+		HIP_TRY(up.up((void**)&d_runs, runs.data(), (size_t)S * sizeof(SlotRun)));
+		HIP_TRY(up.alloc((void**)&hdp.slot_tab, tab_words * 4));
+		HIP_TRY(up.flush());
+		uint32_t most = 0;
+		for (uint32_t k = 0; k < S; ++k) most = std::max<uint32_t>(most, ((runs[k].ncols + 8u) << (runs[k].g - runs[k].half)) + (runs[k].ncols + 8u) * ((runs[k].threads >> 6) + 64u));
+		const uint32_t bx = std::max(1u, std::min(64u, (most + 255u) / 256u));
+		for (uint32_t r0 = 0; r0 < S; r0 += 32768) hipLaunchKernelGGL(slot_tables, dim3(bx, std::min<uint32_t>(32768, S - r0)), dim3(256), 0, us, hdp, d_runs + r0, (uint32_t*)hdp.slot_tab);
+		HIP_TRY(hipGetLastError());
+		HIP_TRY(hipEventRecord(m.ev_upload, us));
+		if (up.unstaged_copies || !up.stage.image || !up.stage.park()) {
+			HIP_TRY(hipStreamSynchronize(us));
+			up.stage.finish();
+		}
+	}
+	b.laps.lap("preview: rows, control words, tables: allocations + copies");
+	{
+		const whamd_status_t opted = opt_in_large_lds(m.device, msg);
+		if (opted != WHAMD_OK) return opted;
+	}
+	const hipStream_t rs = m.stream;
+	m.inflight.run_stream = rs;
+	m.own_stream_used = true;
+	HIP_TRY(hipStreamWaitEvent(rs, m.ev_upload, 0));
+	hdp.bt = (uint8_t*)m.d_arena;
+	hdp.spec_keys = pv.spec_keys;
+	hdp.spec_stride = stride;
+	if (chunked) HIP_TRY(hipMemsetAsync(pv.spec_keys, 0xFF, pv.spec_bytes, rs));
+	m.inflight.timing_pending = false;
+	HIP_TRY(hipEventRecord(m.ev0, rs));
+	m.use_chunks = chunked;
+#ifdef WHAMD_DEBUG_BUILD
+	m.ledger.clear();
+#endif
+	pv.runs.resize(S);
+	uint64_t launches = 0;
+	pv.launching = true;
+	for (uint32_t k = 0; k < S; ++k) {
+		SlotBatchEntry e{};
+		e.run = runs[k];
+		if (k == 0) e.run.has_prev = 0;
+		e.run.rec_lo = (uint32_t)rec[k];
+		e.run.rec_hi = (uint32_t)(rec[k] >> 32);
+		e.run.spec_id = spec[k];
+		e.prev = pv.d_pr[k & 1u];
+		e.cur = pv.d_pr[(k & 1u) ^ 1u];
+		pv.runs[k] = e.run;
+		m.launch_slot_run(hdp, e, launches);
+	}
+	pv.launching = false;
+	HIP_TRY(hipGetLastError());
+	HIP_TRY(hipEventRecord(m.ev3, rs));
+	pv.dp = hdp;
+	pv.use_chunks = chunked;
+	pv.why = PV_RAN;
+	pv.pieces = pieces;
+	pv.launched = S;
+	pv.launches = launches;
+	pv.pending = true;
+	b.laps.lap("preview: launches submitted");
+	return WHAMD_OK;
+}
+
+void DeviceTable::Impl::verify_preview() {
+	Impl& m = *this;
+	Preview& pv = m.preview;
+	pv.agreed = 0;
+	if (!pv.launched) return;
+	const bool same_ground = m.use_slots && !m.windowed && m.jobs.size() == 1 && m.lanes.size() == 1 && m.dp.bt == pv.dp.bt && m.dp.spec_keys == pv.dp.spec_keys &&
+	                         m.use_chunks == pv.use_chunks && (!m.use_chunks || m.dp.spec_stride == pv.dp.spec_stride) && !m.dp.dbg && !m.dp.dbg_flags &&
+	                         m.d_pr[0] == pv.d_pr[0] && m.d_pr[1] == pv.d_pr[1] && !m.side_by_side;
+	for (uint32_t k = 0; same_ground && k < pv.launched && k + 1 < m.schedule.size(); ++k) {
+		const Impl::SuperStep& ss = m.schedule[k];
+		if (ss.entry_count != 1 || !ss.singles.empty() || ss.ck_load >= 0 || ss.ck_save >= 0 || ss.bt_window >= 0) break;
+		const SlotBatchEntry& e = m.slot_entries[ss.entry_off];
+		if (std::memcmp(&e.run, &pv.runs[k], sizeof(SlotRun)) != 0 || e.prev != pv.d_pr[k & 1u] || e.cur != pv.d_pr[(k & 1u) ^ 1u] || e.score_out) break;
+		++pv.agreed;
+	}
+	if (const char* at = debug_env("WHAMD_PREVIEW_MISMATCH_AT")) pv.agreed = std::min<uint32_t>(pv.agreed, (uint32_t)std::max(0, atoi(at)));
+	if (getenv("WHAMD_DEBUG_TIMING"))
+		fprintf(stderr, "[whamd timing] preview: %u plan pieces, %u steps launched, %u agree with the schedule\n", pv.pieces, pv.launched, pv.agreed);
+}
+
+whamd_status_t DeviceTable::upload(Problem& p, int device, std::string& msg, bool from_create) {
 	Impl& m = *impl_;
 	whamd_status_t st = m.open(device, msg);
 	if (st != WHAMD_OK || p.n_cols == 0) return st;
@@ -1433,11 +1729,12 @@
 	b.ped_slots = m.use_slots && m.splan.ped;
 	b.laps.next_stage();
 	if (debug_env("WHAMD_DEBUG_PLAN")) m.dump_plan(p);
-	if ((st = m.describe_columns(p, b, msg)) != WHAMD_OK) return st;
-	if ((st = m.lay_out_arena(p, b, msg)) != WHAMD_OK) return st;
 	m.upload_stream = debug_env("WHAMD_UPLOAD_ON_TABLE_STREAM") ? nullptr : upload_stream_of(device);
 	if (!m.upload_stream) m.upload_stream = m.stream;
 	if (m.upload_stream == m.stream) m.own_stream_used = true;
+	if ((st = m.start_preview(p, b, from_create, msg)) != WHAMD_OK) return st;
+	if ((st = m.describe_columns(p, b, msg)) != WHAMD_OK) return st;
+	if ((st = m.lay_out_arena(p, b, msg)) != WHAMD_OK) return st;
 	TableUploader up(device, m.upload_stream, m.allocations);
 	b.laps.lap("staging area taken");
 	up.open_block(m.upload_bound(p, b));
@@ -1458,7 +1755,9 @@
 	b.laps.summary((double)b.bt / 1e9);
 	if ((st = m.arm_debug_stamps(up, msg)) != WHAMD_OK) return st;
 	if ((st = opt_in_large_lds(device, msg)) != WHAMD_OK) return st;
-	return m.record_group_backtrace(b.n, up, msg);
+	if ((st = m.record_group_backtrace(b.n, up, msg)) != WHAMD_OK) return st;
+	m.verify_preview();
+	return WHAMD_OK;
 }
 
 namespace {
@@ -1622,12 +1921,12 @@
 	launches += 1;
 }
 
-void DeviceTable::Impl::launch_slot_run(const SlotBatchEntry& e, uint64_t& launches) {
+void DeviceTable::Impl::launch_slot_run(const DevProblem& dp, const SlotBatchEntry& e, uint64_t& launches) {
 	Impl& m = *this;
 	const SlotRun& run = e.run;
 	const hipStream_t rs = m.inflight.run_stream;
 	const bool spec = run.spec_id != 0 && m.use_chunks && !debug_env("WHAMD_NO_SPEC_KERNEL");
-	const bool stamps = DEBUG_BUILD && (m.dp.dbg != nullptr || m.dp.dbg_flags != 0);
+	const bool stamps = DEBUG_BUILD && (dp.dbg != nullptr || dp.dbg_flags != 0);
 	launches += 1;
 	if (m.splan.ped) {
 		const PedSlotExtra& ex = m.splan.pextra[e.pad];
@@ -1640,7 +1939,7 @@
 			kernel = pedslot_runx_kernel(ex.tb, ex.nf, xc, spec);
 		}
 #endif
-		hipLaunchKernelGGL(kernel, dim3(1u << run.g), dim3(run.threads), lds, rs, m.dp, run, ex, e.prev, e.cur);
+		hipLaunchKernelGGL(kernel, dim3(1u << run.g), dim3(run.threads), lds, rs, dp, run, ex, e.prev, e.cur);
 #ifdef WHAMD_DEBUG_BUILD
 		LaunchFacts facts = LaunchFacts::of_run(run, spec, stamps);
 		facts.ped = 1; facts.tb = (int32_t)ex.tb; facts.nf = (int32_t)ex.nf; facts.pack = (run.yflags & 16u) != 0;
@@ -1655,7 +1954,7 @@
 		const uint32_t pack = (grid.x <= 32u && !m.side_by_side && !debug_env("WHAMD_NO_XCD_PACK")) ? 1u : 0u;
 		const uint32_t xc = streamed ? 0u : (run.ncols <= 8u && !stamps) ? 8u : (run.ncols <= 16u && !stamps) ? 16u : run.ncols <= 24u ? 24u : 32u;
 		const SlotRunXFn kernel = slot_runx_kernel(xc, stamps, spec);
-		hipLaunchKernelGGL(kernel, dim3(pack ? grid.x * 8u : grid.x), block, lds_x, rs, m.dp, run, e.prev, e.cur, e.score_out, pack);
+		hipLaunchKernelGGL(kernel, dim3(pack ? grid.x * 8u : grid.x), block, lds_x, rs, dp, run, e.prev, e.cur, e.score_out, pack);
 #ifdef WHAMD_DEBUG_BUILD
 		LaunchFacts facts = LaunchFacts::of_run(run, spec, stamps);
 		facts.ped = 0; facts.streamed = streamed; facts.pack = (int32_t)pack;
@@ -1665,7 +1964,7 @@
 	}
 	const size_t lds = slot_run_lds_bytes(run.threads, run.lr, run.ncols);
 	const SlotRunFn kernel = slot_run_kernel(run.lr, (run.yflags & 1u) != 0, stamps, spec);
-	hipLaunchKernelGGL(kernel, grid, block, lds, rs, m.dp, run, e.prev, e.cur, e.score_out);
+	hipLaunchKernelGGL(kernel, grid, block, lds, rs, dp, run, e.prev, e.cur, e.score_out);
 #ifdef WHAMD_DEBUG_BUILD
 	LaunchFacts facts = LaunchFacts::of_run(run, spec, stamps);
 	facts.ped = 0;
@@ -1689,23 +1988,40 @@
 	m.inflight.rewind(m.stream);
 }
 
-whamd_status_t DeviceTable::Impl::begin_solve(const Problem& p, Solution& s, std::string& msg) {
+whamd_status_t DeviceTable::Impl::arm_keys(std::string& msg) {
+	Impl& m = *this;
+	const hipStream_t rs = m.inflight.run_stream;
+	for (const Impl::Lane& lane : m.lanes) HIP_TRY(hipMemsetAsync(lane.d_keys, 0xFF, m.key_entries * 8, rs));
+	HIP_TRY(hipMemsetAsync(m.dp.last_keys, 0xFF, (size_t)MAX_T_WIDE * 8, rs));
+	return WHAMD_OK;
+}
+
+whamd_status_t DeviceTable::Impl::begin_solve(const Problem& p, Solution& s, std::string& msg, bool behind_preview) {
 	Impl& m = *this;
 	const hipStream_t rs = m.inflight.run_stream;
 	const uint32_t n = p.n_cols;
 	s.path_index.assign(n, 0);
 	s.path_trans.assign(n, 0);
 	s.superreads_done = false;
-	m.inflight.launches = 0;
-	m.inflight.next_super = 0;
+	if (m.preview.pending && !behind_preview && rs != m.stream) HIP_TRY(hipStreamWaitEvent(rs, m.ev3, 0));
+	m.preview.pending = false;
+	m.preview.continued = behind_preview;
+	m.inflight.launches = behind_preview ? m.preview.launches : 0;
+	m.inflight.next_super = behind_preview ? m.preview.agreed : 0;
 #ifdef WHAMD_DEBUG_BUILD
-	m.ledger.clear();
+	if (!behind_preview) m.ledger.clear();
 #endif
 	if (n == 0) return WHAMD_OK;
 	if (rs == m.stream) m.own_stream_used = true;
 	if (m.ev_upload && (m.upload_pending || rs != m.stream)) HIP_TRY(hipStreamWaitEvent(rs, m.ev_upload, 0));
-	for (const Impl::Lane& lane : m.lanes) HIP_TRY(hipMemsetAsync(lane.d_keys, 0xFF, m.key_entries * 8, rs));
-	HIP_TRY(hipMemsetAsync(m.dp.last_keys, 0xFF, (size_t)MAX_T_WIDE * 8, rs));
+	{
+		const whamd_status_t armed = m.arm_keys(msg);
+		if (armed != WHAMD_OK) return armed;
+	}
+	if (behind_preview) {
+		m.inflight.timing_pending = false;
+		return WHAMD_OK;
+	}
 	if (m.use_chunks) HIP_TRY(hipMemsetAsync(m.dp.spec_keys, 0xFF, ((size_t)m.n_spec + 1) * m.dp.spec_stride * 8, rs));
 	if (m.windowed) HIP_TRY(hipMemsetAsync(m.d_path_trans, 0, (size_t)n * 4, rs));
 	m.inflight.timing_pending = false;
@@ -1728,7 +2044,7 @@
 	const dim3 grid(ss.grid_x, ss.entry_count), block(ss.threads);
 	if (ss.ck_load >= 0) HIP_TRY(hipMemcpyAsync(ss.io[0], m.d_checkpoints + (size_t)ss.ck_load * m.checkpoint_bytes, m.checkpoint_bytes, hipMemcpyDeviceToDevice, rs));
 	if (ss.entry_count == 1) {
-		if (m.use_slots) m.launch_slot_run(m.slot_entries[ss.entry_off], launches);
+		if (m.use_slots) m.launch_slot_run(m.dp, m.slot_entries[ss.entry_off], launches);
 		else m.launch_run(m.entries[ss.entry_off], launches);
 	} else if (ss.entry_count > 1) {
 		if (m.use_slots) { const SlotBatchFn kernel = slot_batch_kernel(m.slot_lr_used); hipLaunchKernelGGL(kernel, grid, block, ss.lds, rs, m.dp, m.d_slot_entries + ss.entry_off); }
@@ -1813,7 +2129,8 @@
 		m.inflight.enqueue_open = true;
 		m.inflight.run_stream = m.stream;
 		m.inflight.group_tables = 1;
-		const whamd_status_t st = m.begin_solve(p, s, msg);
+		const bool behind_preview = n && m.preview.pending && m.preview.agreed > 0 && m.preview.agreed == m.preview.launched && !m.side_by_side;
+		const whamd_status_t st = m.begin_solve(p, s, msg, behind_preview);
 		if (st != WHAMD_OK) return st;
 		if (n == 0) {
 			s.optimal_score = 0;
@@ -2157,6 +2474,7 @@
 	if (m.inflight.tail_elsewhere) HIP_TRY(hipEventSynchronize(m.ev3));
 	else { HIP_TRY(hipStreamSynchronize(m.stream)); m.own_stream_used = false; }
 	m.upload_pending = false;
+	m.give_preview_block();
 	const uint32_t n = p.n_cols;
 	std::memcpy(s.path_index.data(), m.h_pinned, (size_t)n * 4);
 	std::memcpy(s.path_trans.data(), m.h_pinned + n, (size_t)n * 4);
@@ -2267,6 +2585,76 @@
 	return ledger.size();
 }
 
+static const char* const* preview_why_lines() {
+	static const char* const why[13] = {
+		"", "no preview: switched off", "no preview: not inside whamd_dptable_create", "no preview: not a single-individual table on slot runs", "no preview: a debug switch changes the launches",
+		"no preview: the table shares its launches", "no preview: the create is held to a thread budget", "no preview: more than one connected component", "no preview: too few plan pieces",
+		"no preview: not alone", "no preview: the table does not begin with slot runs", "no preview: too close to the table's end", "no preview: the backtrace arena does not fit one window"};
+	return why;
+}
+
+whamd_status_t DeviceTable::debug_preview_plan(Problem& p, uint32_t pieces, whamd_debug_preview_plan_result* out, uint64_t* rec_predicted, uint64_t* rec_laid_out,
+                                               uint32_t* spec_predicted, uint32_t* spec_laid_out, size_t capacity, std::string& msg) {
+	Impl m;
+	TableBuild b;
+	b.n = p.n_cols;
+	b.tbits = 2 * p.n_triples;
+	b.ni = std::max<uint32_t>(p.n_ind, 1);
+	b.free_b = (size_t)1 << 40;
+	if (p.T != 1 || p.n_cols == 0) { msg = "a single-individual table expected"; return WHAMD_ERR_UNSUPPORTED; }
+	m.wide = !select_kernels(p.T, p.n_ind, m.fused, m.keysfn);
+	m.use_slots = plan_forward_slots(p, std::max(8, m.slot_l), m.symmetry, m.splan, m.slot_lr);
+	if (!m.use_slots) { msg = "the table is not planned on slot runs"; return WHAMD_ERR_UNSUPPORTED; }
+	m.plan = ResidentPlan();
+	m.plan.steps = m.splan.steps;
+	m.plan.component_first_step = m.splan.component_first_step;
+	m.plan.col_to_res.assign(p.n_cols, -1);
+	m.preview.mode = 1;
+	m.preview.pieces_wanted = pieces;
+	Impl::PreviewPlan pp;
+	m.plan_preview(p, b, true, pp);
+	whamd_status_t st = m.describe_columns(p, b, msg);
+	if (st == WHAMD_OK) st = m.lay_out_arena(p, b, msg);
+	if (st != WHAMD_OK) return st;
+	m.build_slot_blobs(b);
+	m.lay_out_slot_tables(b, false);
+	m.make_jobs();
+	m.make_units(b);
+	m.cut_chunks(p);
+	static const char* const* why = preview_why_lines();
+	*out = whamd_debug_preview_plan_result{};
+	out->n_pieces = slot_plan_pieces(p.n_cols);
+	out->pieces = pp.pieces;
+	out->steps = pp.steps;
+	out->n_steps = (uint32_t)m.plan.steps.size();
+	out->why_not = why[pp.why < Impl::PV_WHYS ? pp.why : 0];
+	out->chunked_predicted = pp.chunked; out->chunked = m.use_chunks;
+	out->n_seeds_predicted = pp.n_spec; out->n_seeds = m.n_spec;
+	out->stride_predicted = pp.stride; out->stride = m.use_chunks ? m.dp.spec_stride : 64u;
+	out->arena_predicted = pp.arena; out->arena_laid_out = b.bt;
+	out->windowed = m.windowed;
+	out->exchange_predicted = (uint64_t)(1ull << pp.max_f) * p.T * 4; out->exchange_laid_out = b.exchange_bytes;
+	for (uint32_t k = 0; k < pp.steps && k < capacity; ++k) {
+		const SlotRun& run = m.splan.runs[m.plan.steps[k].index];
+		if (rec_predicted) rec_predicted[k] = pp.rec[k];
+		if (rec_laid_out) rec_laid_out[k] = ((uint64_t)run.rec_hi << 32) | run.rec_lo;
+		if (spec_predicted) spec_predicted[k] = pp.spec[k];
+		if (spec_laid_out) spec_laid_out[k] = run.spec_id;
+	}
+	return WHAMD_OK;
+}
+
+void DeviceTable::debug_preview(whamd_debug_preview* out) const {
+	static const char* const* why = preview_why_lines();
+	const Impl::Preview& pv = impl_->preview;
+	out->ran = pv.why == Impl::PV_RAN;
+	out->continued = pv.continued;
+	out->pieces = pv.pieces;
+	out->launched_steps = pv.launched;
+	out->agreed_steps = pv.agreed;
+	out->why_not = why[pv.why < Impl::PV_WHYS ? pv.why : 0];
+}
+
 void DeviceTable::Impl::note(uint32_t site, const void* kernel, dim3 grid, dim3 block, size_t lds, hipStream_t on, bool forward, const LaunchFacts& facts) {
 	whamd_debug_launch rec = facts;
 	rec.kernel = kernel;
@@ -2275,6 +2663,8 @@
 	rec.lds = (uint32_t)lds;
 	rec.own_stream = on == stream ? 1u : 0u;
 	rec.forward = forward ? 1u : 0u;
+	rec.preview = preview.launching ? 1 : 0;
+	rec.reserved = 0;
 	rec.count = 0;
 	rec.name = nullptr;
 	for (whamd_debug_launch& have : ledger)
diff --git a/whatshap_amd/csrc/slot_plan.cpp b/whatshap_amd/csrc/slot_plan.cpp
--- a/whatshap_amd/csrc/slot_plan.cpp
+++ b/whatshap_amd/csrc/slot_plan.cpp
@@ -374,12 +374,11 @@
 	long pf2 = pf1;
 	auto tp2 = tp1;
 	{
-		constexpr uint32_t PLAN_PIECE = 8192;
-		const uint32_t n_pieces = std::max<uint32_t>(1, n / PLAN_PIECE);
+		const uint32_t n_pieces = slot_plan_pieces(n);
 		std::vector<SlotPlan> parts(n_pieces);
 		std::vector<std::vector<RunDraft>> part_drafts(n_pieces);
 		std::vector<uint32_t> bounds(n_pieces + 1);
-		for (uint32_t t = 0; t <= n_pieces; ++t) bounds[t] = (uint32_t)((uint64_t)n * t / n_pieces);
+		for (uint32_t t = 0; t <= n_pieces; ++t) bounds[t] = slot_plan_piece_begin(n, t);
 		parallel_ranges(n_pieces, host_threads(n_pieces, 1), [&](uint64_t q0, uint64_t q1, uint32_t) {
 			for (uint64_t q = q0; q < q1; ++q) plan_range(bounds[q], bounds[q + 1], parts[q], part_drafts[q]);
 		});
diff --git a/whatshap_amd/csrc/slots.h b/whatshap_amd/csrc/slots.h
--- a/whatshap_amd/csrc/slots.h
+++ b/whatshap_amd/csrc/slots.h
@@ -187,6 +187,10 @@
 	uint64_t table_words = 0;
 };
 
+constexpr uint32_t PLAN_PIECE = 8192;
+inline uint32_t slot_plan_pieces(uint32_t n_cols) { return n_cols / PLAN_PIECE > 1 ? n_cols / PLAN_PIECE : 1; }
+inline uint32_t slot_plan_piece_begin(uint32_t n_cols, uint32_t piece) { return (uint32_t)((uint64_t)n_cols * piece / slot_plan_pieces(n_cols)); }
+
 bool plan_forward_slots(const Problem& p, int l_pref, int use_symmetry, SlotPlan& plan, int lr = 2, bool genotype_mode = false);
 
 bool emulate_slot_plan(const Problem& p, const SlotPlan& plan, std::vector<uint32_t>& path_index, uint32_t& score, std::string& msg);
```

After: 2.302 million variant-columns/s, median of 6. +3.7%, better.
